# liuhuang31/Megatts2_HierSpeechpp

Measured on AMD Instinct MI355X. Metric: 16kHz audio samples/sec (whole node) + RTF, HierSpeech++ vocoder batch=32, higher is better.
Workload: dtype f32; 1 GPU; vocoder-only infer(): 32 utterances x 4 s per GPU (BASELINE.json configs[1]), synthetic weights; batch_per_gpu=32, frames=200, global_batch=32, parallelism=dp1 (contiguous utterance shards of the global batch, one RCCL weight broadcast), launch_mode=hipGraph replay of the captured step

## Files before the change

include/hsp.h:

```cpp
#ifndef HSP_H_
#define HSP_H_

#include <stdint.h>

#ifdef __cplusplus
extern "C" {
#endif
#if defined(__GNUC__) || defined(__clang__)
#pragma GCC visibility push(default)
#endif

#define HSP_VERSION 104
#define HSP_EINVAL (-1)

int hsp_version(void);
const char* hsp_arch(void);


enum {
  HSP_PRO_NONE = 0,
  HSP_PRO_LRELU = 1,
  HSP_PRO_ACT1D = 2,
  HSP_PRO_SILU = 3
};

enum {
  HSP_ACT_NONE = 0,
  HSP_ACT_TANH = 1,
  HSP_ACT_GELU_TANH = 2,
  HSP_ACT_RELU = 3,
  HSP_ACT_MISH = 4,
  HSP_ACT_SILU = 5,
  HSP_ACT_SOFTPLUS = 6,
  HSP_ACT_GELU_ERF = 7
};

enum {
  HSP_ROWS_PLAIN = 0,
  HSP_ROWS_GATE_WN = 1,
  HSP_ROWS_GATE_GLU = 2,
  HSP_ROWS_SHUFFLE = 3
};

enum { HSP_MASK_NONE = 0, HSP_MASK_PRE = 1, HSP_MASK_POST = 2, HSP_MASK_BOTH = 3 };

typedef struct hsp_conv1d_args {
  const float* x;
  int64_t x_bs, x_cs, x_ts;
  int32_t B, Cin, Lin;
  const float* w;
  int32_t K, M, dil, pad, stride;
  const float* zeros;
  int32_t w_ld;
  float* y;
  int64_t y_bs, y_cs;
  int32_t Cout, Lout;
  int32_t ncols;
  int32_t prologue;
  float slope;
  const float* alpha_exp;
  const float* beta_inv;
  const float* filt;
  int32_t rows, gate_half, up, shuf_pad;
  const float* bias;
  const float* cbias;
  int64_t cbias_bs;
  int32_t act;
  const float* mask;
  int64_t mask_bs;
  int32_t mask_mode;
  const float* cscale;
  int64_t cscale_bs;
  float scale;
  const float* res;
  int64_t res_bs, res_cs;
  int32_t accumulate;
  float post_scale;
  int32_t debug;
  const float* ln_c1;
  float ln_eps;
  int32_t split_row;
  int32_t accumulate2;
  int32_t mask_mode2;
  float* y2;
  int64_t y2_bs, y2_cs;
  int64_t res_ts;
  int64_t w_bs;
} hsp_conv1d_args;

int hsp_conv1d_mfma_f32(const hsp_conv1d_args* a, void* stream);
int hsp_conv1d_direct_f32(const hsp_conv1d_args* a, void* stream);
int hsp_conv1d_mfma_plan(const hsp_conv1d_args* a, int32_t out4[4]);

int hsp_act_f32(const float* x, float* y, int64_t n, int32_t act, void* stream);
int hsp_reflect_pad_f32(const float* x, int64_t x_bs, float* y, int32_t B, int32_t L, int32_t pad, void* stream);
int hsp_f0_convert_f32(const float* f0_src, int32_t n_src, const float* f0_trg, int32_t n_trg, float* out, void* stream);

int hsp_reflect_pad_ragged_f32(const float* x, int64_t x_bs, const int64_t* lengths, float* y, int64_t y_bs, int32_t B,
                               int32_t L, int32_t pad, int32_t Lo, void* stream);
int hsp_f0_convert_batch_f32(const float* f0_src, int64_t src_bs, const int64_t* n_src, const float* f0_trg,
                             int64_t trg_bs, const int64_t* n_trg, int32_t nt_max, float* out, int64_t out_bs,
                             int32_t B, int32_t n_max, void* stream);
int hsp_stft_frames_ragged_f32(const float* x, int64_t x_bs, const int64_t* lengths, const float* window, float* frames,
                               int32_t B, int32_t L, int32_t n_fft, int32_t hop, int32_t T, int32_t f_ld, void* stream);
int hsp_abs_max_rows_f32(const float* x, int64_t x_bs, const int64_t* lengths, float* out, int32_t B, int64_t n,
                         void* stream);
int hsp_peak_int16_gains(const float* x, int64_t x_bs, const int64_t* lengths, const float* gains, int16_t* out,
                         int64_t o_bs, int32_t B, int64_t n, void* stream);

int hsp_mag_pha_f32(const float* spec, int64_t s_ld, float* mag, float* pha, int32_t n_freqs, int32_t T, float compress,
                    void* stream);
int hsp_lsigmoid_mul_f32(const float* m, const float* slope, float beta, const float* mag, float* out, int32_t T,
                         int32_t F, void* stream);
int hsp_atan2_f32(const float* y, const float* x, float* out, int64_t n, void* stream);
int hsp_polar_f32(const float* mag, const float* pha, float power, float* re, int64_t re_ld, float* im, int64_t im_ld,
                  int32_t F, int32_t T, void* stream);

int hsp_norm_factor_rows_f32(const float* x, int64_t x_bs, const int64_t* lengths, float* scale, float* inv, int32_t B,
                             int64_t L, void* stream);
int hsp_stft_frames_packed_f32(const float* x, int64_t x_bs, const int64_t* lengths, const float* scale,
                               const float* window, float* frames, const int32_t* seg, const int32_t* seg_host, int32_t B,
                               int64_t L, int32_t n_fft, int32_t hop, int32_t T_tot, int32_t f_ld, void* stream);
int hsp_instnorm_prelu_seg_f32(float* x, int64_t x_cs, int32_t C, int32_t T_tot, int32_t F, const int32_t* seg,
                               const int32_t* seg_host, int32_t B, const float* gamma, const float* beta,
                               const float* slope, float eps, void* stream);
int hsp_zero_gaps_f32(float* x, int64_t x_cs, int32_t C, int32_t T_tot, int32_t F, const int32_t* seg,
                      const int32_t* seg_host, int32_t B, void* stream);
int hsp_dwconv_bn_silu_seg_f32(const float* x, const float* w, const float* bias, const float* bn_weight,
                               const float* bn_bias, const float* bn_mean, const float* bn_var, float bn_eps, float* y,
                               int32_t A, int32_t C, int32_t N, int32_t K, const int32_t* seg, const int32_t* seg_host,
                               int32_t B, void* stream);
int hsp_istft_ola_seg_f32(const float* frames, int64_t f_ld, const float* window, const float* inv, float* out,
                          int64_t out_bs, int64_t n_max, int32_t n_fft, int32_t hop, const int32_t* seg,
                          const int32_t* seg_host, int32_t B, int32_t T_tot, void* stream);

int hsp_act1d_snakebeta_f32(const float* x, float* y, int32_t B, int32_t C, int32_t L,
                            const float* alpha_exp, const float* beta_inv, const float* filt,
                            void* stream);
int hsp_act1d_snakebeta_ragged_f32(const float* x, float* y, int32_t B, int32_t C, int32_t L, const int64_t* lens,
                                   const float* alpha_exp, const float* beta_inv, const float* filt, void* stream);
int hsp_snake_consts_f32(const float* alpha_log, const float* beta_log, float* alpha_exp,
                         float* beta_inv, int32_t C, void* stream);

int hsp_fold_weight_norm_f32(const float* v, const float* g, float* w, int32_t rows, int32_t cols,
                             void* stream);
int hsp_gather_f32(const float* src, const int32_t* map, float* dst, int64_t n, void* stream);

int hsp_sequence_mask_f32(const int64_t* length, float* mask, int32_t B, int32_t T, void* stream);
int hsp_flip_channels_f32(const float* x, float* y, int32_t B, int32_t C, int32_t T, void* stream);
int hsp_sample_prior_f32(const float* stats, const float* noise, const float* mask, float* z,
                         int32_t B, int32_t C, int32_t T, float noise_scale, void* stream);
int hsp_layernorm_mod_f32(const float* x, float* y, int32_t B, int32_t C, int32_t T, float eps,
                          const float* mask, const float* shift, const float* scale, int64_t mod_bs,
                          const float* gamma, const float* beta, void* stream);
typedef struct hsp_mha_args {
  const float *q, *k, *v;
  float* o;
  int64_t q_bs, k_bs, v_bs, o_bs;
  int32_t B, H, D, Tq, Tk;
  float qk_scale;
  const float* mask_q;
  const float* mask_k;
  const float* rel_k;
  const float* rel_v;
  int32_t window;
  int64_t q_cs, k_cs, v_cs, o_cs;
  const float* mask_dense;
  int64_t mask_dense_bs;
} hsp_mha_args;
int hsp_mha_f32(const hsp_mha_args* a, void* stream);
#define HSP_MHA_TOK 0
#define HSP_MHA_MFMA_WHOLE 1
#define HSP_MHA_MFMA_SLAB 2
#define HSP_MHA_MFMA_STREAM 3
#define HSP_MHA_ROW 4
#define HSP_MHA_ROW_STREAM 5
int hsp_mha_plan(const hsp_mha_args* a, int32_t out4[4]);
typedef struct hsp_mha_proj_args {
  const float *q, *k, *v;
  int64_t q_bs, q_cs, k_bs, k_cs, v_bs, v_cs;
  int32_t B, H, D, Tq, Tk;
  float qk_scale;
  const float* wt;
  int32_t M, wt_ld;
  const float* bias;
  const float* mask;
  int64_t mask_bs;
  const float* cscale;
  int64_t cscale_bs;
  const float* res;
  int64_t res_bs, res_cs, res_ts;
  float* y;
  int64_t y_bs, y_cs, y_ts;
  int32_t debug;
  const int64_t* key_len;
} hsp_mha_proj_args;
int hsp_mha_proj_f32(const hsp_mha_proj_args* a, void* stream);
int hsp_mha_proj_supported(int32_t H, int32_t D, int32_t M, int32_t Tk);
int hsp_masked_mean_f32(const float* x, const float* mask, float* out, int32_t B, int32_t C,
                        int32_t T, void* stream);
int hsp_mask_mul_f32(const float* x, const float* mask, float* y, int32_t B, int32_t C, int32_t T, void* stream);
int hsp_linear_interp_f32(const float* x, float* y, int32_t B, int32_t C, int32_t Lin, int32_t Lout, void* stream);
int hsp_linear_interp_ragged_f32(const float* x, float* y, int32_t B, int32_t C, int32_t Lin, int32_t Lout,
                                 const int64_t* lin, const int64_t* lout, void* stream);
int hsp_axpby_f32(const float* x, const float* z, float* y, float a, float b, int64_t n, void* stream);


int hsp_plm_embed_f32(const float* tc, int64_t tc_bs, int64_t tc_cs, int32_t Dtc, const int64_t* codes,
                      int64_t codes_bs, const float* emb, int32_t Demb, int32_t n_emb, const float* pe_t,
                      int32_t P, const float* alpha, float* x, int64_t x_bs, int64_t x_cs, int32_t B, int32_t n,
                      void* stream);
int hsp_plm_embed_step_f32(const float* tc, int64_t tc_bs, int64_t tc_cs, int32_t Dtc, int64_t* codes,
                           int64_t codes_bs, const float* emb, int32_t Demb, int32_t n_emb, const float* pe_t,
                           int32_t P, const float* alpha, float* x, int64_t x_bs, int64_t x_cs, int32_t B, int32_t n,
                           const float* logits, int64_t l_bs, int64_t l_cs, int32_t n_logits, void* stream);
int hsp_argmax_f32(const float* logits, int64_t l_bs, int64_t l_cs, int32_t B, int32_t N, int64_t* out,
                   int64_t out_bs, void* stream);

typedef struct hsp_sample_args {
  float temperature;
  int32_t top_k;
  float top_p;
  float repetition_penalty;
  const int64_t* seeds;
  float* probs;
  int64_t probs_bs;
} hsp_sample_args;
int hsp_plm_embed_sample_f32(const float* tc, int64_t tc_bs, int64_t tc_cs, int32_t Dtc, int64_t* codes,
                             int64_t codes_bs, const float* emb, int32_t Demb, int32_t n_emb, const float* pe_t,
                             int32_t P, const float* alpha, float* x, int64_t x_bs, int64_t x_cs, int32_t B, int32_t n,
                             const float* logits, int64_t l_bs, int64_t l_cs, int32_t n_logits, int32_t j,
                             const hsp_sample_args* args, void* stream);
int hsp_sample_f32(const float* logits, int64_t l_bs, int64_t l_cs, int32_t B, int32_t N, int64_t* out, int64_t out_bs,
                   int32_t j, const hsp_sample_args* args, void* stream);

#define HSP_PLM_DECODE_SPLIT 12
typedef struct hsp_plm_decode_args {
  const float* x;
  int64_t x_bs, x_cs;
  float* y;
  int64_t y_bs, y_cs;
  float *k_cache, *v_cache;
  int64_t bs, cs;
  int32_t t, B, D, H, F;
  float eps;
  const float *g1, *b1, *wqkv_t, *bqkv, *wo_t, *bo, *g2, *b2, *w1_t, *c1, *w2_t, *c2;
  void* workspace;
  int64_t workspace_bytes;
  int32_t debug;
} hsp_plm_decode_args;
int hsp_plm_decode_supported(int32_t D, int32_t H, int32_t F);
int64_t hsp_plm_decode_workspace_bytes(int32_t B, int32_t D);
int hsp_plm_decode_layer_f32(const hsp_plm_decode_args* a, void* stream);
int hsp_plm_decode_layer_pos_f32(const hsp_plm_decode_args* a, const int32_t* pos, void* stream);
int hsp_plm_embed_pos_f32(const float* tc, int64_t tc_bs, int64_t tc_cs, int32_t Dtc, const int64_t* codes,
                          int64_t codes_bs, const float* emb, int32_t Demb, int32_t n_emb, const float* pe_t, int32_t P,
                          const float* alpha, float* x, int64_t x_bs, int64_t x_cs, int32_t B, const int32_t* pos,
                          int32_t max_pos, void* stream);
int hsp_plm_choose_advance_f32(const float* logits, int64_t l_bs, int64_t l_cs, int32_t B, int32_t N, int64_t* codes,
                               int64_t codes_bs, int32_t* pos, const int32_t* len, int32_t max_pos,
                               const hsp_sample_args* args, void* stream);
#define HSP_PLM_PREFILL_MAX_N 65536
typedef struct hsp_plm_prefill_attn_args {
  const float* qkv;
  int64_t q_rs;
  float* out;
  int64_t o_rs;
  float *k_cache, *v_cache;
  int64_t cs;
  int32_t n, D, H;
  int32_t debug;
} hsp_plm_prefill_attn_args;
int hsp_plm_prefill_attn_supported(int32_t D, int32_t H);
int hsp_plm_prefill_attn_f32(const hsp_plm_prefill_attn_args* a, void* stream);
int hsp_copy_strided_f32(const float* x, int64_t s_bs, int64_t s_cs, int64_t s_ts, float* y, int32_t B,
                         int32_t C, int32_t T, void* stream);


int hsp_embedding_sum_f32(const int64_t* id0, const int64_t* id1, const int64_t* id2, const float* tab0,
                          const float* tab1, const float* tab2, int32_t n0, int32_t n1, int32_t n2, float scale,
                          float* out, int64_t o_bs, int64_t o_cs, int32_t B, int32_t C, int32_t T, void* stream);
int hsp_lstm_bidir_f32(const float* xproj, int64_t xp_bs, const float* whh_t, const float* bhh,
                       const int64_t* lengths, float* out, int64_t o_bs, int64_t o_cs, int32_t B, int32_t H,
                       int32_t N, void* stream);
int hsp_duration_f32(const float* logw, int64_t lw_bs, const int64_t* lengths, float length_scale, float* dur,
                     int64_t d_bs, float* frames, int32_t B, int32_t N, void* stream);
int hsp_maxpool1d_f32(const float* x, int64_t x_bs, int64_t x_cs, float* y, int32_t B, int32_t C, int32_t L,
                      int32_t k, void* stream);
int hsp_vq_nearest_f32(const float* x, int64_t x_bs, int64_t x_cs, const float* embed, int64_t* codes, int64_t c_bs,
                       int32_t B, int32_t D, int32_t T, int32_t bins, int32_t rep, int32_t Tout, void* stream);
int hsp_gaussian_upsample_f32(const float* x, int64_t x_bs, int64_t x_cs, const float* dur, int64_t d_bs,
                              const float* rng, int64_t r_bs, const int64_t* lengths, const float* frames,
                              float* out, int32_t B, int32_t C, int32_t N, int32_t T, void* stream);
int hsp_add_cbias_f32(const float* x, int64_t x_bs, int64_t x_cs, const float* cb, int64_t cb_bs, float* y,
                      int32_t B, int32_t C, int32_t T, void* stream);

int hsp_zero_below_f32(const float* x, float thr, float* y, int64_t n, void* stream);
int hsp_peak_int16(const float* x, int64_t x_bs, const int64_t* lengths, float gain, int16_t* out, int64_t o_bs,
                   int32_t B, int64_t n, void* stream);

int64_t hsp_loudness_workspace_bytes(int32_t B, int64_t n);
int hsp_loudness_coefs_f64(int32_t sample_rate, double* coefs);
int hsp_loudness_f32(const float* x, int64_t x_bs, const int64_t* lengths, int32_t B, int64_t n, int32_t sample_rate,
                     void* workspace, int64_t workspace_bytes, float* lufs, float* peak, void* stream);
int hsp_loudness_gains_f32(const float* lufs, const float* peak, float target_lufs, float ceiling, float* gains,
                           int32_t* limited, int32_t B, void* stream);

int hsp_resample_f32(const float* x, int64_t x_bs, const int64_t* lengths, int32_t B, int32_t L, const float* bank,
                     const int32_t* tap0, int32_t n_taps, int32_t o, int32_t n, int32_t width, float* y, int64_t y_bs,
                     int32_t T_out, void* stream);

int hsp_stft_frames_f32(const float* x, const float* window, float* frames, int32_t B, int32_t L, int32_t n_fft,
                        int32_t hop, int32_t T, int32_t f_ld, void* stream);
int hsp_power_mel_log_f32(const float* spec, int64_t s_bs, int32_t s_ld, const float* fb, const int32_t* f_lo,
                          const int32_t* f_hi, float* out, int32_t B, int32_t n_freqs, int32_t n_mels,
                          int32_t T_out, float eps, void* stream);

#define HSP_DFTSEG_TABLE_FLOATS 4160
typedef struct hsp_dftseg_args {
  const float* x;
  int64_t x_bs, x_cs;
  float* y;
  int64_t y_bs, y_cs;
  int32_t B, C, L;
  int32_t k, dil, pad, nseg, Np;
  float* xf;
  int64_t xf_bs;
  const float* dft;
  const float* bias;
  const float* res;
  int64_t res_bs, res_cs;
  int32_t accumulate;
  float post_scale;
  const float* act_alpha_exp;
  const float* act_beta_inv;
  const float* act_filt;
  int32_t prod3;
  const int64_t* act_len;
} hsp_dftseg_args;
int hsp_dftseg_fwd_f32(const hsp_dftseg_args* a, void* stream);
int hsp_dftseg_inv_f32(const hsp_dftseg_args* a, void* stream);
int hsp_dftseg_tables_f32(float* fwd, float* inv);
int hsp_dftseg_pair_supported(const hsp_dftseg_args* inv, const hsp_dftseg_args* fwd);
int hsp_dftseg_pair_f32(const hsp_dftseg_args* inv, const hsp_dftseg_args* fwd, void* stream);

int hsp_dftseg_supported(const hsp_dftseg_args* a);

typedef struct hsp_cprod3_args {
  const float* xf;
  float* yf;
  const float* w;
  const float* zeros;
  int64_t xf_bs, yf_bs;
  int32_t bins, C, Np;
  int32_t debug;
} hsp_cprod3_args;
int hsp_cprod3_f32(const hsp_cprod3_args* a, void* stream);
int hsp_cprod3_supported(const hsp_cprod3_args* a);
#define HSP_WSPEC_BLOCK 0
#define HSP_WSPEC_THREE 1
int hsp_dftseg_weight_spectrum_f32(const float* w, int32_t k, int32_t C, int32_t w_ld, const double* tw, float* out,
                                   int32_t form, void* stream);

int hsp_conv1d_f32(const hsp_conv1d_args* a, void* stream);
int hsp_convtr1d_f32(const hsp_conv1d_args* a, void* stream);
int hsp_wn_layer_f32(const hsp_conv1d_args* in_layer, const hsp_conv1d_args* res, const hsp_conv1d_args* skip,
                     void* stream);
int hsp_ffn_conv_f32(const hsp_conv1d_args* fc1, const hsp_conv1d_args* fc2, void* stream);
int hsp_layernorm_modulate_f32(const float* x, float* y, int32_t B, int32_t C, int32_t T, float eps,
                               const float* mask, const float* shift, const float* scale, int64_t mod_bs,
                               void* stream);

#if defined(__GNUC__) || defined(__clang__)
#pragma GCC visibility pop
#endif
#ifdef __cplusplus
}
#endif
#endif
```

megatts2_hierspeechpp_amd/_lib.py:

```python
from __future__ import annotations

import ctypes as C
import os
from typing import Optional

import torch

_HERE = os.path.dirname(os.path.abspath(__file__))
LIB_PATH = os.environ.get("HSP_LIB", os.path.join(_HERE, "libhsp.so"))

PRO_NONE, PRO_LRELU, PRO_ACT1D, PRO_SILU = 0, 1, 2, 3
ACT_NONE, ACT_TANH, ACT_GELU_TANH, ACT_RELU, ACT_MISH, ACT_SILU, ACT_SOFTPLUS, ACT_GELU_ERF = 0, 1, 2, 3, 4, 5, 6, 7
ROWS_PLAIN, ROWS_GATE_WN, ROWS_GATE_GLU, ROWS_SHUFFLE = 0, 1, 2, 3
MASK_NONE, MASK_PRE, MASK_POST, MASK_BOTH = 0, 1, 2, 3
EINVAL = -1
MHA_TOK, MHA_MFMA_WHOLE, MHA_MFMA_SLAB, MHA_MFMA_STREAM, MHA_ROW, MHA_ROW_STREAM = range(6)

_fp = C.c_void_p


class Conv1dArgs(C.Structure):
    _fields_ = [
        ("x", _fp), ("x_bs", C.c_int64), ("x_cs", C.c_int64), ("x_ts", C.c_int64),
        ("B", C.c_int32), ("Cin", C.c_int32), ("Lin", C.c_int32),
        ("w", _fp), ("K", C.c_int32), ("M", C.c_int32), ("dil", C.c_int32), ("pad", C.c_int32), ("stride", C.c_int32),
        ("zeros", _fp), ("w_ld", C.c_int32),
        ("y", _fp), ("y_bs", C.c_int64), ("y_cs", C.c_int64),
        ("Cout", C.c_int32), ("Lout", C.c_int32), ("ncols", C.c_int32),
        ("prologue", C.c_int32), ("slope", C.c_float),
        ("alpha_exp", _fp), ("beta_inv", _fp), ("filt", _fp),
        ("rows", C.c_int32), ("gate_half", C.c_int32), ("up", C.c_int32), ("shuf_pad", C.c_int32),
        ("bias", _fp), ("cbias", _fp), ("cbias_bs", C.c_int64),
        ("act", C.c_int32),
        ("mask", _fp), ("mask_bs", C.c_int64), ("mask_mode", C.c_int32),
        ("cscale", _fp), ("cscale_bs", C.c_int64), ("scale", C.c_float),
        ("res", _fp), ("res_bs", C.c_int64), ("res_cs", C.c_int64),
        ("accumulate", C.c_int32), ("post_scale", C.c_float), ("debug", C.c_int32),
        ("ln_c1", _fp), ("ln_eps", C.c_float),
        ("split_row", C.c_int32), ("accumulate2", C.c_int32), ("mask_mode2", C.c_int32), ("y2", _fp),
        ("y2_bs", C.c_int64), ("y2_cs", C.c_int64), ("res_ts", C.c_int64), ("w_bs", C.c_int64),
    ]


class MhaArgs(C.Structure):
    _fields_ = [
        ("q", _fp), ("k", _fp), ("v", _fp), ("o", _fp),
        ("q_bs", C.c_int64), ("k_bs", C.c_int64), ("v_bs", C.c_int64), ("o_bs", C.c_int64),
        ("B", C.c_int32), ("H", C.c_int32), ("D", C.c_int32), ("Tq", C.c_int32), ("Tk", C.c_int32),
        ("qk_scale", C.c_float),
        ("mask_q", _fp), ("mask_k", _fp), ("rel_k", _fp), ("rel_v", _fp), ("window", C.c_int32),
        ("q_cs", C.c_int64), ("k_cs", C.c_int64), ("v_cs", C.c_int64), ("o_cs", C.c_int64),
        ("mask_dense", _fp), ("mask_dense_bs", C.c_int64),
    ]


class MhaProjArgs(C.Structure):
    _fields_ = [
        ("q", _fp), ("k", _fp), ("v", _fp),
        ("q_bs", C.c_int64), ("q_cs", C.c_int64), ("k_bs", C.c_int64), ("k_cs", C.c_int64), ("v_bs", C.c_int64),
        ("v_cs", C.c_int64),
        ("B", C.c_int32), ("H", C.c_int32), ("D", C.c_int32), ("Tq", C.c_int32), ("Tk", C.c_int32),
        ("qk_scale", C.c_float),
        ("wt", _fp), ("M", C.c_int32), ("wt_ld", C.c_int32),
        ("bias", _fp), ("mask", _fp), ("mask_bs", C.c_int64), ("cscale", _fp), ("cscale_bs", C.c_int64),
        ("res", _fp), ("res_bs", C.c_int64), ("res_cs", C.c_int64), ("res_ts", C.c_int64),
        ("y", _fp), ("y_bs", C.c_int64), ("y_cs", C.c_int64), ("y_ts", C.c_int64), ("debug", C.c_int32),
        ("key_len", _fp),
    ]


class DftSegArgs(C.Structure):
    _fields_ = [
        ("x", _fp), ("x_bs", C.c_int64), ("x_cs", C.c_int64),
        ("y", _fp), ("y_bs", C.c_int64), ("y_cs", C.c_int64),
        ("B", C.c_int32), ("C", C.c_int32), ("L", C.c_int32),
        ("k", C.c_int32), ("dil", C.c_int32), ("pad", C.c_int32), ("nseg", C.c_int32), ("Np", C.c_int32),
        ("xf", _fp), ("xf_bs", C.c_int64), ("dft", _fp),
        ("bias", _fp), ("res", _fp), ("res_bs", C.c_int64), ("res_cs", C.c_int64),
        ("accumulate", C.c_int32), ("post_scale", C.c_float),
        ("act_alpha_exp", _fp), ("act_beta_inv", _fp), ("act_filt", _fp), ("prod3", C.c_int32),
        ("act_len", _fp),
    ]


class Cprod3Args(C.Structure):
    _fields_ = [
        ("xf", _fp), ("yf", _fp), ("w", _fp), ("zeros", _fp), ("xf_bs", C.c_int64), ("yf_bs", C.c_int64),
        ("bins", C.c_int32), ("C", C.c_int32), ("Np", C.c_int32), ("debug", C.c_int32),
    ]


class SampleArgs(C.Structure):
    _fields_ = [
        ("temperature", C.c_float), ("top_k", C.c_int32), ("top_p", C.c_float), ("repetition_penalty", C.c_float),
        ("seeds", _fp), ("probs", _fp), ("probs_bs", C.c_int64),
    ]


class PlmDecodeArgs(C.Structure):
    _fields_ = [
        ("x", _fp), ("x_bs", C.c_int64), ("x_cs", C.c_int64),
        ("y", _fp), ("y_bs", C.c_int64), ("y_cs", C.c_int64),
        ("k_cache", _fp), ("v_cache", _fp), ("bs", C.c_int64), ("cs", C.c_int64),
        ("t", C.c_int32), ("B", C.c_int32), ("D", C.c_int32), ("H", C.c_int32), ("F", C.c_int32), ("eps", C.c_float),
        ("g1", _fp), ("b1", _fp), ("wqkv_t", _fp), ("bqkv", _fp), ("wo_t", _fp), ("bo", _fp), ("g2", _fp), ("b2", _fp),
        ("w1_t", _fp), ("c1", _fp), ("w2_t", _fp), ("c2", _fp),
        ("workspace", _fp), ("workspace_bytes", C.c_int64), ("debug", C.c_int32),
    ]


class PlmPrefillAttnArgs(C.Structure):
    _fields_ = [
        ("qkv", _fp), ("q_rs", C.c_int64), ("out", _fp), ("o_rs", C.c_int64),
        ("k_cache", _fp), ("v_cache", _fp), ("cs", C.c_int64),
        ("n", C.c_int32), ("D", C.c_int32), ("H", C.c_int32), ("debug", C.c_int32),
    ]


WSPEC_BLOCK, WSPEC_THREE = 0, 1


SIGNATURES = {
    "hsp_version": (C.c_int, []),
    "hsp_arch": (C.c_char_p, []),
    "hsp_conv1d_mfma_f32": (C.c_int, [C.POINTER(Conv1dArgs), _fp]),
    "hsp_conv1d_direct_f32": (C.c_int, [C.POINTER(Conv1dArgs), _fp]),
    "hsp_conv1d_mfma_plan": (C.c_int, [C.POINTER(Conv1dArgs), C.POINTER(C.c_int32 * 4)]),
    "hsp_act1d_snakebeta_f32": (C.c_int, [_fp, _fp, C.c_int32, C.c_int32, C.c_int32, _fp, _fp, _fp, _fp]),
    "hsp_act1d_snakebeta_ragged_f32": (C.c_int, [_fp, _fp, C.c_int32, C.c_int32, C.c_int32, _fp, _fp, _fp, _fp, _fp]),
    "hsp_snake_consts_f32": (C.c_int, [_fp, _fp, _fp, _fp, C.c_int32, _fp]),
    "hsp_fold_weight_norm_f32": (C.c_int, [_fp, _fp, _fp, C.c_int32, C.c_int32, _fp]),
    "hsp_gather_f32": (C.c_int, [_fp, _fp, _fp, C.c_int64, _fp]),
    "hsp_sequence_mask_f32": (C.c_int, [_fp, _fp, C.c_int32, C.c_int32, _fp]),
    "hsp_flip_channels_f32": (C.c_int, [_fp, _fp, C.c_int32, C.c_int32, C.c_int32, _fp]),
    "hsp_sample_prior_f32": (C.c_int, [_fp, _fp, _fp, _fp, C.c_int32, C.c_int32, C.c_int32, C.c_float, _fp]),
    "hsp_layernorm_mod_f32": (C.c_int, [_fp, _fp, C.c_int32, C.c_int32, C.c_int32, C.c_float, _fp, _fp, _fp,
                                        C.c_int64, _fp, _fp, _fp]),
    "hsp_mha_f32": (C.c_int, [C.POINTER(MhaArgs), _fp]),
    "hsp_mha_plan": (C.c_int, [C.POINTER(MhaArgs), C.POINTER(C.c_int32 * 4)]),
    "hsp_mha_proj_f32": (C.c_int, [C.POINTER(MhaProjArgs), _fp]),
    "hsp_dftseg_fwd_f32": (C.c_int, [C.POINTER(DftSegArgs), _fp]),
    "hsp_dftseg_inv_f32": (C.c_int, [C.POINTER(DftSegArgs), _fp]),
    "hsp_dftseg_tables_f32": (C.c_int, [_fp, _fp]),
    "hsp_dftseg_pair_supported": (C.c_int, [C.POINTER(DftSegArgs), C.POINTER(DftSegArgs)]),
    "hsp_dftseg_pair_f32": (C.c_int, [C.POINTER(DftSegArgs), C.POINTER(DftSegArgs), _fp]),
    "hsp_dftseg_supported": (C.c_int, [C.POINTER(DftSegArgs)]),
    "hsp_cprod3_f32": (C.c_int, [C.POINTER(Cprod3Args), _fp]),
    "hsp_cprod3_supported": (C.c_int, [C.POINTER(Cprod3Args)]),
    "hsp_dftseg_weight_spectrum_f32": (C.c_int, [_fp, C.c_int32, C.c_int32, C.c_int32, _fp, _fp, C.c_int32, _fp]),
    "hsp_mha_proj_supported": (C.c_int, [C.c_int32, C.c_int32, C.c_int32, C.c_int32]),
    "hsp_masked_mean_f32": (C.c_int, [_fp, _fp, _fp, C.c_int32, C.c_int32, C.c_int32, _fp]),
    "hsp_mask_mul_f32": (C.c_int, [_fp, _fp, _fp, C.c_int32, C.c_int32, C.c_int32, _fp]),
    "hsp_linear_interp_f32": (C.c_int, [_fp, _fp, C.c_int32, C.c_int32, C.c_int32, C.c_int32, _fp]),
    "hsp_linear_interp_ragged_f32": (C.c_int, [_fp, _fp, C.c_int32, C.c_int32, C.c_int32, C.c_int32, _fp, _fp, _fp]),
    "hsp_axpby_f32": (C.c_int, [_fp, _fp, _fp, C.c_float, C.c_float, C.c_int64, _fp]),
    "hsp_plm_embed_f32": (C.c_int, [_fp, C.c_int64, C.c_int64, C.c_int32, _fp, C.c_int64, _fp, C.c_int32, C.c_int32,
                                    _fp, C.c_int32, _fp, _fp, C.c_int64, C.c_int64, C.c_int32, C.c_int32, _fp]),
    "hsp_plm_embed_step_f32": (C.c_int, [_fp, C.c_int64, C.c_int64, C.c_int32, _fp, C.c_int64, _fp, C.c_int32, C.c_int32,
                                         _fp, C.c_int32, _fp, _fp, C.c_int64, C.c_int64, C.c_int32, C.c_int32, _fp, C.c_int64,
                                         C.c_int64, C.c_int32, _fp]),
    "hsp_argmax_f32": (C.c_int, [_fp, C.c_int64, C.c_int64, C.c_int32, C.c_int32, _fp, C.c_int64, _fp]),
    "hsp_plm_embed_sample_f32": (C.c_int, [_fp, C.c_int64, C.c_int64, C.c_int32, _fp, C.c_int64, _fp, C.c_int32,
                                           C.c_int32, _fp, C.c_int32, _fp, _fp, C.c_int64, C.c_int64, C.c_int32,
                                           C.c_int32, _fp, C.c_int64, C.c_int64, C.c_int32, C.c_int32,
                                           C.POINTER(SampleArgs), _fp]),
    "hsp_sample_f32": (C.c_int, [_fp, C.c_int64, C.c_int64, C.c_int32, C.c_int32, _fp, C.c_int64, C.c_int32,
                                 C.POINTER(SampleArgs), _fp]),
    "hsp_plm_decode_supported": (C.c_int, [C.c_int32, C.c_int32, C.c_int32]),
    "hsp_plm_decode_workspace_bytes": (C.c_int64, [C.c_int32, C.c_int32]),
    "hsp_plm_decode_layer_f32": (C.c_int, [C.POINTER(PlmDecodeArgs), _fp]),
    "hsp_plm_decode_layer_pos_f32": (C.c_int, [C.POINTER(PlmDecodeArgs), _fp, _fp]),
    "hsp_plm_embed_pos_f32": (C.c_int, [_fp, C.c_int64, C.c_int64, C.c_int32, _fp, C.c_int64, _fp, C.c_int32, C.c_int32,
                                        _fp, C.c_int32, _fp, _fp, C.c_int64, C.c_int64, C.c_int32, _fp, C.c_int32, _fp]),
    "hsp_plm_choose_advance_f32": (C.c_int, [_fp, C.c_int64, C.c_int64, C.c_int32, C.c_int32, _fp, C.c_int64, _fp, _fp,
                                             C.c_int32, C.POINTER(SampleArgs), _fp]),
    "hsp_plm_prefill_attn_supported": (C.c_int, [C.c_int32, C.c_int32]),
    "hsp_plm_prefill_attn_f32": (C.c_int, [C.POINTER(PlmPrefillAttnArgs), _fp]),
    "hsp_embedding_sum_f32": (C.c_int, [_fp, _fp, _fp, _fp, _fp, _fp, C.c_int32, C.c_int32, C.c_int32, C.c_float, _fp,
                                        C.c_int64, C.c_int64, C.c_int32, C.c_int32, C.c_int32, _fp]),
    "hsp_lstm_bidir_f32": (C.c_int, [_fp, C.c_int64, _fp, _fp, _fp, _fp, C.c_int64, C.c_int64, C.c_int32, C.c_int32,
                                     C.c_int32, _fp]),
    "hsp_duration_f32": (C.c_int, [_fp, C.c_int64, _fp, C.c_float, _fp, C.c_int64, _fp, C.c_int32, C.c_int32, _fp]),
    "hsp_gaussian_upsample_f32": (C.c_int, [_fp, C.c_int64, C.c_int64, _fp, C.c_int64, _fp, C.c_int64, _fp, _fp, _fp,
                                            C.c_int32, C.c_int32, C.c_int32, C.c_int32, _fp]),
    "hsp_act_f32": (C.c_int, [_fp, _fp, C.c_int64, C.c_int32, _fp]),
    "hsp_reflect_pad_f32": (C.c_int, [_fp, C.c_int64, _fp, C.c_int32, C.c_int32, C.c_int32, _fp]),
    "hsp_f0_convert_f32": (C.c_int, [_fp, C.c_int32, _fp, C.c_int32, _fp, _fp]),
    "hsp_reflect_pad_ragged_f32": (C.c_int, [_fp, C.c_int64, _fp, _fp, C.c_int64, C.c_int32, C.c_int32, C.c_int32,
                                             C.c_int32, _fp]),
    "hsp_f0_convert_batch_f32": (C.c_int, [_fp, C.c_int64, _fp, _fp, C.c_int64, _fp, C.c_int32, _fp, C.c_int64, C.c_int32,
                                           C.c_int32, _fp]),
    "hsp_stft_frames_ragged_f32": (C.c_int, [_fp, C.c_int64, _fp, _fp, _fp, C.c_int32, C.c_int32, C.c_int32, C.c_int32,
                                             C.c_int32, C.c_int32, _fp]),
    "hsp_abs_max_rows_f32": (C.c_int, [_fp, C.c_int64, _fp, _fp, C.c_int32, C.c_int64, _fp]),
    "hsp_peak_int16_gains": (C.c_int, [_fp, C.c_int64, _fp, _fp, _fp, C.c_int64, C.c_int32, C.c_int64, _fp]),
    "hsp_mag_pha_f32": (C.c_int, [_fp, C.c_int64, _fp, _fp, C.c_int32, C.c_int32, C.c_float, _fp]),
    "hsp_lsigmoid_mul_f32": (C.c_int, [_fp, _fp, C.c_float, _fp, _fp, C.c_int32, C.c_int32, _fp]),
    "hsp_atan2_f32": (C.c_int, [_fp, _fp, _fp, C.c_int64, _fp]),
    "hsp_polar_f32": (C.c_int, [_fp, _fp, C.c_float, _fp, C.c_int64, _fp, C.c_int64, C.c_int32, C.c_int32, _fp]),
    "hsp_norm_factor_rows_f32": (C.c_int, [_fp, C.c_int64, _fp, _fp, _fp, C.c_int32, C.c_int64, _fp]),
    "hsp_stft_frames_packed_f32": (C.c_int, [_fp, C.c_int64, _fp, _fp, _fp, _fp, _fp, _fp, C.c_int32, C.c_int64, C.c_int32,
                                             C.c_int32, C.c_int32, C.c_int32, _fp]),
    "hsp_instnorm_prelu_seg_f32": (C.c_int, [_fp, C.c_int64, C.c_int32, C.c_int32, C.c_int32, _fp, _fp, C.c_int32, _fp, _fp,
                                             _fp, C.c_float, _fp]),
    "hsp_zero_gaps_f32": (C.c_int, [_fp, C.c_int64, C.c_int32, C.c_int32, C.c_int32, _fp, _fp, C.c_int32, _fp]),
    "hsp_dwconv_bn_silu_seg_f32": (C.c_int, [_fp, _fp, _fp, _fp, _fp, _fp, _fp, C.c_float, _fp, C.c_int32, C.c_int32,
                                             C.c_int32, C.c_int32, _fp, _fp, C.c_int32, _fp]),
    "hsp_istft_ola_seg_f32": (C.c_int, [_fp, C.c_int64, _fp, _fp, _fp, C.c_int64, C.c_int64, C.c_int32, C.c_int32, _fp, _fp,
                                        C.c_int32, C.c_int32, _fp]),
    "hsp_maxpool1d_f32": (C.c_int, [_fp, C.c_int64, C.c_int64, _fp, C.c_int32, C.c_int32, C.c_int32, C.c_int32, _fp]),
    "hsp_vq_nearest_f32": (C.c_int, [_fp, C.c_int64, C.c_int64, _fp, _fp, C.c_int64, C.c_int32, C.c_int32, C.c_int32,
                                     C.c_int32, C.c_int32, C.c_int32, _fp]),
    "hsp_add_cbias_f32": (C.c_int, [_fp, C.c_int64, C.c_int64, _fp, C.c_int64, _fp, C.c_int32, C.c_int32, C.c_int32, _fp]),
    "hsp_zero_below_f32": (C.c_int, [_fp, C.c_float, _fp, C.c_int64, _fp]),
    "hsp_peak_int16": (C.c_int, [_fp, C.c_int64, _fp, C.c_float, _fp, C.c_int64, C.c_int32, C.c_int64, _fp]),
    "hsp_loudness_workspace_bytes": (C.c_int64, [C.c_int32, C.c_int64]),
    "hsp_loudness_coefs_f64": (C.c_int, [C.c_int32, _fp]),
    "hsp_loudness_f32": (C.c_int, [_fp, C.c_int64, _fp, C.c_int32, C.c_int64, C.c_int32, _fp, C.c_int64, _fp, _fp, _fp]),
    "hsp_loudness_gains_f32": (C.c_int, [_fp, _fp, C.c_float, C.c_float, _fp, _fp, C.c_int32, _fp]),
    "hsp_resample_f32": (C.c_int, [_fp, C.c_int64, _fp, C.c_int32, C.c_int32, _fp, _fp, C.c_int32, C.c_int32, C.c_int32,
                                   C.c_int32, _fp, C.c_int64, C.c_int32, _fp]),
    "hsp_copy_strided_f32": (C.c_int, [_fp, C.c_int64, C.c_int64, C.c_int64, _fp, C.c_int32, C.c_int32, C.c_int32,
                                       _fp]),
    "hsp_conv1d_f32": (C.c_int, [C.POINTER(Conv1dArgs), _fp]),
    "hsp_convtr1d_f32": (C.c_int, [C.POINTER(Conv1dArgs), _fp]),
    "hsp_wn_layer_f32": (C.c_int, [C.POINTER(Conv1dArgs), C.POINTER(Conv1dArgs), C.POINTER(Conv1dArgs), _fp]),
    "hsp_ffn_conv_f32": (C.c_int, [C.POINTER(Conv1dArgs), C.POINTER(Conv1dArgs), _fp]),
    "hsp_layernorm_modulate_f32": (C.c_int, [_fp, _fp, C.c_int32, C.c_int32, C.c_int32, C.c_float, _fp, _fp, _fp,
                                             C.c_int64, _fp]),
    "hsp_stft_frames_f32": (C.c_int, [_fp, _fp, _fp, C.c_int32, C.c_int32, C.c_int32, C.c_int32, C.c_int32, C.c_int32,
                                      _fp]),
    "hsp_power_mel_log_f32": (C.c_int, [_fp, C.c_int64, C.c_int32, _fp, _fp, _fp, _fp, C.c_int32, C.c_int32, C.c_int32,
                                        C.c_int32, C.c_float, _fp]),
}

_lib: Optional[C.CDLL] = None


class HspError(RuntimeError):
    pass


def lib() -> C.CDLL:
    global _lib
    if _lib is None:
        if not os.path.exists(LIB_PATH):
            raise HspError(
                f"{LIB_PATH} not found: build the HIP kernels first "
                "(python -c 'import __graft_entry__ as g; g.build()' or make -C megatts2_hierspeechpp_amd/csrc). "
                "There is no CPU fallback for the product path.")
        handle = C.CDLL(LIB_PATH)
        for name, (res, args) in SIGNATURES.items():
            fn = getattr(handle, name)
            fn.restype, fn.argtypes = res, args
        _lib = handle
    return _lib


def check(code: int, what: str) -> None:
    if code != 0:
        kind = "invalid arguments" if code == EINVAL else f"hipError_t {code}"
        raise HspError(f"{what} failed: {kind}")


def ptr(t: Optional[torch.Tensor]) -> Optional[int]:
    if t is None:
        return None
    if not t.is_cuda:
        raise HspError("libhsp kernels run on the GPU only (got a CPU tensor); there is no CPU fallback")
    return t.data_ptr()


def fptr(t: Optional[torch.Tensor]) -> Optional[int]:
    if t is not None and t.dtype != torch.float32:
        raise HspError(f"expected float32, got {t.dtype}")
    return ptr(t)


def stream_ptr() -> int:
    return torch.cuda.current_stream().cuda_stream
```

megatts2_hierspeechpp_amd/csrc/hsp_bgemm.hip:

```cpp
#include "hsp_device.h"

#ifdef HSP_TUNING
#define BG_DBG(a, bit) (((a).debug & (bit)) != 0)
#else
#define BG_DBG(a, bit) false
#endif

namespace {

typedef float bg_f32x16 __attribute__((ext_vector_type(16)));
constexpr int BG_KS = 48;
constexpr int bg_gs(int tm, int tn) { return tm * tn >= 2 ? 2 : 4; }

#define BG_GPTR(p) ((const __attribute__((address_space(1))) void*)(p))
#define BG_LPTR(p) ((__attribute__((address_space(3))) void*)(p))

template <int TM, int TN>
struct BgCfg {
  static constexpr int BM = 64 * TM, BN = 64 * TN;
  static constexpr int NST = TM * TN == 2 ? 4 : 3;
  static constexpr int STAGE = BG_KS * (BM + BN);
  static constexpr int NIW = BG_KS * BM / 256, NIX = BG_KS * BN / 256;
  static constexpr int LPW = (NIW + NIX) / 4;
  static constexpr int LDS_BYTES = NST * STAGE * (int)sizeof(float);
  static_assert(NIW % 4 == 0 && NIX % 4 == 0, "four producer waves share a stage evenly");
  static_assert(LPW * (NST - 1) <= 63, "vmcnt is six bits");
};

__device__ __forceinline__ void bg_barrier() {
  asm volatile("s_waitcnt lgkmcnt(0)" ::: "memory");
  __builtin_amdgcn_s_barrier();
  asm volatile("" ::: "memory");
}

typedef const __attribute__((address_space(3))) float* bg_lptr;
template <int TM, int TN, int G>
__device__ __forceinline__ void bg_read(float (&A)[bg_gs(TM, TN) * TM], float (&B)[bg_gs(TM, TN) * TN], bg_lptr wa, bg_lptr xa) {
  constexpr int GS = bg_gs(TM, TN);
#pragma unroll
  for (int step = 0; step < GS; ++step) {
    const int kk = GS * G + step;
#pragma unroll
    for (int j = 0; j < TM; ++j) A[step * TM + j] = wa[kk * 2 * 64 * TM + j * 32];
#pragma unroll
    for (int j = 0; j < TN; ++j) B[step * TN + j] = xa[kk * 2 * 64 * TN + j * 32];
  }
}

template <int TM, int TN, bool LN, int SEL, bool TAIL, int G = 0>
__device__ __forceinline__ void bg_stage(bg_f32x16 (&acc)[TM * TN], float (&A0)[bg_gs(TM, TN) * TM],
                                         float (&B0)[bg_gs(TM, TN) * TN], float (&A1)[bg_gs(TM, TN) * TM],
                                         float (&B1)[bg_gs(TM, TN) * TN], bg_lptr wa, bg_lptr xa, float& s1, float& s2,
                                         float pivot, int rows2) {
  constexpr int GS = bg_gs(TM, TN), NG = BG_KS / (2 * GS);
  if constexpr (G < NG) {
    if constexpr (G + 1 < NG) bg_read<TM, TN, G + 1>(A1, B1, wa, xa);
#pragma unroll
    for (int i = 0; i < GS; ++i) {
      if constexpr (LN) {
        float d = B0[i * TN + SEL] - pivot;
        if constexpr (TAIL) d = GS * G + i < rows2 ? d : 0.0f;
        s1 += d;
        s2 = fmaf(d, d, s2);
      }
#pragma unroll
      for (int tm = 0; tm < TM; ++tm)
#pragma unroll
        for (int tn = 0; tn < TN; ++tn)
          acc[tm * TN + tn] = __builtin_amdgcn_mfma_f32_32x32x2f32(A0[i * TM + tm], B0[i * TN + tn], acc[tm * TN + tn], 0, 0, 0);
    }
    __builtin_amdgcn_sched_barrier(0);
    bg_stage<TM, TN, LN, SEL, TAIL, G + 1>(acc, A1, B1, A0, B0, wa, xa, s1, s2, pivot, rows2);
  }
}

template <int TM, int TN, bool LN, int ACT>
__device__ __forceinline__ void bg_epilogue(const hsp_conv1d_args& a, const bg_f32x16 (&acc)[TM * TN], int b, int mw, int nw,
                                            int l32, int half, float bvl, float c1l, const float (&mean)[TN],
                                            const float (&rstd)[TN]) {
#pragma unroll
  for (int tm = 0; tm < TM; ++tm) {
    float bvr[16], c1r[16];
#pragma unroll
    for (int r = 0; r < 16; ++r) {
      const int src = tm * 32 + (r & 3) + 8 * (r >> 2) + 4 * half;
      bvr[r] = __shfl(bvl, src, 64);
      c1r[r] = LN ? __shfl(c1l, src, 64) : 0.0f;
    }
    {
      const unsigned yo = 4u * (unsigned)(l32 + 4 * half * a.y_cs), ro = 4u * (unsigned)(l32 + 4 * half * a.res_cs);
      const char* ybase = reinterpret_cast<const char*>(a.y + (int64_t)b * a.y_bs + nw);
      const char* rbase = a.res ? reinterpret_cast<const char*>(a.res + (int64_t)b * a.res_bs + nw) : nullptr;
#pragma unroll
      for (int tn = 0; tn < TN; ++tn) {
        if (nw + tn * 32 + l32 < a.ncols) {
          float rv[16];
#pragma unroll
          for (int r = 0; r < 16; ++r) {
            const int mc = min(mw + tm * 32 + (r & 3) + 8 * (r >> 2), a.Cout - 1 - 4 * half);
            rv[r] = rbase ? *reinterpret_cast<const float*>(rbase + (int64_t)mc * a.res_cs * 4 + tn * 128 + ro) : 0.0f;
          }
#pragma unroll
          for (int q = 0; q < 4; ++q) {
            const int mu = mw + tm * 32 + 8 * q;
            if (mu + 4 * half < a.Cout) {
#pragma unroll
              for (int i = 0; i < 4; ++i) {
                const int r = 4 * q + i;
                const float fin = acc[tm * TN + tn][r];
                float v = fin + bvr[r];
                if constexpr (LN) v = fmaf(rstd[tn], fmaf(-mean[tn], c1r[r], fin), bvr[r]);
                if constexpr (ACT == HSP_ACT_RELU) v = fmaxf(v, 0.0f);
                else if constexpr (ACT == HSP_ACT_GELU_TANH) v = hsp_apply_act(v, HSP_ACT_GELU_TANH);
                v += rv[r];
                *reinterpret_cast<float*>(const_cast<char*>(ybase) + (int64_t)(mu + i) * a.y_cs * 4 + tn * 128 + yo) = v;
              }
            }
          }
        }
      }
    }
  }
}

template <int TM, int TN, int ACT>
__device__ __forceinline__ void bg_epilogue_ext(const hsp_conv1d_args& a, const bg_f32x16 (&acc)[TM * TN], int b, int m0, int mw,
                                                int nw, int l32, int half, float bvl) {
  const bool second = a.split_row > 0 && m0 >= a.split_row;
  const int mo = second ? a.split_row : 0;
  const int mmode = second ? a.mask_mode2 : a.mask_mode;
  const bool accum = (second ? a.accumulate2 : a.accumulate) != 0;
  const int64_t ycs = second ? a.y2_cs : a.y_cs;
  const char* ybase = reinterpret_cast<const char*>((second ? a.y2 + (int64_t)b * a.y2_bs : a.y + (int64_t)b * a.y_bs) + nw);
  const char* rbase = (a.res && !second) ? reinterpret_cast<const char*>(a.res + (int64_t)b * a.res_bs + nw) : nullptr;
  const unsigned yo = 4u * (unsigned)(l32 + 4 * half * (int)ycs), ro = 4u * (unsigned)(l32 + 4 * half * a.res_cs);
  const float csl = a.cscale ? a.cscale[(int64_t)b * a.cscale_bs + min(mw + l32 + 32 * half, a.Cout - 1)] : 1.0f;
  const float sc = a.scale, ps = a.post_scale;
#pragma unroll
  for (int tm = 0; tm < TM; ++tm) {
    float bvr[16], csr[16];
#pragma unroll
    for (int r = 0; r < 16; ++r) {
      const int src = tm * 32 + (r & 3) + 8 * (r >> 2) + 4 * half;
      bvr[r] = __shfl(bvl, src, 64);
      csr[r] = __shfl(csl, src, 64);
    }
#pragma unroll
    for (int tn = 0; tn < TN; ++tn) {
      const int n = nw + tn * 32 + l32;
      if (n < a.ncols) {
        const float mk = mmode != HSP_MASK_NONE ? a.mask[(int64_t)b * a.mask_bs + n] : 1.0f;
        const float mk_pre = (mmode & HSP_MASK_PRE) ? mk : 1.0f, mk_post = (mmode & HSP_MASK_POST) ? mk : 1.0f;
        float rv[16], yv[16];
#pragma unroll
        for (int r = 0; r < 16; ++r) {
          const int mc = min(mw + tm * 32 + (r & 3) + 8 * (r >> 2), a.Cout - 1 - 4 * half) - mo;
          rv[r] = rbase ? *reinterpret_cast<const float*>(rbase + (int64_t)mc * a.res_cs * 4 + tn * 128 + ro) : 0.0f;
          yv[r] = accum ? *reinterpret_cast<const float*>(ybase + (int64_t)mc * ycs * 4 + tn * 128 + yo) : 0.0f;
        }
#pragma unroll
        for (int q = 0; q < 4; ++q) {
          const int mu = mw + tm * 32 + 8 * q;
          if (mu + 4 * half < a.Cout) {
#pragma unroll
            for (int i = 0; i < 4; ++i) {
              const int r = 4 * q + i;
              float v = acc[tm * TN + tn][r] + bvr[r];
              if constexpr (ACT == HSP_ACT_RELU) v = fmaxf(v, 0.0f);
              else if constexpr (ACT == HSP_ACT_GELU_TANH) v = hsp_apply_act(v, HSP_ACT_GELU_TANH);
              v *= mk_pre;
              v *= csr[r];
              v *= sc;
              v += rv[r];
              v *= mk_post;
              v += yv[r];
              *reinterpret_cast<float*>(const_cast<char*>(ybase) + (int64_t)(mu + i - mo) * ycs * 4 + tn * 128 + yo) = v * ps;
            }
          }
        }
      }
    }
  }
}

template <int N>
__device__ __forceinline__ void bg_wait_vm() { asm volatile("s_waitcnt vmcnt(%0)" ::"n"(N) : "memory"); }

template <int TM, int TN, bool LN, bool EXT>
__global__ __launch_bounds__(512, 1) void bgemm_kernel(const hsp_conv1d_args a, int n_mt, int n_nt, int per_xcd,
                                                       int total) {
  using C = BgCfg<TM, TN>;
  extern __shared__ __attribute__((aligned(16))) float lds[];
  const int xcd = blockIdx.x & 7, idx = blockIdx.x >> 3;
  int id = xcd * per_xcd + idx;
  if (id >= total) return;
  const int mt = id % n_mt;
  id /= n_mt;
  const int nt = id % n_nt;
  const int b = id / n_nt;
  const int m0 = mt * C::BM, n0 = nt * C::BN;
  const int tid = threadIdx.x, lane = tid & 63, wave = __builtin_amdgcn_readfirstlane(tid >> 6);
  const int K = a.Cin;
  const int nstage = (K + BG_KS - 1) / BG_KS;
#ifdef HSP_TUNING
  unsigned long long* stamps = ((a.debug & (1 << 20)) && blockIdx.x == 0 && lane == 0 && (wave == 0 || wave == 4))
                                   ? (unsigned long long*)a.filt : nullptr;
#define BG_STAMP(i) do { if (stamps) stamps[i] = __builtin_readcyclecounter(); } while (0)
#else
#define BG_STAMP(i) do { } while (0)
#endif
  if (wave == 0) BG_STAMP(0);

  if (wave >= 4) {
    const int pw = wave - 4;
    constexpr int LPRW = C::BM / 4, RPIW = 64 / LPRW;
    constexpr int LPRX = C::BN / 4, RPIX = 64 / LPRX;
    const int rw = lane / LPRW, cw = (lane % LPRW) * 4;
    const int rx = lane / LPRX, cx = (lane % LPRX) * 4;
    const bool mok = m0 + cw < a.M, nok = n0 + cx < a.ncols;
    const float* wsrc = a.w + m0 + cw;
    const float* xsrc = a.x + (int64_t)b * a.x_bs + n0 + cx;
    const bool wfast = m0 + C::BM <= a.M, xfast = n0 + C::BN <= a.ncols && a.x_cs < (1 << 26);
    const float* wlane = a.w + m0 + rw * a.w_ld + cw;
    const float* xlane = a.x + (int64_t)b * a.x_bs + n0 + (xfast ? rx * (int)a.x_cs : 0) + cx;
    const int wld = a.w_ld, xcs = (int)a.x_cs;
    auto issue = [&](int s) __attribute__((always_inline)) {
      float* Ws = lds + (s % C::NST) * C::STAGE;
      float* Xs = Ws + BG_KS * C::BM;
      const int k0 = s * BG_KS;
      const bool kfull = k0 + BG_KS <= K;
      if (wfast && kfull) {
#pragma unroll
        for (int q = 0; q < C::NIW / 4; ++q) {
          const int r0 = (pw + 4 * q) * RPIW;
          const int eo = __builtin_amdgcn_readfirstlane((k0 + r0) * wld);
          __builtin_amdgcn_global_load_lds(BG_GPTR(wlane + eo), BG_LPTR(Ws + r0 * C::BM), 16, 0, 0);
        }
      } else {
#pragma unroll
        for (int q = 0; q < C::NIW / 4; ++q) {
          const int r0 = (pw + 4 * q) * RPIW;
          const int k = k0 + r0 + rw;
          const float* src = (mok && k < K) ? wsrc + (int64_t)k * a.w_ld : a.zeros;
          __builtin_amdgcn_global_load_lds(BG_GPTR(src), BG_LPTR(Ws + r0 * C::BM), 16, 0, 0);
        }
      }
      if (xfast && kfull) {
#pragma unroll
        for (int q = 0; q < C::NIX / 4; ++q) {
          const int r0 = (pw + 4 * q) * RPIX;
          const int eo = __builtin_amdgcn_readfirstlane((k0 + r0) * xcs);
          __builtin_amdgcn_global_load_lds(BG_GPTR(xlane + eo), BG_LPTR(Xs + r0 * C::BN), 16, 0, 0);
        }
      } else {
#pragma unroll
        for (int q = 0; q < C::NIX / 4; ++q) {
          const int r0 = (pw + 4 * q) * RPIX;
          const int k = k0 + r0 + rx;
          const float* src = (nok && k < K) ? xsrc + (int64_t)k * a.x_cs : a.zeros;
          __builtin_amdgcn_global_load_lds(BG_GPTR(src), BG_LPTR(Xs + r0 * C::BN), 16, 0, 0);
        }
      }
    };
    const int npre = nstage < C::NST ? nstage : C::NST;
    BG_STAMP(4);
    for (int s = 0; s < npre; ++s) issue(s);
    BG_STAMP(5);
    for (int s = 0; s < nstage; ++s) {
      const int behind = (s + C::NST < nstage ? s + C::NST : nstage) - (s + 1);
      if (behind >= 3) bg_wait_vm<3 * C::LPW>();
      else if (behind == 2) bg_wait_vm<2 * C::LPW>();
      else if (behind == 1) bg_wait_vm<C::LPW>();
      else bg_wait_vm<0>();
      if (s == 0) BG_STAMP(6);
      bg_barrier();
      if (s + C::NST < nstage) {
        bg_barrier();
        if (!BG_DBG(a, 1)) issue(s + C::NST);
      }
    }
    return;
  }

  const int l32 = lane & 31, half = lane >> 5;
  const int wm = wave & 1, wn = wave >> 1;
  const int mw = m0 + wm * (32 * TM), nw = n0 + wn * (32 * TN);
  bg_f32x16 acc[TM * TN];
#pragma unroll
  for (int t = 0; t < TM * TN; ++t)
#pragma unroll
    for (int r = 0; r < 16; ++r) acc[t][r] = 0.0f;
  float bvl, c1l = 0.0f;
  {
    const int mc = min(mw + lane, a.Cout - 1);
    bvl = a.bias ? a.bias[mc] : 0.0f;
    if (a.cbias) bvl += a.cbias[(int64_t)b * a.cbias_bs + mc];
    if constexpr (LN) c1l = a.ln_c1[mc];
  }
  constexpr int GS = bg_gs(TM, TN);
  const int sel = TN == 2 ? wm : 0;
  float s1 = 0.0f, s2 = 0.0f, pivot = 0.0f;
  float A0[GS * TM], B0[GS * TN], A1[GS * TM], B1[GS * TN];
  for (int s = 0; s < nstage; ++s) {
    bg_barrier();
    if (s == 0) BG_STAMP(1);
    const float* Ws = lds + (s % C::NST) * C::STAGE;
    const float* Xs = Ws + BG_KS * C::BM;
    if (LN && s == 0) pivot = Xs[wn * (32 * TN) + sel * 32 + l32];
    int rows = K - s * BG_KS;
    rows = rows > BG_KS ? BG_KS : rows;
    const bg_lptr wa = (bg_lptr)(Ws + half * C::BM + wm * (32 * TM) + l32);
    const bg_lptr xa = (bg_lptr)(Xs + half * C::BN + wn * (32 * TN) + l32);
    if (!BG_DBG(a, 2)) {
      bg_read<TM, TN, 0>(A0, B0, wa, xa);
      if constexpr (!LN) {
        bg_stage<TM, TN, false, 0, false>(acc, A0, B0, A1, B1, wa, xa, s1, s2, pivot, 0);
      } else if (BG_DBG(a, 1 << 25)) {
        bg_stage<TM, TN, false, 0, false>(acc, A0, B0, A1, B1, wa, xa, s1, s2, pivot, 0);
        s2 = 1.0f;
      } else if (rows == BG_KS) {
        if (sel) bg_stage<TM, TN, true, TN - 1, false>(acc, A0, B0, A1, B1, wa, xa, s1, s2, pivot, 0);
        else bg_stage<TM, TN, true, 0, false>(acc, A0, B0, A1, B1, wa, xa, s1, s2, pivot, 0);
      } else {
        if (sel) bg_stage<TM, TN, true, TN - 1, true>(acc, A0, B0, A1, B1, wa, xa, s1, s2, pivot, rows >> 1);
        else bg_stage<TM, TN, true, 0, true>(acc, A0, B0, A1, B1, wa, xa, s1, s2, pivot, rows >> 1);
      }
    }
    if (s + C::NST < nstage) bg_barrier();
  }

  BG_STAMP(2);
  float mean[TN], rstd[TN];
#pragma unroll
  for (int tn = 0; tn < TN; ++tn) {
    mean[tn] = 0.0f;
    rstd[tn] = 1.0f;
  }
  if constexpr (LN) {
    const float t1 = s1 + __shfl_xor(s1, 32, 64);
    const float t2 = s2 + __shfl_xor(s2, 32, 64);
    const float dm = t1 / (float)K;
    const float mu = pivot + dm;
    const float var = fmaxf(t2 / (float)K - dm * dm, 0.0f);
    const float rs = 1.0f / sqrtf(var + a.ln_eps);
    if constexpr (TN == 1) {
      mean[0] = mu;
      rstd[0] = rs;
    } else {
      float* xch = lds + (nstage % C::NST) * C::STAGE;
      if (half == 0) {
        xch[((wn * 2 + wm) * 2 + 0) * 32 + l32] = mu;
        xch[((wn * 2 + wm) * 2 + 1) * 32 + l32] = rs;
      }
      bg_barrier();
      const float mu2 = xch[((wn * 2 + (1 - wm)) * 2 + 0) * 32 + l32];
      const float rs2 = xch[((wn * 2 + (1 - wm)) * 2 + 1) * 32 + l32];
      mean[0] = wm == 0 ? mu : mu2;
      mean[TN - 1] = wm == 0 ? mu2 : mu;
      rstd[0] = wm == 0 ? rs : rs2;
      rstd[TN - 1] = wm == 0 ? rs2 : rs;
    }
  }

  if constexpr (EXT) {
    static_assert(!LN, "the extended epilogue is not built with the fused LayerNorm");
    if (a.act == HSP_ACT_RELU) bg_epilogue_ext<TM, TN, HSP_ACT_RELU>(a, acc, b, m0, mw, nw, l32, half, bvl);
    else if (a.act == HSP_ACT_GELU_TANH) bg_epilogue_ext<TM, TN, HSP_ACT_GELU_TANH>(a, acc, b, m0, mw, nw, l32, half, bvl);
    else bg_epilogue_ext<TM, TN, HSP_ACT_NONE>(a, acc, b, m0, mw, nw, l32, half, bvl);
  } else {
    if (a.act == HSP_ACT_RELU) bg_epilogue<TM, TN, LN, HSP_ACT_RELU>(a, acc, b, mw, nw, l32, half, bvl, c1l, mean, rstd);
    else if (a.act == HSP_ACT_GELU_TANH) bg_epilogue<TM, TN, LN, HSP_ACT_GELU_TANH>(a, acc, b, mw, nw, l32, half, bvl, c1l, mean, rstd);
    else bg_epilogue<TM, TN, LN, HSP_ACT_NONE>(a, acc, b, mw, nw, l32, half, bvl, c1l, mean, rstd);
  }
  BG_STAMP(3);
#undef BG_STAMP
}

template <int TM, int TN, bool LN, bool EXT>
int bg_launch(const hsp_conv1d_args& a, hipStream_t s, int n_mt, int n_nt, int total) {
  using C = BgCfg<TM, TN>;
  static_assert(C::LDS_BYTES > 32 * 1024, "every launch raises the LDS limit");
  const int per_xcd = (total + 7) / 8;
  return hsp_launch<bgemm_kernel<TM, TN, LN, EXT>>(8 * per_xcd, 512, C::LDS_BYTES, C::LDS_BYTES, s, a, n_mt, n_nt, per_xcd, total);
}

inline bool bg_extended(const hsp_conv1d_args& a) {
  return a.mask_mode != HSP_MASK_NONE || a.cscale || a.accumulate || a.scale != 1.0f || a.post_scale != 1.0f || a.split_row > 0;
}

template <int TM, int TN>
int bg_go(const hsp_conv1d_args& a, hipStream_t s, int32_t* plan_out) {
  using C = BgCfg<TM, TN>;
  const int n_mt = (a.M + C::BM - 1) / C::BM, n_nt = (a.ncols + C::BN - 1) / C::BN;
  const int64_t total = (int64_t)n_mt * n_nt * a.B;
  if (total <= 0 || total > 0x3fffffff) return -1;
  if (plan_out) {
    plan_out[0] = C::BM; plan_out[1] = C::BN; plan_out[2] = -2; plan_out[3] = C::LDS_BYTES;
    return 0;
  }
  if (bg_extended(a)) return bg_launch<TM, TN, false, true>(a, s, n_mt, n_nt, (int)total);
  return a.ln_c1 ? bg_launch<TM, TN, true, false>(a, s, n_mt, n_nt, (int)total)
                 : bg_launch<TM, TN, false, false>(a, s, n_mt, n_nt, (int)total);
}

}

int hsp_bgemm_try(const hsp_conv1d_args& a, hipStream_t s, int32_t* plan_out) {
  auto al16 = [](const void* p) { return (reinterpret_cast<uintptr_t>(p) & 15) == 0; };
  if (BG_DBG(a, 1 << 22)) return -1;
  if (a.K != 1 || a.stride != 1 || a.pad != 0 || a.prologue != HSP_PRO_NONE || a.rows != HSP_ROWS_PLAIN) return -1;
  if (a.x_ts != 1 || a.Lin != a.ncols || a.Lout != a.ncols) return -1;
  if ((a.Cin & 3) || (a.ncols & 3) || (a.x_bs & 3) || (a.x_cs & 3) || !al16(a.x) || !al16(a.w) || (a.w_ld & 3)) return -1;
  if (a.Cin < 96 || a.Cin > 8192) return -1;
  if (a.ln_c1 && !(a.ln_eps > 0.0f)) return -1;
  if (a.mask_mode != HSP_MASK_NONE && !a.mask) return -1;
  if (a.act != HSP_ACT_NONE && a.act != HSP_ACT_RELU && a.act != HSP_ACT_GELU_TANH) return -1;
  if (a.y_cs >= (1 << 24) || a.res_cs >= (1 << 24) || (a.Cout & 3)) return -1;
  const bool ext = bg_extended(a);
  if (ext && a.ln_c1) return -1;
  if (a.split_row) {
    if (a.split_row < 0 || (a.split_row % 64) || a.split_row >= a.Cout || !a.y2 || a.y2_cs >= (1 << 24)) return -1;
    if (a.mask_mode2 != HSP_MASK_NONE && !a.mask) return -1;
  }
#ifdef HSP_TUNING
  if (!a.split_row) {
    if (a.debug & (1 << 18)) return bg_go<2, 2>(a, s, plan_out);
    if (a.debug & (1 << 19)) return bg_go<2, 1>(a, s, plan_out);
    if (a.debug & (1 << 21)) return bg_go<1, 2>(a, s, plan_out);
  }
  if (a.debug & (1 << 23)) return bg_go<1, 1>(a, s, plan_out);
#endif
  auto tiles = [&](int bm, int bn) { return (int64_t)((a.M + bm - 1) / bm) * ((a.ncols + bn - 1) / bn) * a.B; };
  auto waste_ok = [&](int bm) { return 4 * (int64_t)(((a.M + bm - 1) / bm) * bm - a.M) <= a.M; };
  const int64_t t64 = tiles(64, 64);
  if (t64 < 96 && !a.split_row) return -1;
  if (t64 >= 5000 && a.Cin <= 256 && !a.ln_c1 && !a.split_row && !bg_extended(a)) return -1;
  if (t64 >= 700 && a.M >= 768 && waste_ok(128) && a.ncols >= 512 && !a.split_row) {
    const int64_t t128 = tiles(128, 128);
    const int64_t rounds = (t128 + 255) / 256;
    if (100 * rounds * 256 <= 115 * t128) return bg_go<2, 2>(a, s, plan_out);
  }
  return bg_go<1, 1>(a, s, plan_out);
}
```

megatts2_hierspeechpp_amd/csrc/hsp_conv1d_direct.hip:

```cpp
#include <type_traits>
#include "hsp_device.h"

namespace {

__global__ __launch_bounds__(256) void conv1d_direct_kernel(const hsp_conv1d_args a) {
  const int64_t total = (int64_t)a.B * a.Cout * a.Lout;
  for (int64_t idx = (int64_t)blockIdx.x * blockDim.x + threadIdx.x; idx < total;
       idx += (int64_t)gridDim.x * blockDim.x) {
    const int t = (int)(idx % a.Lout);
    const int64_t r = idx / a.Lout;
    const int co = (int)(r % a.Cout);
    const int b = (int)(r / a.Cout);
    const float* xb = a.x + (int64_t)b * a.x_bs;
    float acc = 0.0f;
    for (int j = 0; j < a.K; ++j) {
      const int p = t * a.stride + j * a.dil - a.pad;
      if (p < 0 || p >= a.Lin) continue;
      const float* wj = a.w + (int64_t)j * a.Cin * a.w_ld + co;
      const float* xp = xb + (int64_t)p * a.x_ts;
      if (a.prologue == HSP_PRO_NONE) {
        float acc4[4] = {0.f, 0.f, 0.f, 0.f};
        int ci = 0;
        for (; ci + 8 <= a.Cin; ci += 8) {
          float wv[8], xv[8];
#pragma unroll
          for (int u = 0; u < 8; ++u) {
            wv[u] = wj[(int64_t)(ci + u) * a.w_ld];
            xv[u] = xp[(int64_t)(ci + u) * a.x_cs];
          }
#pragma unroll
          for (int u = 0; u < 8; ++u) acc4[u & 3] = fmaf(wv[u], xv[u], acc4[u & 3]);
        }
        for (; ci < a.Cin; ++ci) acc4[0] = fmaf(wj[(int64_t)ci * a.w_ld], xp[(int64_t)ci * a.x_cs], acc4[0]);
        acc += (acc4[0] + acc4[1]) + (acc4[2] + acc4[3]);
      } else {
        for (int ci = 0; ci < a.Cin; ++ci) {
          float xv = xp[(int64_t)ci * a.x_cs];
          if (a.prologue == HSP_PRO_LRELU) xv = xv > 0.0f ? xv : xv * a.slope;
          else if (a.prologue == HSP_PRO_SILU) xv = xv * hsp_sigmoid(xv);
          acc = fmaf(wj[(int64_t)ci * a.w_ld], xv, acc);
        }
      }
    }
    float v = acc;
    if (a.bias) v += a.bias[co];
    if (a.cbias) v += a.cbias[(int64_t)b * a.cbias_bs + co];
    v = hsp_apply_act(v, a.act);
    hsp_epilogue_store(a, b, co, t, v);
  }
}

constexpr int C1_MAXW = 4096;

template <int N, class F>
__device__ __forceinline__ void c1_static_for(F&& f) {
  if constexpr (N > 0) {
    c1_static_for<N - 1>(f);
    f(std::integral_constant<int, N - 1>{});
  }
}

template <int K>
__global__ __launch_bounds__(256) void conv1d_cout1_kernel(const hsp_conv1d_args a, int n_tiles) {
  constexpr int H = (K - 1) / 2, CU = 4;
  __shared__ float ws[C1_MAXW];
  for (int e = threadIdx.x; e < a.Cin * K; e += 256) {
    const int c = e / K, j = e - c * K;
    ws[e] = a.w[((int64_t)j * a.Cin + c) * a.w_ld];
  }
  __syncthreads();
  const int tile = blockIdx.x % n_tiles, b = blockIdx.x / n_tiles;
  const int t = tile * 1024 + 4 * threadIdx.x;
  if (t >= a.Lout) return;
  const int L = a.Lin;
  const float* xb = a.x + (int64_t)b * a.x_bs + t;
  const int64_t xcs = a.x_cs;
  float acc0 = 0.f, acc1 = 0.f, acc2 = 0.f, acc3 = 0.f;
  const bool lo = t - 4 >= 0, hi = t + 4 < L;
  const int offl = lo ? -4 : 0, offh = hi ? 4 : 0;
  const int ngroups = a.Cin / CU;
  for (int g = 0; g < ngroups; ++g) {
    const float* xc = xb + (int64_t)(g * CU) * xcs;
    float4 va[CU], vb[CU], vc[CU];
    c1_static_for<CU>([&](auto uu) __attribute__((always_inline)) {
      constexpr int u = decltype(uu)::value;
      va[u] = *reinterpret_cast<const float4*>(xc + u * xcs + offl);
      vb[u] = *reinterpret_cast<const float4*>(xc + u * xcs);
      vc[u] = *reinterpret_cast<const float4*>(xc + u * xcs + offh);
    });
    c1_static_for<CU>([&](auto uu) __attribute__((always_inline)) {
      constexpr int u = decltype(uu)::value;
      const float w_[12] = {lo ? va[u].x : 0.f, lo ? va[u].y : 0.f, lo ? va[u].z : 0.f, lo ? va[u].w : 0.f,
                            vb[u].x, vb[u].y, vb[u].z, vb[u].w,
                            hi ? vc[u].x : 0.f, hi ? vc[u].y : 0.f, hi ? vc[u].z : 0.f, hi ? vc[u].w : 0.f};
      const float* wc = ws + (g * CU + u) * K;
      c1_static_for<K>([&](auto jj) __attribute__((always_inline)) {
        constexpr int j = decltype(jj)::value;
        const float wj = wc[j];
        acc0 = fmaf(wj, w_[4 + j - H], acc0);
        acc1 = fmaf(wj, w_[5 + j - H], acc1);
        acc2 = fmaf(wj, w_[6 + j - H], acc2);
        acc3 = fmaf(wj, w_[7 + j - H], acc3);
      });
    });
  }
  for (int c = ngroups * CU; c < a.Cin; ++c) {
    const float* xc = xb + (int64_t)c * xcs;
    const float4 va = *reinterpret_cast<const float4*>(xc + offl);
    const float4 vb = *reinterpret_cast<const float4*>(xc);
    const float4 vc = *reinterpret_cast<const float4*>(xc + offh);
    const float w_[12] = {lo ? va.x : 0.f, lo ? va.y : 0.f, lo ? va.z : 0.f, lo ? va.w : 0.f, vb.x, vb.y, vb.z, vb.w,
                          hi ? vc.x : 0.f, hi ? vc.y : 0.f, hi ? vc.z : 0.f, hi ? vc.w : 0.f};
    const float* wc = ws + c * K;
    c1_static_for<K>([&](auto jj) __attribute__((always_inline)) {
      constexpr int j = decltype(jj)::value;
      const float wj = wc[j];
      acc0 = fmaf(wj, w_[4 + j - H], acc0);
      acc1 = fmaf(wj, w_[5 + j - H], acc1);
      acc2 = fmaf(wj, w_[6 + j - H], acc2);
      acc3 = fmaf(wj, w_[7 + j - H], acc3);
    });
  }
  const float bz = a.bias ? a.bias[0] : 0.0f;
  const float sc = a.scale * a.post_scale;
  float4 o;
  o.x = hsp_apply_act(acc0 + bz, a.act) * sc;
  o.y = hsp_apply_act(acc1 + bz, a.act) * sc;
  o.z = hsp_apply_act(acc2 + bz, a.act) * sc;
  o.w = hsp_apply_act(acc3 + bz, a.act) * sc;
  *reinterpret_cast<float4*>(a.y + (int64_t)b * a.y_bs + t) = o;
}

constexpr int LV_WAVES = 8, LV_BB = 8, LV_MAXC = 1024;

__global__ __launch_bounds__(64 * LV_WAVES) void linear_vec_kernel(const hsp_conv1d_args a) {
  __shared__ float xs[LV_BB][LV_MAXC];
  __shared__ float part[LV_WAVES][LV_BB][64];
  const int tid = threadIdx.x, lane = tid & 63, wave = tid >> 6;
  const int co = blockIdx.x * 64 + lane;
  const int b0 = blockIdx.y * LV_BB, nb = min(LV_BB, a.B - b0);
  for (int e = tid; e < nb * a.Cin; e += 64 * LV_WAVES) {
    const int bb = e / a.Cin, ci = e - bb * a.Cin;
    float v = a.x[(int64_t)(b0 + bb) * a.x_bs + (int64_t)ci * a.x_cs];
    if (a.prologue == HSP_PRO_LRELU) v = v > 0.0f ? v : v * a.slope;
    else if (a.prologue == HSP_PRO_SILU) v = v * hsp_sigmoid(v);
    xs[bb][ci] = v;
  }
  __syncthreads();
  const int per = (a.Cin + LV_WAVES - 1) / LV_WAVES;
  const int c0 = wave * per, c1 = min(c0 + per, a.Cin);
  const float* wc = a.w + min(co, a.M - 1);
  float acc[LV_BB];
#pragma unroll
  for (int bb = 0; bb < LV_BB; ++bb) acc[bb] = 0.0f;
  int ci = c0;
  for (; ci + 8 <= c1; ci += 8) {
    float wv[8];
#pragma unroll
    for (int u = 0; u < 8; ++u) wv[u] = wc[(int64_t)(ci + u) * a.w_ld];
#pragma unroll
    for (int u = 0; u < 8; ++u)
#pragma unroll
      for (int bb = 0; bb < LV_BB; ++bb) acc[bb] = fmaf(wv[u], xs[bb][ci + u], acc[bb]);
  }
  for (; ci < c1; ++ci) {
    const float wv = wc[(int64_t)ci * a.w_ld];
#pragma unroll
    for (int bb = 0; bb < LV_BB; ++bb) acc[bb] = fmaf(wv, xs[bb][ci], acc[bb]);
  }
#pragma unroll
  for (int bb = 0; bb < LV_BB; ++bb) part[wave][bb][lane] = acc[bb];
  __syncthreads();
  if (co >= a.Cout) return;
  for (int bb = wave; bb < nb; bb += LV_WAVES) {
    float v = 0.0f;
#pragma unroll
    for (int w = 0; w < LV_WAVES; ++w) v += part[w][bb][lane];
    const int b = b0 + bb;
    if (a.bias) v += a.bias[co];
    if (a.cbias) v += a.cbias[(int64_t)b * a.cbias_bs + co];
    v = hsp_apply_act(v, a.act);
    hsp_epilogue_store(a, b, co, 0, v);
  }
}

bool linear_vec_fast(const hsp_conv1d_args& a) {
  return a.K == 1 && a.Lin == 1 && a.Lout == 1 && a.stride == 1 && a.pad == 0 && a.Cin >= 64 && a.Cin <= LV_MAXC && a.Cout >= 64;
}

bool cout1_fast(const hsp_conv1d_args& a) {
  auto al16 = [](const void* p) { return (reinterpret_cast<uintptr_t>(p) & 15) == 0; };
  return a.Cout == 1 && a.stride == 1 && a.dil == 1 && a.K <= 9 && (a.K & 1) && a.pad == (a.K - 1) / 2 && a.x_ts == 1 &&
         a.Lin == a.Lout && (a.Lin & 3) == 0 && (a.x_cs & 3) == 0 && (a.x_bs & 3) == 0 && (a.y_bs & 3) == 0 && al16(a.x) &&
         al16(a.y) && a.prologue == HSP_PRO_NONE && !a.cbias && !a.cscale && !a.res && !a.accumulate &&
         a.mask_mode == HSP_MASK_NONE && (int64_t)a.Cin * a.K <= C1_MAXW;
}

}

extern "C" int hsp_conv1d_direct_f32(const hsp_conv1d_args* ap, void* stream) {
  if (!ap) return HSP_EINVAL;
  const hsp_conv1d_args& a = *ap;
  if (!a.x || !a.w || !a.y) return HSP_EINVAL;
  if (a.B <= 0 || a.Cin <= 0 || a.Lin <= 0 || a.K <= 0 || a.M <= 0 || a.Cout <= 0 || a.Lout <= 0) return HSP_EINVAL;
  if (a.stride < 1 || a.dil < 1 || a.rows != HSP_ROWS_PLAIN || a.Cout > a.M || a.w_ld < a.M) return HSP_EINVAL;
  if (a.prologue != HSP_PRO_NONE && a.prologue != HSP_PRO_LRELU && a.prologue != HSP_PRO_SILU) return HSP_EINVAL;
  if (a.mask_mode != HSP_MASK_NONE && !a.mask) return HSP_EINVAL;
  if (a.res && a.res_ts > 1) return HSP_EINVAL;
  if (a.w_bs) return HSP_EINVAL;
  if (a.ln_c1 || a.split_row) return HSP_EINVAL;
  if (linear_vec_fast(a)) {
    const unsigned gx = (unsigned)((a.Cout + 63) / 64), gy = (unsigned)((a.B + LV_BB - 1) / LV_BB);
    if (gy > 65535) return HSP_EINVAL;
    hipLaunchKernelGGL(linear_vec_kernel, dim3(gx, gy), dim3(64 * LV_WAVES), 0, static_cast<hipStream_t>(stream), a);
    return (int)hipGetLastError();
  }
  if (cout1_fast(a)) {
    const int n_tiles = (a.Lout + 1023) / 1024;
    const int64_t nb = (int64_t)n_tiles * a.B;
    if (nb > 0x7fffffff) return HSP_EINVAL;
    const hipStream_t st = static_cast<hipStream_t>(stream);
    switch (a.K) {
      case 1: hipLaunchKernelGGL(conv1d_cout1_kernel<1>, dim3((unsigned)nb), dim3(256), 0, st, a, n_tiles); break;
      case 3: hipLaunchKernelGGL(conv1d_cout1_kernel<3>, dim3((unsigned)nb), dim3(256), 0, st, a, n_tiles); break;
      case 5: hipLaunchKernelGGL(conv1d_cout1_kernel<5>, dim3((unsigned)nb), dim3(256), 0, st, a, n_tiles); break;
      case 7: hipLaunchKernelGGL(conv1d_cout1_kernel<7>, dim3((unsigned)nb), dim3(256), 0, st, a, n_tiles); break;
      default: hipLaunchKernelGGL(conv1d_cout1_kernel<9>, dim3((unsigned)nb), dim3(256), 0, st, a, n_tiles); break;
    }
    return (int)hipGetLastError();
  }
  const int64_t total = (int64_t)a.B * a.Cout * a.Lout;
  int64_t blocks = (total + 255) / 256;
  if (blocks > 262144) blocks = 262144;
  hipLaunchKernelGGL(conv1d_direct_kernel, dim3((unsigned)blocks), dim3(256), 0, static_cast<hipStream_t>(stream), a);
  return (int)hipGetLastError();
}
```

megatts2_hierspeechpp_amd/csrc/hsp_conv1d_mfma.hip:

```cpp
#include "hsp_conv1d_mfma_kernel.h"

int hsp_rgemm_try(const hsp_conv1d_args& a, hipStream_t s, int32_t* plan_out);
int hsp_bgemm_try(const hsp_conv1d_args& a, hipStream_t s, int32_t* plan_out);

namespace {
using namespace hspconv;

int validate(const hsp_conv1d_args& a) {
  if (!a.x || !a.w || !a.y) return HSP_EINVAL;
#ifndef HSP_TUNING
  if (a.debug != 0) return HSP_EINVAL;
#endif
  if (a.B <= 0 || a.Cin <= 0 || a.Lin <= 0 || a.K <= 0 || a.M <= 0 || a.Cout <= 0 || a.Lout <= 0 || a.ncols <= 0)
    return HSP_EINVAL;
  if (a.stride != 1 || (a.M & 3) || (a.w_ld & 3) || a.w_ld < a.M || a.dil < 1) return HSP_EINVAL;
  if ((reinterpret_cast<uintptr_t>(a.w) & 15) != 0 || a.w_bs < 0 || (a.w_bs & 3)) return HSP_EINVAL;
  if (a.w_bs && (a.ln_c1 || a.split_row || (a.res && a.res_ts > 1))) return HSP_EINVAL;
  if ((int64_t)a.K * a.Cin * a.w_ld >= (1ll << 31)) return HSP_EINVAL;
  if ((int64_t)a.Cin * a.x_cs + (int64_t)a.Lin * a.x_ts >= (1ll << 31) || a.x_cs < 0 || a.x_ts < 0) return HSP_EINVAL;
  if (a.y_cs < 0 || (int64_t)a.Cout * a.y_cs + a.Lout >= (1ll << 31)) return HSP_EINVAL;
  if (a.res && (a.res_cs < 0 || (int64_t)a.Cout * a.res_cs + a.Lout >= (1ll << 31))) return HSP_EINVAL;
  if (a.res_ts < 0 || (a.res && a.res_ts > 1 && (int64_t)a.Cout * a.res_cs + (int64_t)a.Lout * a.res_ts >= (1ll << 31))) return HSP_EINVAL;
  if (a.prologue == HSP_PRO_ACT1D && (!a.alpha_exp || !a.beta_inv || !a.filt || a.x_ts != 1)) return HSP_EINVAL;
  if (!a.zeros || (reinterpret_cast<uintptr_t>(a.zeros) & 15) != 0) return HSP_EINVAL;
  if (a.prologue != HSP_PRO_NONE && a.prologue != HSP_PRO_LRELU && a.prologue != HSP_PRO_ACT1D) return HSP_EINVAL;
  if (a.mask_mode != HSP_MASK_NONE && !a.mask) return HSP_EINVAL;
  if (a.rows == HSP_ROWS_GATE_WN || a.rows == HSP_ROWS_GATE_GLU) {
    if (a.gate_half <= 0 || (a.gate_half & 31) || a.M != 2 * a.gate_half || a.Cout != a.gate_half) return HSP_EINVAL;
    if (a.prologue == HSP_PRO_ACT1D) return HSP_EINVAL;
  } else if (a.rows == HSP_ROWS_SHUFFLE) {
    if (a.up <= 0 || a.up > 16 || a.M < a.Cout * a.up || a.M - a.Cout * a.up > 3 || a.M > (1 << 16)) return HSP_EINVAL;
  } else if (a.rows != HSP_ROWS_PLAIN) {
    return HSP_EINVAL;
  }
  return 0;
}

int dispatch(const hsp_conv1d_args& a, hipStream_t s, int32_t* plan_out) {
  const bool gated = a.rows == HSP_ROWS_GATE_WN || a.rows == HSP_ROWS_GATE_GLU;
  const bool act = a.prologue == HSP_PRO_ACT1D;
  const bool short_seq = (int64_t)((a.M + 127) / 128) * ((a.ncols + 127) / 128) * a.B <= 128;
  if (a.res && a.res_ts > 1) {
    const int e = hsp_rgemm_try(a, s, plan_out);
    return e >= 0 ? e : HSP_EINVAL;
  }
  if (a.K == 1 && !a.w_bs && !HSP_DBG(a, 128)) {
    const int e = hsp_bgemm_try(a, s, plan_out);
    if (e >= 0) return e;
  }
  if ((short_seq || a.ln_c1 || a.split_row || HSP_DBG(a, 1 << 24)) && !a.w_bs && !HSP_DBG(a, 128)) {
    const int e = hsp_rgemm_try(a, s, plan_out);
    if (e >= 0) return e;
  }
  if (a.ln_c1 || a.split_row) return HSP_EINVAL;
  int epi = select_epilogue(a);
  if (act && epi != HSP_EPI_INIT) epi = HSP_EPI_GEN;
  if ((a.K - 1) * a.dil + 3 > 64)
    return gated ? hsp_conv_tile_S64GW(a, epi, act, s, plan_out) : hsp_conv_tile_S64W(a, epi, act, s, plan_out);
#ifdef HSP_TUNING
  if (!gated && a.debug & 256) return hsp_conv_tile_M128(a, epi, act, s, plan_out);
  if (!gated && a.debug & 1024) return hsp_conv_tile_M64(a, epi, act, s, plan_out);
  if (!gated && a.debug & 4096) return hsp_conv_tile_S64(a, epi, act, s, plan_out);
  if (!gated && a.debug & 8192) return hsp_conv_tile_M64P(a, epi, act, s, plan_out);
#endif
  if (short_seq) {
    if (gated) {
      const int64_t t128 = (int64_t)((a.M + 63) / 64) * ((a.ncols + 127) / 128) * a.B;
      if ((t128 <= 48 || (HSP_DBG(a, 1 << 28) && t128 <= 512)) && !HSP_DBG(a, 1 << 27)) {
        const int e = hsp_conv_tile_S64G2(a, epi, act, s, plan_out);
        if (e != HSP_EINVAL) return e;
      }
      return hsp_conv_tile_S64G(a, epi, act, s, plan_out);
    }
    if (a.M > 32) return hsp_conv_tile_S64(a, epi, act, s, plan_out);
    return hsp_conv_tile_S32(a, epi, act, s, plan_out);
  }
  if (gated) return hsp_conv_tile_M128(a, epi, act, s, plan_out);
  if (a.M > 64) return hsp_conv_tile_M128(a, epi, act, s, plan_out);
  if (a.M > 32) return act ? hsp_conv_tile_M64(a, epi, act, s, plan_out) : hsp_conv_tile_M64P(a, epi, act, s, plan_out);
  return act ? hsp_conv_tile_M32(a, epi, act, s, plan_out) : hsp_conv_tile_M32P(a, epi, act, s, plan_out);
}

}

extern "C" int hsp_conv1d_mfma_f32(const hsp_conv1d_args* a, void* stream) {
  if (!a) return HSP_EINVAL;
  if (int e = validate(*a)) return e;
  return dispatch(*a, static_cast<hipStream_t>(stream), nullptr);
}

extern "C" int hsp_conv1d_mfma_plan(const hsp_conv1d_args* a, int32_t out4[4]) {
  if (!a || !out4) return HSP_EINVAL;
  if (int e = validate(*a)) return e;
  return dispatch(*a, nullptr, out4);
}
```

megatts2_hierspeechpp_amd/csrc/hsp_conv1d_mfma_kernel.h:

```cpp
#pragma once
#include <atomic>
#include <type_traits>
#include "hsp_device.h"

typedef float f32x16 __attribute__((ext_vector_type(16)));

#ifdef HSP_TUNING
#define HSP_DBG(a, bit) (((a).debug & (bit)) != 0)
#else
#define HSP_DBG(a, bit) false
#endif

enum {
  HSP_EPI_INIT = 0,
  HSP_EPI_VEC = 1,
  HSP_EPI_GATE = 2,
  HSP_EPI_SHUF = 3,
  HSP_EPI_GEN = 4
};

namespace hspconv {

template <int WM, int WN, int TM, int TN, int NPW_, int MINW_, int XSLACK_ = 64, int KS_ = 1>
struct Cfg {
  static constexpr int kKS = KS_;
  static constexpr int NCW = WM * WN * KS_;
  static constexpr int kWM = WM, kWN = WN, kTM = TM, kTN = TN;
  static constexpr int BM = WM * TM * 32;
  static constexpr int BN = WN * TN * 32;
  static constexpr int NPW = NPW_;
  static constexpr int NPT = NPW_ * 64;
  static constexpr int THREADS = 64 * (WM * WN * KS_ + NPW_);
  static constexpr int MINW = MINW_;
  static constexpr int XWP = BN + XSLACK_;
};

struct LdsPlan {
  int kc, lkc;
  int rpw;
  int xw;
  int xwp;
  int xrw;
  int xrwp;
  int a2w;
  int ws_sz, xa_sz, scr_sz;
  int xa_off, scr_off, total;
};

template <class C>
__host__ __device__ inline LdsPlan make_plan(int K, int dil, int prologue, int lkc) {
  LdsPlan p;
  p.lkc = lkc;
  p.kc = 1 << lkc;
  p.rpw = (p.kc + C::NPW - 1) / C::NPW;
  p.xw = C::BN + (K - 1) * dil;
  p.xwp = C::XWP;
  p.xrw = p.xw + 10;
  p.xrwp = (p.xrw + 63) & ~63;
  p.a2w = 2 * p.xw + 10;
  p.ws_sz = K * p.kc * C::BM;
  p.xa_sz = p.kc * p.xwp;
  p.scr_sz = prologue == HSP_PRO_ACT1D ? 2 * p.rpw * p.xrwp + ((p.a2w + 3) & ~3) : 0;
  p.xa_off = 2 * p.ws_sz;
  p.scr_off = p.xa_off + 2 * p.xa_sz;
  p.total = p.scr_off + C::NPW * p.scr_sz;
  return p;
}

template <int N, class F>
__device__ __forceinline__ void static_for(F&& f) {
  if constexpr (N > 0) {
    static_for<N - 1>(f);
    f(std::integral_constant<int, N - 1>{});
  }
}

__device__ __forceinline__ void lds_barrier() {
  asm volatile("s_waitcnt lgkmcnt(0)" ::: "memory");
  __builtin_amdgcn_s_barrier();
  asm volatile("" ::: "memory");
}

#define HSP_BARRIER(a) do { if (!HSP_DBG(a, 2048)) lds_barrier(); } while (0)

__device__ __forceinline__ unsigned lds_addr(const float* p) {
  return (unsigned)(size_t)(const __attribute__((address_space(3))) float*)p;
}

template <int N, int I = 0>
__device__ __forceinline__ void ds_read_frags(float (&f)[N], unsigned addr) {
  if constexpr (I < N) {
    asm volatile("ds_read_b32 %0, %1 offset:%2" : "=v"(f[I]) : "v"(addr), "n"(I * 128));
    ds_read_frags<N, I + 1>(f, addr);
  }
}

template <int N, int OFF, int I = 0>
__device__ __forceinline__ void ds_read_frags_at(float (&f)[N], unsigned addr) {
  if constexpr (I < N) {
    static_assert(OFF + I * 128 < 65536, "ds_read immediate offsets are 16 bits");
    asm volatile("ds_read_b32 %0, %1 offset:%2" : "=v"(f[I]) : "v"(addr), "n"(OFF + I * 128));
    ds_read_frags_at<N, OFF, I + 1>(f, addr);
  }
}

template <int N, int I = 0>
__device__ __forceinline__ void bind_frags(float (&f)[N]) {
  if constexpr (I < N) {
    asm volatile("" : "+v"(f[I]));
    bind_frags<N, I + 1>(f);
  }
}
template <int NA, int NB>
__device__ __forceinline__ void wait_frags(float (&fa)[NA], float (&fb)[NB]) {
  asm volatile("s_waitcnt lgkmcnt(0)" ::: "memory");
  bind_frags<NA>(fa);
  bind_frags<NB>(fb);
}

__device__ __forceinline__ void wave_lds_fence() { asm volatile("s_waitcnt lgkmcnt(0)" ::: "memory"); }

struct ProdArgs {
  const float* w;
  const float* zeros;
  const float* alpha_exp;
  const float* beta_inv;
  const float* filt;
  int K, Cin, Lin, M, w_ld, x_cs, x_ts, prologue;
  float slope;
};

#define HSP_GPTR(p) ((const __attribute__((address_space(1))) void*)(p))
#define HSP_LPTR(p) ((__attribute__((address_space(3))) void*)(p))
__device__ __forceinline__ void dma16(const float* g, float* l) {
  __builtin_amdgcn_global_load_lds(HSP_GPTR(g), HSP_LPTR(l), 16, 0, 0);
}
__device__ __forceinline__ void dma4(const float* g, float* l) {
  __builtin_amdgcn_global_load_lds(HSP_GPTR(g), HSP_LPTR(l), 4, 0, 0);
}
__device__ __forceinline__ void wait_vm0() { asm volatile("s_waitcnt vmcnt(0)" ::: "memory"); }

template <class C>
struct Prod {
  static constexpr int CPR = C::BM / 4;
  static constexpr int RPI = (64 / CPR) > 0 ? (64 / CPR) : 1;

  static __device__ __forceinline__ void dma_w(const ProdArgs& a, const LdsPlan& P, float* Ws, int c0, int m0, int pw,
                                               int lane) {
    const int r_in = lane / CPR, col = (lane % CPR) * 4;
    const int lipj = P.lkc - __builtin_ctz(RPI);
    const int ninstr = a.K << lipj;
    const bool colok = m0 + col < a.M;
    const float* wcol = a.w + m0 + col;
    for (int q = pw; q < ninstr; q += C::NPW) {
      const int j = q >> lipj, g = q & ((1 << lipj) - 1);
      const int ci = c0 + g * RPI + r_in;
      const float* src = (colok && ci < a.Cin) ? wcol + (j * a.Cin + ci) * a.w_ld : a.zeros;
      dma16(src, Ws + ((j << P.lkc) + g * RPI) * C::BM);
    }
  }

  static __device__ __forceinline__ void dma_x(const ProdArgs& a, const LdsPlan& P, float* Xa, const float* xb, int c0,
                                               int p0, int pw, int lane) {
    const int npr = P.xwp >> 6;
    for (int kc = pw; kc < P.kc; kc += C::NPW) {
      const int ci = c0 + kc;
      const float* xc = xb + ci * a.x_cs;
      for (int i = 0; i < npr; ++i) {
        const int p = p0 + lane + 64 * i;
        const float* src = (ci < a.Cin && p >= 0 && p < a.Lin) ? xc + p * a.x_ts : a.zeros;
        dma4(src, Xa + kc * P.xwp + 64 * i);
      }
    }
  }
  static __device__ __forceinline__ void dma_x16(const ProdArgs& a, const LdsPlan& P, float* Xa, const float* xb,
                                                 int c0, int p0a, int pw, int lane) {
    const int ngrp = (P.xw + 3 + 3) >> 2;
    for (int kc = pw; kc < P.kc; kc += C::NPW) {
      const int ci = c0 + kc;
      const float* xc = xb + ci * a.x_cs;
      for (int g0 = 0; g0 < ngrp; g0 += 64) {
        const int g = g0 + lane, p = p0a + 4 * g;
        if (g < ngrp) {
          const float* src = (ci < a.Cin && p >= 0 && p < a.Lin) ? xc + p : a.zeros;
          dma16(src, Xa + kc * P.xwp + 4 * g0);
        }
      }
    }
  }
  static __device__ __forceinline__ void dma_w_fast(const float* wtile, int w_ld, int Cin, int K, const LdsPlan& P,
                                                    float* Ws, int c0, int pw, unsigned wofs) {
    const int lipj = P.lkc - __builtin_ctz(RPI);
    const int ninstr = K << lipj;
    for (int q = pw; q < ninstr; q += C::NPW) {
      const int j = q >> lipj, g = q & ((1 << lipj) - 1);
      const char* base = reinterpret_cast<const char*>(wtile + (size_t)(j * Cin + c0 + g * RPI) * (size_t)w_ld);
      dma16(reinterpret_cast<const float*>(base + wofs), Ws + ((j << P.lkc) + g * RPI) * C::BM);
    }
  }
  static __device__ __forceinline__ void dma_x16_fast(const float* xtile, int x_cs, int Lin, const LdsPlan& P, float* Xa,
                                                      int c0, int p0a, int pw, int lane) {
    const int ngrp = (P.xw + 3 + 3) >> 2;
    for (int g0 = 0; g0 < ngrp; g0 += 64) {
      const int g = g0 + lane, p = p0a + 4 * g;
      if (g < ngrp && p >= 0 && p < Lin) {
        const unsigned xofs = 16u * (unsigned)lane;
        for (int kc = pw; kc < P.kc; kc += C::NPW) {
          const char* base = reinterpret_cast<const char*>(xtile + (size_t)(c0 + kc) * (size_t)x_cs + 4 * g0);
          dma16(reinterpret_cast<const float*>(base + xofs), Xa + kc * P.xwp + 4 * g0);
        }
      }
    }
  }
  static __device__ __forceinline__ void zero_x_rows(const LdsPlan& P, float* Xa0, int pw, int lane) {
    for (int bsel = 0; bsel < 2; ++bsel)
      for (int kc = pw; kc < P.kc; kc += C::NPW)
        for (int s = lane; s < P.xwp; s += 64) Xa0[bsel * P.xa_sz + kc * P.xwp + s] = 0.0f;
    wave_lds_fence();
  }
  static __device__ __forceinline__ void lrelu_x(const ProdArgs& a, const LdsPlan& P, float* Xa, int pw, int lane) {
    for (int kc = pw; kc < P.kc; kc += C::NPW)
      for (int s = lane; s < P.xwp; s += 64) {
        const float v = Xa[kc * P.xwp + s];
        Xa[kc * P.xwp + s] = v > 0.0f ? v : v * a.slope;
      }
  }

  static __device__ __forceinline__ void dma_raw(const ProdArgs& a, const LdsPlan& P, float* rawbuf, const float* xb,
                                                 int c0, int p0, int pw, int lane) {
    const int npr = P.xrwp >> 6;
    for (int rs = 0; rs < P.rpw; ++rs) {
      const int ci = c0 + pw + rs * C::NPW;
      const float* xc = xb + ci * a.x_cs;
      for (int i = 0; i < npr; ++i) {
        const float* src = ci < a.Cin ? xc + hsp_clampi(p0 - 5 + lane + 64 * i, 0, a.Lin - 1) : a.zeros;
        dma4(src, rawbuf + rs * P.xrwp + 64 * i);
      }
    }
  }

  typedef float f32x2 __attribute__((ext_vector_type(2)));
  static __device__ __forceinline__ void act_row(const ProdArgs& a, const LdsPlan& P, const float* raw, float* a2,
                                                 float* xa, int ci, int p0, int lane) {
    const int L = a.Lin;
    const int mlo = 2 * p0 - 5;
    const bool interior = mlo >= 0 && mlo + P.a2w <= 2 * L;
    const float* hu = a.filt;
    const float* hd = a.filt + 12;
    const int cic = ci < a.Cin ? ci : a.Cin - 1;
    const float kf = a.alpha_exp[cic] * 0.318309886183790672f, kb = 0.5f * a.beta_inv[cic];
    if (interior) {
      const int npair = (P.a2w - 1) >> 1;
      for (int i = lane; i < npair; i += 64) {
        float xv[7];
#pragma unroll
        for (int t = 0; t < 7; ++t) xv[t] = raw[i + t];
        f32x2 u = {0.0f, 0.0f};
#pragma unroll
        for (int t = 0; t < 6; ++t) {
          const f32x2 xx = {xv[t], xv[t + 1]};
          const f32x2 hh = {hu[11 - 2 * t], hu[10 - 2 * t]};
          u = __builtin_elementwise_fma(xx, hh, u);
        }
        u = u * 2.0f;
        a2[2 * i + 1] = hsp_snake_hw(u.x, kf, kb);
        a2[2 * i + 2] = hsp_snake_hw(u.y, kf, kb);
      }
      if (lane < 2) {
        const float* xr_ = lane ? raw + P.xw + 4 : raw;
        float uu = 0.0f;
#pragma unroll
        for (int t = 0; t < 6; ++t) uu = fmaf(xr_[t], lane ? hu[11 - 2 * t] : hu[10 - 2 * t], uu);
        a2[lane ? P.a2w - 1 : 0] = hsp_snake_hw(2.0f * uu, kf, kb);
      }
    } else {
      for (int s = lane; s < P.a2w; s += 64) {
        const int m = hsp_clampi(mlo + s, 0, 2 * L - 1);
        const int q = m >> 1, odd = m & 1;
        const float* xr_ = raw + (q - 3 + odd) - (p0 - 5);
        float u = 0.0f;
#pragma unroll
        for (int t = 0; t < 6; ++t) u = fmaf(xr_[t], odd ? hu[10 - 2 * t] : hu[11 - 2 * t], u);
        a2[s] = hsp_snake_hw(2.0f * u, kf, kb);
      }
    }
    wave_lds_fence();
    for (int s = lane; s < P.xwp; s += 64) {
      const int p = p0 + s;
      f32x2 v = {0.0f, 0.0f};
      if (p >= 0 && p < L && s < P.xw) {
        const f32x2* ar = reinterpret_cast<const f32x2*>(a2 + 2 * s);
#pragma unroll
        for (int k = 0; k < 6; ++k) {
          const f32x2 hh = {hd[2 * k], hd[2 * k + 1]};
          v = __builtin_elementwise_fma(ar[k], hh, v);
        }
      }
      xa[s] = v.x + v.y;
    }
    wave_lds_fence();
  }

  static __device__ __forceinline__ void act_rows(const ProdArgs& a, const LdsPlan& P, const float* rawbuf, float* a2,
                                                  float* Xa, int c0, int p0, int pw, int lane) {
    for (int rs = 0; rs < P.rpw; ++rs) {
      const int row = pw + rs * C::NPW;
      if (row < P.kc) act_row(a, P, rawbuf + rs * P.xrwp, a2, Xa + row * P.xwp, c0 + row, p0, lane);
    }
  }
};


template <class C, int EPI, bool ACT, int TM, int TN>
__device__ __forceinline__ void conv_consume(const hsp_conv1d_args& a, const LdsPlan& P, float* const lds, const int b,
                                             const int m0, const int t0, const int p0, const int wm, const int wn,
                                             const int lane, const int nchunks, const int lkc, const int xvec,
                                             const int ks = 0) {
  constexpr int BM = C::BM;
  const int KC = P.kc;
  __builtin_assume(nchunks > 0);
  const int wave = wm * C::kWN + wn;
  const int l32 = lane & 31, half = lane >> 5;
  const int mw = m0 + wm * (TM * 32);
  const int tw = t0 + wn * (TN * 32) + l32;
  f32x16 acc[TM][TN];

  static_assert(C::kKS == 1 || EPI != HSP_EPI_INIT, "a K split with the accumulator-init epilogue would add the residual once per group");
  if constexpr (EPI == HSP_EPI_INIT) {
    const int rcs = (int)a.res_cs, ycs = (int)a.y_cs;
    const int lrow = mw + 4 * half;
    int tcl[TN];
#pragma unroll
    for (int n = 0; n < TN; ++n) tcl[n] = min(tw + n * 32, a.ncols - 1);
    auto init = [&](auto full_tag) __attribute__((always_inline)) {
      constexpr bool FULL = decltype(full_tag)::value;
      auto vec1 = [&](const float* p, int c) __attribute__((always_inline)) -> float {
        if constexpr (FULL) return (p + c)[lrow];
        else return p[min(lrow + c, a.Cout - 1)];
      };
      auto mat = [&](const float* p, int c, int cs, int n) __attribute__((always_inline)) -> float {
        if constexpr (FULL) return (p + c * cs)[lrow * cs + tcl[n]];
        else return p[min(lrow + c, a.Cout - 1) * cs + tcl[n]];
      };
      float add[TM][16];
      if (a.bias) {
        static_for<TM>([&](auto ii) __attribute__((always_inline)) {
          constexpr int i = decltype(ii)::value;
          static_for<16>([&](auto rr) __attribute__((always_inline)) {
            constexpr int r = decltype(rr)::value;
            add[i][r] = vec1(a.bias, i * 32 + HSP_ACC_ROW(r, 0));
          });
        });
      } else {
#pragma unroll
        for (int i = 0; i < TM; ++i)
#pragma unroll
          for (int r = 0; r < 16; ++r) add[i][r] = 0.0f;
      }
      if (a.res) {
        const float* const rb = a.res + (int64_t)b * a.res_bs;
        static_for<TM>([&](auto ii) __attribute__((always_inline)) {
          constexpr int i = decltype(ii)::value;
          static_for<16>([&](auto rr) __attribute__((always_inline)) {
            constexpr int r = decltype(rr)::value;
            static_for<TN>([&](auto nn) __attribute__((always_inline)) {
              constexpr int n = decltype(nn)::value;
              acc[i][n][r] = mat(rb, i * 32 + HSP_ACC_ROW(r, 0), rcs, n);
            });
          });
        });
      } else {
#pragma unroll
        for (int i = 0; i < TM; ++i)
#pragma unroll
          for (int n = 0; n < TN; ++n)
#pragma unroll
            for (int r = 0; r < 16; ++r) acc[i][n][r] = 0.0f;
      }
      static_for<TM>([&](auto ii) __attribute__((always_inline)) {
        constexpr int i = decltype(ii)::value;
        static_for<TN>([&](auto nn) __attribute__((always_inline)) {
          constexpr int n = decltype(nn)::value;
          static_for<16>([&](auto rr) __attribute__((always_inline)) {
            constexpr int r = decltype(rr)::value;
            acc[i][n][r] += add[i][r];
          });
        });
      });
      if (a.cbias) {
        const float* const cb = a.cbias + (int64_t)b * a.cbias_bs;
        static_for<TM>([&](auto ii) __attribute__((always_inline)) {
          constexpr int i = decltype(ii)::value;
          static_for<16>([&](auto rr) __attribute__((always_inline)) {
            constexpr int r = decltype(rr)::value;
            const float c = vec1(cb, i * 32 + HSP_ACC_ROW(r, 0));
            static_for<TN>([&](auto nn) __attribute__((always_inline)) {
              constexpr int n = decltype(nn)::value;
              acc[i][n][r] += c;
            });
          });
        });
      }
      if (a.accumulate) {
        const float* const yb = a.y + (int64_t)b * a.y_bs;
        static_for<TM>([&](auto ii) __attribute__((always_inline)) {
          constexpr int i = decltype(ii)::value;
          static_for<TN>([&](auto nn) __attribute__((always_inline)) {
            constexpr int n = decltype(nn)::value;
            float tmp[16];
            static_for<16>([&](auto rr) __attribute__((always_inline)) {
              constexpr int r = decltype(rr)::value;
              tmp[r] = mat(yb, i * 32 + HSP_ACC_ROW(r, 0), ycs, n);
            });
            __builtin_amdgcn_sched_barrier(0);
            static_for<16>([&](auto rr) __attribute__((always_inline)) {
              constexpr int r = decltype(rr)::value;
              acc[i][n][r] += tmp[r];
            });
            __builtin_amdgcn_sched_barrier(0);
          });
        });
      }
    };
    if (mw + TM * 32 <= a.Cout) {
      init(std::true_type{});
    } else if (mw < a.Cout) {
      init(std::false_type{});
    } else {
#pragma unroll
      for (int i = 0; i < TM; ++i)
#pragma unroll
        for (int n = 0; n < TN; ++n)
#pragma unroll
          for (int r = 0; r < 16; ++r) acc[i][n][r] = 0.0f;
    }
  } else {
#pragma unroll
    for (int i = 0; i < TM; ++i)
#pragma unroll
      for (int j = 0; j < TN; ++j)
#pragma unroll
        for (int r = 0; r < 16; ++r) acc[i][j][r] = 0.0f;
  }

  const int wlane = half * BM + wm * (TM * 32) + l32;
  const int xlane = half * P.xwp + wn * (TN * 32) + l32 + (xvec ? (p0 & 3) : 0);
  const int nsteps = ((a.K * KC) >> 1) / C::kKS;

  HSP_BARRIER(a);
  {
    constexpr int kStepA = 2 * BM * 4;
    constexpr int rowB = 2 * C::XWP * 4;
    const int spanB = (KC >> 1) * rowB;
    const int tapB = 4 * a.dil;
    float fa0[TM], fb0[TN], fa1[TM], fb1[TN];
    auto mma_set = [&](const float (&fa)[TM], const float (&fb)[TN]) __attribute__((always_inline)) {
#pragma unroll
      for (int i = 0; i < TM; ++i)
#pragma unroll
        for (int n = 0; n < TN; ++n)
          acc[i][n] = __builtin_amdgcn_mfma_f32_32x32x2f32(fa[i], fb[n], acc[i][n], 0, 0, 0);
    };
    unsigned aA = lds_addr(lds + wlane);
    unsigned aB = lds_addr(lds + P.xa_off + xlane);
    int offA0 = 0, pairB0 = 0, tapoff0 = 0;
    if constexpr (C::kKS > 1) {
      const int s0 = ks * nsteps;
      offA0 = s0 * kStepA;
      pairB0 = (s0 & ((KC >> 1) - 1)) * rowB;
      tapoff0 = (s0 >> (lkc - 1)) * tapB;
    }
    unsigned va = aA + (unsigned)offA0, vb = aB + (unsigned)(pairB0 + tapoff0);
    const bool run = !HSP_DBG(a, 2);
    if (run) {
      ds_read_frags<TM>(fa0, va);
      ds_read_frags<TN>(fb0, vb);
    }
    for (int c = 0; c < nchunks; ++c) {
      if (!run) {
        HSP_BARRIER(a);
        continue;
      }
      int offA = offA0, pairB = pairB0, tapoff = tapoff0;
      int offB = 0;
      auto advance = [&]() __attribute__((always_inline)) {
        int t;
        asm volatile(
            "s_add_i32 %[oa], %[oa], %[sa]\n\t"
            "s_add_i32 %[pb], %[pb], %[sb]\n\t"
            "s_cmp_eq_u32 %[pb], %[span]\n\t"
            "s_cselect_b32 %[pb], 0, %[pb]\n\t"
            "s_cselect_b32 %[t], %[tap], 0\n\t"
            "s_add_i32 %[to], %[to], %[t]"
            : [oa] "+s"(offA), [pb] "+s"(pairB), [to] "+s"(tapoff), [t] "=&s"(t)
            : [sa] "n"(2 * kStepA), [sb] "n"(2 * rowB), [span] "s"(spanB), [tap] "s"(tapB)
            : "scc");
        offB = pairB + tapoff;
      };
      auto slot_a = [&](bool walk) __attribute__((always_inline)) {
        wait_frags(fa0, fb0);
        __builtin_amdgcn_sched_barrier(0);
        if (walk) advance();
        ds_read_frags_at<TM, kStepA>(fa1, va);
        ds_read_frags_at<TN, rowB>(fb1, vb);
        __builtin_amdgcn_sched_barrier(0);
        mma_set(fa0, fb0);
        __builtin_amdgcn_sched_barrier(0);
      };
      for (int s = 0; s + 2 < nsteps; s += 2) {
        slot_a(true);
        wait_frags(fa1, fb1);
        __builtin_amdgcn_sched_barrier(0);
        va = aA + (unsigned)offA;
        vb = aB + (unsigned)offB;
        ds_read_frags<TM>(fa0, va);
        ds_read_frags<TN>(fb0, vb);
        __builtin_amdgcn_sched_barrier(0);
        mma_set(fa1, fb1);
        __builtin_amdgcn_sched_barrier(0);
      }
      slot_a(false);
      HSP_BARRIER(a);
      bind_frags<TM>(fa1);
      bind_frags<TN>(fb1);
      if (c + 1 < nchunks) {
        const int nb = (c + 1) & 1;
        aA = lds_addr(lds + nb * P.ws_sz + wlane);
        aB = lds_addr(lds + P.xa_off + nb * P.xa_sz + xlane);
        va = aA + (unsigned)offA0;
        vb = aB + (unsigned)(pairB0 + tapoff0);
        __builtin_amdgcn_sched_barrier(0);
        ds_read_frags<TM>(fa0, va);
        ds_read_frags<TN>(fb0, vb);
      }
      __builtin_amdgcn_sched_barrier(0);
      mma_set(fa1, fb1);
      __builtin_amdgcn_sched_barrier(0);
    }
  }

  if constexpr (C::kKS > 1) {
    static_assert(C::kKS == 2, "one partner group per wave");
    float* const red = lds + C::kWM * C::kWN * (32 * 36) + (wm * C::kWN + wn) * (TM * TN * 16 * 64) + lane;
    if (ks > 0) {
      static_for<TM>([&](auto ii) __attribute__((always_inline)) {
        constexpr int i = decltype(ii)::value;
        static_for<TN>([&](auto nn) __attribute__((always_inline)) {
          constexpr int n = decltype(nn)::value;
          static_for<16>([&](auto rr) __attribute__((always_inline)) {
            constexpr int r = decltype(rr)::value;
            red[((i * TN + n) * 16 + r) * 64] = acc[i][n][r];
          });
        });
      });
    }
    lds_barrier();
    if (ks > 0) return;
    static_for<TM>([&](auto ii) __attribute__((always_inline)) {
      constexpr int i = decltype(ii)::value;
      static_for<TN>([&](auto nn) __attribute__((always_inline)) {
        constexpr int n = decltype(nn)::value;
        static_for<16>([&](auto rr) __attribute__((always_inline)) {
          constexpr int r = decltype(rr)::value;
          acc[i][n][r] += red[((i * TN + n) * 16 + r) * 64];
        });
      });
    });
  }

  if (HSP_DBG(a, 16)) return;
  if constexpr (EPI == HSP_EPI_INIT) {
    float* const yb = a.y + (int64_t)b * a.y_bs;
    const int ycs = (int)a.y_cs;
    const bool full = mw + TM * 32 <= a.Cout && t0 + wn * (TN * 32) + TN * 32 <= a.ncols;
    const float ps = a.post_scale;
    if (full) {
      const int lrow = mw + 4 * half;
      int voff[TN];
#pragma unroll
      for (int n = 0; n < TN; ++n) voff[n] = lrow * ycs + tw + n * 32;
      static_for<TM>([&](auto ii) __attribute__((always_inline)) {
        constexpr int i = decltype(ii)::value;
        static_for<16>([&](auto rr) __attribute__((always_inline)) {
          constexpr int r = decltype(rr)::value;
          float* const yp = yb + (i * 32 + HSP_ACC_ROW(r, 0)) * ycs;
          static_for<TN>([&](auto nn) __attribute__((always_inline)) {
            constexpr int n = decltype(nn)::value;
            if (HSP_DBG(a, 65536)) __builtin_nontemporal_store(acc[i][n][r] * ps, yp + voff[n]);
            else yp[voff[n]] = acc[i][n][r] * ps;
          });
        });
      });
    } else {
      static_for<TM>([&](auto ii) __attribute__((always_inline)) {
        constexpr int i = decltype(ii)::value;
        static_for<TN>([&](auto nn) __attribute__((always_inline)) {
          constexpr int n = decltype(nn)::value;
          const int t = tw + n * 32;
          static_for<16>([&](auto rr) __attribute__((always_inline)) {
            constexpr int r = decltype(rr)::value;
            const int row = mw + i * 32 + HSP_ACC_ROW(r, half);
            if (row < a.Cout && t < a.ncols) yb[row * ycs + t] = acc[i][n][r] * ps;
          });
        });
      });
    }
  } else if constexpr (EPI == HSP_EPI_VEC) {
    constexpr int ESTR = 36;
    float* const stage = lds + wave * (32 * ESTR);
    const int er = lane >> 3, ec = (lane & 7) * 4;
    const float4 z4 = make_float4(0.f, 0.f, 0.f, 0.f);
    static_for<TM>([&](auto ii) __attribute__((always_inline)) {
      constexpr int i = decltype(ii)::value;
      float add[4], cs[4];
#pragma unroll
      for (int q = 0; q < 4; ++q) {
        const int co = mw + i * 32 + er + 8 * q;
        add[q] = 0.0f;
        cs[q] = a.scale;
        if (co < a.Cout) {
          if (a.bias) add[q] = a.bias[co];
          if (a.cbias) add[q] += a.cbias[(int64_t)b * a.cbias_bs + co];
          if (a.cscale) cs[q] *= a.cscale[(int64_t)b * a.cscale_bs + co];
        }
      }
      static_for<TN>([&](auto nn) __attribute__((always_inline)) {
        constexpr int n = decltype(nn)::value;
        const int t = t0 + wn * (TN * 32) + n * 32 + ec;
        const bool tok = t < a.ncols;
        float4 rs[4], yo[4];
#pragma unroll
        for (int q = 0; q < 4; ++q) {
          const int co = mw + i * 32 + er + 8 * q;
          const bool ok = tok && co < a.Cout;
          rs[q] = z4;
          yo[q] = z4;
          if (ok && a.res) rs[q] = *reinterpret_cast<const float4*>(a.res + (int64_t)b * a.res_bs + (int64_t)co * a.res_cs + t);
          if (ok && a.accumulate) yo[q] = *reinterpret_cast<const float4*>(a.y + (int64_t)b * a.y_bs + (int64_t)co * a.y_cs + t);
        }
        float4 mk = make_float4(1.f, 1.f, 1.f, 1.f);
        if (a.mask_mode != HSP_MASK_NONE && tok) mk = *reinterpret_cast<const float4*>(a.mask + (int64_t)b * a.mask_bs + t);
        static_for<16>([&](auto rr) __attribute__((always_inline)) {
          constexpr int r = decltype(rr)::value;
          stage[HSP_ACC_ROW(r, half) * ESTR + l32] = acc[i][n][r];
        });
        wave_lds_fence();
#pragma unroll
        for (int q = 0; q < 4; ++q) {
          const int co = mw + i * 32 + er + 8 * q;
          if (tok && co < a.Cout) {
            const float4 v = *reinterpret_cast<const float4*>(stage + (er + 8 * q) * ESTR + ec);
            float e[4] = {v.x, v.y, v.z, v.w};
            const float r4[4] = {rs[q].x, rs[q].y, rs[q].z, rs[q].w};
            const float y4[4] = {yo[q].x, yo[q].y, yo[q].z, yo[q].w};
            const float m4[4] = {mk.x, mk.y, mk.z, mk.w};
#pragma unroll
            for (int u = 0; u < 4; ++u) {
              float x = hsp_apply_act(e[u] + add[q], a.act);
              if (a.mask_mode & HSP_MASK_PRE) x *= m4[u];
              x = fmaf(x, cs[q], r4[u]);
              if (a.mask_mode & HSP_MASK_POST) x *= m4[u];
              e[u] = (x + y4[u]) * a.post_scale;
            }
            *reinterpret_cast<float4*>(a.y + (int64_t)b * a.y_bs + (int64_t)co * a.y_cs + t) =
                make_float4(e[0], e[1], e[2], e[3]);
          }
        }
        wave_lds_fence();
      });
    });
  } else if constexpr (EPI == HSP_EPI_GATE) {
    static_assert(TM % 2 == 0, "gated rows need both halves of a channel in one wave");
    const int H = a.gate_half;
    static_for<TM / 2>([&](auto ih) __attribute__((always_inline)) {
      constexpr int i = 2 * decltype(ih)::value;
      const int mpair = mw + i * 32;
      static_for<TN>([&](auto nn) __attribute__((always_inline)) {
        constexpr int n = decltype(nn)::value;
        const int t = tw + n * 32;
        if (mpair < a.M && t < a.ncols) {
          static_for<16>([&](auto rr) __attribute__((always_inline)) {
            constexpr int r = decltype(rr)::value;
            const int co = (mpair >> 6) * 32 + HSP_ACC_ROW(r, half);
            if (co < H) {
              float va = acc[i][n][r], vb = acc[i + 1][n][r];
              if (a.bias) { va += a.bias[co]; vb += a.bias[H + co]; }
              if (a.cbias) {
                va += a.cbias[(int64_t)b * a.cbias_bs + co];
                vb += a.cbias[(int64_t)b * a.cbias_bs + H + co];
              }
              const float v = (a.rows == HSP_ROWS_GATE_WN ? hsp_tanh(va) : va) * hsp_sigmoid(vb);
              hsp_epilogue_store(a, b, co, t, v);
            }
          });
        }
      });
    });
  } else if constexpr (EPI == HSP_EPI_SHUF) {
    if ((a.up == 4 || a.up == 2) && !HSP_DBG(a, 262144)) {
      typedef float st4 __attribute__((ext_vector_type(4), aligned(4)));
      typedef float st2 __attribute__((ext_vector_type(2), aligned(4)));
      const float sc = a.scale * a.post_scale;
      const int upl = a.up == 4 ? 2 : 1;
      static_for<TM>([&](auto ii) __attribute__((always_inline)) {
        constexpr int i = decltype(ii)::value;
        float* yrow[4][2];
        float bz[4][2];
        bool rok[4][2];
#pragma unroll
        for (int q = 0; q < 4; ++q)
#pragma unroll
          for (int c2 = 0; c2 < 2; ++c2) {
            const int m = mw + i * 32 + 8 * q + 4 * half + 2 * c2;
            const int co = m >> upl;
            rok[q][c2] = m < a.M && co < a.Cout;
            yrow[q][c2] = a.y + (int64_t)b * a.y_bs + (int64_t)(rok[q][c2] ? co : 0) * a.y_cs;
            bz[q][c2] = (rok[q][c2] && a.bias) ? a.bias[co] : 0.0f;
          }
        static_for<TN>([&](auto nn) __attribute__((always_inline)) {
          constexpr int n = decltype(nn)::value;
          const int t = tw + n * 32;
          if (t < a.ncols) {
            const int to0 = a.up * t - a.shuf_pad;
            const bool inside = to0 >= 0 && to0 + a.up <= a.Lout;
            static_for<4>([&](auto qq) __attribute__((always_inline)) {
              constexpr int q = decltype(qq)::value;
              if (a.up == 4) {
                if (rok[q][0]) {
                  const st4 v = {(acc[i][n][4 * q] + bz[q][0]) * sc, (acc[i][n][4 * q + 1] + bz[q][0]) * sc,
                                 (acc[i][n][4 * q + 2] + bz[q][0]) * sc, (acc[i][n][4 * q + 3] + bz[q][0]) * sc};
                  if (inside) *reinterpret_cast<st4*>(yrow[q][0] + to0) = v;
                  else {
#pragma unroll
                    for (int ph = 0; ph < 4; ++ph)
                      if (to0 + ph >= 0 && to0 + ph < a.Lout) yrow[q][0][to0 + ph] = v[ph];
                  }
                }
              } else {
#pragma unroll
                for (int c2 = 0; c2 < 2; ++c2) {
                  if (rok[q][c2]) {
                    const st2 v = {(acc[i][n][4 * q + 2 * c2] + bz[q][c2]) * sc, (acc[i][n][4 * q + 2 * c2 + 1] + bz[q][c2]) * sc};
                    if (inside) *reinterpret_cast<st2*>(yrow[q][c2] + to0) = v;
                    else {
#pragma unroll
                      for (int ph = 0; ph < 2; ++ph)
                        if (to0 + ph >= 0 && to0 + ph < a.Lout) yrow[q][c2][to0 + ph] = v[ph];
                    }
                  }
                }
              }
            });
          }
        });
      });
      return;
    }
    const float up_inv = 1.0f / (float)a.up;
    static_for<TM>([&](auto ii) __attribute__((always_inline)) {
      constexpr int i = decltype(ii)::value;
      float* yrow[16];
      float bz[16];
      int toff[16];
#pragma unroll
      for (int r = 0; r < 16; ++r) {
        const int m = mw + i * 32 + HSP_ACC_ROW(r, half);
        const int co = (int)(((float)m + 0.5f) * up_inv);
        const bool ok = m < a.M && co < a.Cout;
        toff[r] = ok ? (m - co * a.up) - a.shuf_pad : -(1 << 30);
        yrow[r] = a.y + (int64_t)b * a.y_bs + (int64_t)(ok ? co : 0) * a.y_cs;
        bz[r] = (ok && a.bias) ? a.bias[co] : 0.0f;
      }
      static_for<TN>([&](auto nn) __attribute__((always_inline)) {
        constexpr int n = decltype(nn)::value;
        const int t = tw + n * 32;
        if (t < a.ncols) {
          static_for<16>([&](auto rr) __attribute__((always_inline)) {
            constexpr int r = decltype(rr)::value;
            const int to = a.up * t + toff[r];
            if (to >= 0 && to < a.Lout) yrow[r][to] = (acc[i][n][r] + bz[r]) * a.scale * a.post_scale;
          });
        }
      });
    });
  } else {
    const float up_inv = a.rows == HSP_ROWS_SHUFFLE ? 1.0f / (float)a.up : 1.0f;
    static_for<TM>([&](auto ii) __attribute__((always_inline)) {
      constexpr int i = decltype(ii)::value;
      static_for<TN>([&](auto nn) __attribute__((always_inline)) {
        constexpr int n = decltype(nn)::value;
        const int t = tw + n * 32;
        if (t < a.ncols) {
          static_for<16>([&](auto rr) __attribute__((always_inline)) {
            constexpr int r = decltype(rr)::value;
            const int m = mw + i * 32 + HSP_ACC_ROW(r, half);
            int co = m, to = t;
            bool ok = m < a.M;
            if (a.rows == HSP_ROWS_SHUFFLE) {
              co = (int)(((float)m + 0.5f) * up_inv);
              to = a.up * t + (m - co * a.up) - a.shuf_pad;
              ok = ok && to >= 0 && to < a.Lout;
            }
            ok = ok && co < a.Cout;
            if (ok) {
              float v = acc[i][n][r];
              if (a.bias) v += a.bias[co];
              if (a.cbias) v += a.cbias[(int64_t)b * a.cbias_bs + co];
              v = hsp_apply_act(v, a.act);
              hsp_epilogue_store(a, b, co, to, v);
            }
          });
        }
      });
    });
  }
}

template <class C, int EPI, bool ACT>
constexpr bool has_tail_path() {
  return EPI == HSP_EPI_INIT && !ACT && C::kWM * C::kWN == 4 && C::kTM * C::kWM == 4 && C::kTN * C::kWN == 4;
}

template <class C, int EPI, bool ACT>
__global__ __launch_bounds__(C::THREADS, C::MINW) void conv1d_mfma_kernel(const hsp_conv1d_args a, const int n_mt,
                                                                          const int n_nt, const int lkc,
                                                                          const int xvec, const int sched) {
  extern __shared__ __attribute__((aligned(16))) float lds[];
  constexpr int BM = C::BM, BN = C::BN, TM = C::kTM, TN = C::kTN;
  const LdsPlan P = make_plan<C>(a.K, a.dil, ACT ? HSP_PRO_ACT1D : HSP_PRO_NONE, lkc);
  const int KC = P.kc;

  int mt, ct;
  {
    const int g = sched & 255;
    const int bid = blockIdx.x;
    if (g == 0) {
      mt = bid % n_mt;
      ct = bid / n_mt;
    } else {
      const int x = bid & 7, q = bid >> 3;
      const int groups_m = n_mt / g, nx = 8 / groups_m;
      mt = (x % groups_m) * g + q % g;
      ct = (q / g) * nx + x / groups_m;
      if (ct >= n_nt * a.B) return;
    }
  }
  int nt, b;
  bool tail_tile = false;
  if (sched >> 8) {
    const int n_main = (n_nt - 1) * a.B;
    if (ct < n_main) {
      nt = ct % (n_nt - 1);
      b = ct / (n_nt - 1);
    } else {
      nt = n_nt - 1;
      b = ct - n_main;
      tail_tile = true;
    }
  } else {
    nt = ct % n_nt;
    b = ct / n_nt;
  }
  const int m0 = mt * BM, t0 = nt * BN;
  const int p0 = t0 - a.pad;

  const int wave = __builtin_amdgcn_readfirstlane(threadIdx.x >> 6);
  const int lane = threadIdx.x & 63;
  const int nchunks = (a.Cin + KC - 1) >> lkc;

  if (wave >= C::NCW) {
    const int pw = wave - C::NCW;
    const float* const wb = a.w + (int64_t)b * a.w_bs;
    const ProdArgs pa{wb, a.zeros, a.alpha_exp, a.beta_inv, a.filt, a.K, a.Cin, a.Lin, a.M, a.w_ld, (int)a.x_cs,
                      (int)a.x_ts, a.prologue, a.slope};
    const float* xb = a.x + (int64_t)b * a.x_bs;
    using PR = Prod<C>;
    float* const Ws0 = lds;
    float* const Xa0 = lds + P.xa_off;
    if constexpr (!ACT) {
      const int p0a = p0 & ~3;
      const bool fast = xvec && m0 + BM <= a.M && (a.Cin & (KC - 1)) == 0 && !HSP_DBG(a, 512);
      if (fast) {
        const float* const wtile = wb + m0;
        const float* const xtile = xb + p0a;
        const int xcs = (int)a.x_cs;
        const unsigned wofs = 4u * (unsigned)((lane / PR::CPR) * a.w_ld + (lane % PR::CPR) * 4);
        if (p0a < 0 || p0a + 4 * ((P.xw + 3 + 3) >> 2) > a.Lin) PR::zero_x_rows(P, Xa0, pw, lane);
        PR::dma_w_fast(wtile, a.w_ld, a.Cin, a.K, P, Ws0, 0, pw, wofs);
        PR::dma_x16_fast(xtile, xcs, a.Lin, P, Xa0, 0, p0a, pw, lane);
        wait_vm0();
        if (a.prologue == HSP_PRO_LRELU) PR::lrelu_x(pa, P, Xa0, pw, lane);
        HSP_BARRIER(a);
        for (int c = 0; c < nchunks; ++c) {
          const int nb = (c + 1) & 1;
          if (c + 1 < nchunks && !HSP_DBG(a, 1)) {
            PR::dma_w_fast(wtile, a.w_ld, a.Cin, a.K, P, Ws0 + nb * P.ws_sz, (c + 1) << lkc, pw, wofs);
            PR::dma_x16_fast(xtile, xcs, a.Lin, P, Xa0 + nb * P.xa_sz, (c + 1) << lkc, p0a, pw, lane);
            wait_vm0();
            if (a.prologue == HSP_PRO_LRELU) PR::lrelu_x(pa, P, Xa0 + nb * P.xa_sz, pw, lane);
          }
          HSP_BARRIER(a);
        }
        return;
      }
      PR::dma_w(pa, P, Ws0, 0, m0, pw, lane);
      if (xvec) PR::dma_x16(pa, P, Xa0, xb, 0, p0a, pw, lane); else PR::dma_x(pa, P, Xa0, xb, 0, p0, pw, lane);
      wait_vm0();
      if (a.prologue == HSP_PRO_LRELU) PR::lrelu_x(pa, P, Xa0, pw, lane);
      HSP_BARRIER(a);
      for (int c = 0; c < nchunks; ++c) {
        const int nb = (c + 1) & 1;
        if (c + 1 < nchunks && !HSP_DBG(a, 1)) {
          PR::dma_w(pa, P, Ws0 + nb * P.ws_sz, (c + 1) << lkc, m0, pw, lane);
          if (xvec) PR::dma_x16(pa, P, Xa0 + nb * P.xa_sz, xb, (c + 1) << lkc, p0a, pw, lane);
          else PR::dma_x(pa, P, Xa0 + nb * P.xa_sz, xb, (c + 1) << lkc, p0, pw, lane);
          wait_vm0();
          if (a.prologue == HSP_PRO_LRELU) PR::lrelu_x(pa, P, Xa0 + nb * P.xa_sz, pw, lane);
        }
        HSP_BARRIER(a);
      }
    } else {
      float* const scr = lds + P.scr_off + pw * P.scr_sz;
      float* const a2 = scr + 2 * P.rpw * P.xrwp;
      const int rsz = P.rpw * P.xrwp;
      PR::dma_raw(pa, P, scr, xb, 0, p0, pw, lane);
      PR::dma_w(pa, P, Ws0, 0, m0, pw, lane);
      wait_vm0();
      PR::act_rows(pa, P, scr, a2, Xa0, 0, p0, pw, lane);
      if (nchunks > 1) PR::dma_raw(pa, P, scr + rsz, xb, KC, p0, pw, lane);
      wait_vm0();
      HSP_BARRIER(a);
      for (int c = 0; c < nchunks; ++c) {
        const int nb = (c + 1) & 1;
        if (c + 1 < nchunks && !HSP_DBG(a, 1)) {
          PR::dma_w(pa, P, Ws0 + nb * P.ws_sz, (c + 1) << lkc, m0, pw, lane);
          if (c + 2 < nchunks) PR::dma_raw(pa, P, scr + (c & 1) * rsz, xb, (c + 2) << lkc, p0, pw, lane);
          PR::act_rows(pa, P, scr + nb * rsz, a2, Xa0 + nb * P.xa_sz, (c + 1) << lkc, p0, pw, lane);
          wait_vm0();
        }
        HSP_BARRIER(a);
      }
    }
    return;
  }

  if constexpr (has_tail_path<C, EPI, ACT>()) {
    if (tail_tile) {
      conv_consume<C, EPI, ACT, 1, 1>(a, P, lds, b, m0, t0, p0, wave, 0, lane, nchunks, lkc, xvec);
      return;
    }
  }
  if constexpr (C::kKS > 1) {
    const int ks = wave / (C::kWM * C::kWN), w2 = wave % (C::kWM * C::kWN);
    conv_consume<C, EPI, ACT, TM, TN>(a, P, lds, b, m0, t0, p0, w2 / C::kWN, w2 % C::kWN, lane, nchunks, lkc, xvec, ks);
  } else {
    conv_consume<C, EPI, ACT, TM, TN>(a, P, lds, b, m0, t0, p0, wave / C::kWN, wave % C::kWN, lane, nchunks, lkc, xvec);
  }
}

constexpr int kMaxLdsBytes = 160 * 1024;
constexpr int kLdsTarget = 80 * 1024;

template <class C>
int pick_lkc(const hsp_conv1d_args& a, int lds_limit) {
  const bool act = a.prologue == HSP_PRO_ACT1D;
  if (C::BN + (a.K - 1) * a.dil + 3 > C::XWP) return -1;
  int cin_p2 = 2;
  while ((1 << cin_p2) < a.Cin && cin_p2 < 6) ++cin_p2;
  for (int lkc = cin_p2; lkc >= 2; --lkc) {
    const LdsPlan P = make_plan<C>(a.K, a.dil, a.prologue, lkc);
    if (P.total * (int)sizeof(float) > lds_limit) continue;
    if (P.kc < Prod<C>::RPI) continue;
    if (C::kKS > 1 && (((a.K * P.kc) >> 1) % (2 * C::kKS) != 0 || P.total < C::kWM * C::kWN * (32 * 36 + C::kTM * C::kTN * 16 * 64))) continue;
    if (act && P.rpw > 2) continue;
    return lkc;
  }
  return -1;
}

template <class C, int EPI, bool ACT>
int launch_one(const hsp_conv1d_args& a, hipStream_t s, int32_t* plan_out) {
  const int64_t tiles = (int64_t)((a.M + C::BM - 1) / C::BM) * ((a.ncols + C::BN - 1) / C::BN) * a.B;
  const bool deep_k3 = HSP_DBG(a, 1 << 29) && a.K <= 3;
  const bool two_per_cu = !deep_k3 && (C::MINW * 256 >= 2 * C::THREADS || ((tiles > 256 || HSP_DBG(a, 1 << 26)) && tiles <= 512 && !HSP_DBG(a, 1 << 21)));
  int lkc = pick_lkc<C>(a, two_per_cu ? kLdsTarget : kMaxLdsBytes);
  if (lkc < 0) lkc = pick_lkc<C>(a, kMaxLdsBytes);
  if (lkc < 0) return HSP_EINVAL;
  int lds_bytes = make_plan<C>(a.K, a.dil, a.prologue, lkc).total * (int)sizeof(float);
  if (plan_out) {
    plan_out[0] = C::BM; plan_out[1] = C::BN; plan_out[2] = 1 << lkc; plan_out[3] = lds_bytes;
    return 0;
  }
  const int n_mt = (a.M + C::BM - 1) / C::BM;
  const int n_nt = (a.ncols + C::BN - 1) / C::BN;
  const int64_t n_ct = (int64_t)n_nt * a.B;
  int g = 0;
  if (HSP_DBG(a, 16384) && n_mt >= 1 && n_mt <= 8 && (8 % n_mt) == 0) {
    const int64_t slab = (int64_t)a.K * a.Cin * C::BM * (int64_t)sizeof(float);
    g = 1;
    for (int cand = n_mt; cand > 1; cand >>= 1)
      if (n_mt % cand == 0 && (int64_t)cand * slab <= (int64_t)3200 * 1024) { g = cand; break; }
  }
  const int rem = a.ncols - (n_nt - 1) * C::BN;
  const int tail = (has_tail_path<C, EPI, ACT>() && n_nt >= 2 && rem <= 32 && !HSP_DBG(a, 32768)) ? 1 : 0;
  int64_t blocks = (int64_t)n_mt * n_ct;
  if (g > 0) {
    const int nx = 8 / (n_mt / g);
    blocks = 8 * (int64_t)g * ((n_ct + nx - 1) / nx);
  }
  if (blocks <= 0 || blocks > 0x7fffffff) return HSP_EINVAL;
  const int sched = g | (tail << 8);
  auto kern = conv1d_mfma_kernel<C, EPI, ACT>;
  static hsp_lds_flags flags;
  if (lds_bytes > 32 * 1024)
    if (int e = hsp_raise_lds_limit(reinterpret_cast<const void*>(kern), kMaxLdsBytes, flags)) return e;
  if (EPI == HSP_EPI_VEC && lds_bytes < C::NCW * 32 * 36 * 4) lds_bytes = C::NCW * 32 * 36 * 4;
  auto al16 = [](const void* p) { return (reinterpret_cast<uintptr_t>(p) & 15) == 0; };
  const bool xvec = !ACT && a.x_ts == 1 && (a.Lin & 3) == 0 && (a.x_cs & 3) == 0 && (a.x_bs & 3) == 0 && al16(a.x) &&
                    !HSP_DBG(a, 64);
  hipLaunchKernelGGL(kern, dim3((unsigned)blocks), dim3(C::THREADS), lds_bytes, s, a, n_mt, n_nt, lkc, xvec ? 1 : 0, sched);
  return (int)hipGetLastError();
}

inline int select_epilogue(const hsp_conv1d_args& a) {
  if (a.rows == HSP_ROWS_GATE_WN || a.rows == HSP_ROWS_GATE_GLU) return HSP_EPI_GATE;
  const bool pointwise = a.act != HSP_ACT_NONE || a.mask_mode != HSP_MASK_NONE || a.cscale;
  if (a.rows == HSP_ROWS_SHUFFLE)
    return (!pointwise && !a.cbias && !a.res && !a.accumulate) ? HSP_EPI_SHUF : HSP_EPI_GEN;
  if (!pointwise && a.scale == 1.0f && !HSP_DBG(a, 32)) return HSP_EPI_INIT;
  auto al16 = [](const void* p) { return (reinterpret_cast<uintptr_t>(p) & 15) == 0; };
  const bool vec = (a.ncols & 3) == 0 && al16(a.y) && (a.y_bs & 3) == 0 && (a.y_cs & 3) == 0 &&
                   (!a.res || (al16(a.res) && (a.res_bs & 3) == 0 && (a.res_cs & 3) == 0)) &&
                   (a.mask_mode == HSP_MASK_NONE || (al16(a.mask) && (a.mask_bs & 3) == 0));
  return vec ? HSP_EPI_VEC : HSP_EPI_GEN;
}

using M128 = Cfg<2, 2, 2, 2, 4, 4>;
using M64 = Cfg<1, 4, 2, 2, 8, 3>;
using M32 = Cfg<1, 4, 1, 4, 8, 3>;
using M64P = Cfg<1, 4, 2, 2, 4, 4>;
using M32P = Cfg<1, 4, 1, 4, 4, 4>;
using S64 = Cfg<2, 2, 1, 1, 4, 2>;
using S64G = Cfg<1, 4, 2, 1, 4, 2>;
using S32 = Cfg<1, 4, 1, 1, 4, 2>;
using S64W = Cfg<2, 2, 1, 1, 4, 2, 128>;
using S64GW = Cfg<1, 4, 2, 1, 4, 2, 128>;
using S64G2 = Cfg<1, 2, 2, 1, 4, 2, 64, 2>;

}

#define HSP_TILE_LIST(X) X(M128) X(M64) X(M32) X(M64P) X(M32P) X(S64) X(S64G) X(S32) X(S64W) X(S64GW) X(S64G2)
#define HSP_TILE_DECL(name) \
  int hsp_conv_tile_##name(const hsp_conv1d_args& a, int epi, bool act, hipStream_t s, int32_t* plan_out);
HSP_TILE_LIST(HSP_TILE_DECL)
#undef HSP_TILE_DECL
```

megatts2_hierspeechpp_amd/hip_layers.py:

```python
from __future__ import annotations

import contextvars
import ctypes as C
import os
from typing import Dict, List, Optional, Tuple

import numpy as np
import torch
from torch import nn

from . import _lib as L
from . import functional as Fh
from .synth import kaiser_sinc_filter12


LAUNCH_HOOK = None
DEBUG_FLAGS = 0


_ZEROS = {}


def _zeros(device) -> torch.Tensor:
    z = _ZEROS.get(device)
    if z is None:
        z = _ZEROS[device] = torch.zeros(64, dtype=torch.float32, device=device)
    return z


_DFT = {}


def _dft_tables(device):
    t = _DFT.get(device)
    if t is None:
        n = 4160
        f = np.zeros(n, dtype=np.float32)
        finv = np.zeros(n, dtype=np.float32)
        L.check(L.lib().hsp_dftseg_tables_f32(f.ctypes.data, finv.ctypes.data), "hsp_dftseg_tables_f32")
        t = _DFT[device] = (torch.from_numpy(f).to(device), torch.from_numpy(finv).to(device))
    return t


_TW = {}


def _wspec_twiddles(device):
    t = _TW.get(device)
    if t is None:
        ang = 2.0 * np.pi * np.arange(128, dtype=np.float64) / 128.0
        t = _TW[device] = torch.from_numpy(np.concatenate([np.cos(ang), np.sin(ang)])).to(device)
    return t


FFT_PRODUCT = os.environ.get("HSP_FFT_PRODUCT", "three")


class RowLengths:

    def __init__(self, frames: torch.Tensor, T: int):
        if frames.dtype != torch.int64 or frames.dim() != 1:
            raise L.HspError(f"row lengths must be int64 [B], got {frames.dtype} {tuple(frames.shape)}")
        self.frames, self.T = frames.contiguous(), int(T)
        self._lens: Dict[int, torch.Tensor] = {}
        self._masks: Dict[int, torch.Tensor] = {}

    def factor(self, L_: int) -> int:
        if L_ % self.T != 0:
            raise L.HspError(f"row_exact: a tensor of {L_} columns is not a whole multiple of the {self.T} frames")
        return L_ // self.T

    def at(self, L_: int) -> torch.Tensor:
        t = self._lens.get(L_)
        if t is None:
            f = self.factor(L_)
            t = self._lens[L_] = self.frames if f == 1 else self.frames * f
        return t

    def mask(self, L_: int) -> torch.Tensor:
        m = self._masks.get(L_)
        if m is None:
            m = self._masks[L_] = Fh.sequence_mask(self.at(L_), L_)
        return m

    def prepare(self, L_: int):
        self.at(L_)
        self.mask(L_)


_ROWS: "contextvars.ContextVar[Optional[RowLengths]]" = contextvars.ContextVar("hsp_row_lengths", default=None)


class row_exact:

    def __init__(self, rows: Optional[RowLengths]):
        self.rows = rows

    def __enter__(self):
        self._token = _ROWS.set(self.rows)
        return self.rows

    def __exit__(self, *exc):
        _ROWS.reset(self._token)
        return False


def row_lengths() -> Optional[RowLengths]:
    return _ROWS.get()


def fft_act_fusable(x) -> bool:
    return (x.stride(2) == 1 and x.shape[2] % 4 == 0 and x.stride(0) % 4 == 0 and x.stride(1) % 4 == 0
            and x.data_ptr() % 16 == 0)


SURVEY_ABI = os.environ.get("HSP_SURVEY_ABI", "0") == "1"
_DEFER: "contextvars.ContextVar[Optional[list]]" = contextvars.ContextVar("hsp_deferred", default=None)


class deferred:

    def __enter__(self):
        assert _DEFER.get() is None, "deferred() does not nest"
        structs = []
        self._token = _DEFER.set(structs)
        return structs

    def __exit__(self, *exc):
        _DEFER.reset(self._token)
        return False


def _bracket(kind: str, call, flops: int, nbytes: int, arg, soft: bool = False, span=None):
    hook = LAUNCH_HOOK
    if call is None:
        if hook is not None and span[0] is not None:
            hook(kind, flops, nbytes, span[0], span[1], arg)
        return 0, span[0], span[1]
    e0 = e1 = None
    if hook is not None:
        e0, e1 = (torch.cuda.Event(enable_timing=True) for _ in range(2))
        e0.record()
    rc = call()
    if soft and rc == L.EINVAL:
        return rc, None, None
    L.check(rc, kind)
    if hook is not None:
        e1.record()
        hook(kind, flops, nbytes, e0, e1, arg)
    return 0, e0, e1


def launch_group(kind: str, fn, structs, *extra):
    flops = sum(e[1] for e in structs if e is not None)
    nbytes = sum(e[2] for e in structs if e is not None)
    ptrs = [C.byref(e[0]) if e is not None else None for e in structs]
    _bracket(kind, lambda: fn(*ptrs, *extra, L.stream_ptr()), flops, nbytes, structs[0][0])


def _launch(kind: str, fn, a, flops: int, nbytes: int, soft: bool = False, keep=()):
    a.debug = DEBUG_FLAGS
    structs = _DEFER.get()
    if structs is not None:
        if soft or a.ln_c1 or a.split_row:
            raise L.HspError("deferred(): no soft / fused-LayerNorm / split launches")
        structs.append((a, flops, nbytes, keep))
        return 0
    if SURVEY_ABI:
        fn = L.lib().hsp_convtr1d_f32 if a.rows == L.ROWS_SHUFFLE else L.lib().hsp_conv1d_f32
    return _bracket(kind, lambda: fn(C.byref(a), L.stream_ptr()), flops, nbytes, a, soft=soft)[0]


def _round_up(x: int, m: int) -> int:
    return (x + m - 1) // m * m


def plain_rows(cout: int) -> np.ndarray:
    m = _round_up(cout, 4)
    rows = np.full(m, -1, np.int64)
    rows[:cout] = np.arange(cout)
    return rows


def gated_rows(half: int) -> np.ndarray:
    assert half % 32 == 0, "gated convs need a half-width that is a multiple of 32"
    m = np.arange(2 * half)
    return ((m >> 5) & 1) * half + (m >> 6) * 32 + (m & 31)


def conv_pack_map(cout: int, cin: int, k: int, rows: np.ndarray) -> np.ndarray:
    M = rows.shape[0]
    j = np.arange(k)[:, None, None]
    ci = np.arange(cin)[None, :, None]
    co = rows[None, None, :]
    idx = (co * cin + ci) * k + j
    idx = np.where(co >= 0, idx, -1)
    return np.ascontiguousarray(np.broadcast_to(idx, (k, cin, M))).astype(np.int32).reshape(-1)


def convtr_pack_map(cin: int, cout: int, k: int, up: int) -> Tuple[np.ndarray, int, int]:
    kp = -(-k // up)
    M = _round_up(cout * up, 4)
    m = np.arange(M)
    co, r = m // up, m % up
    jp = np.arange(kp)[:, None, None]
    ci = np.arange(cin)[None, :, None]
    tap = r[None, None, :] + (kp - 1 - jp) * up
    idx = (ci * cout + co[None, None, :]) * k + tap
    ok = (tap < k) & (co[None, None, :] < cout)
    return np.where(ok, idx, -1).astype(np.int32).reshape(-1), kp, M


class WeightArena:

    ALIGN = 64

    def __init__(self):
        self.specs: List[Tuple[object, str, int]] = []
        self.buffer: Optional[torch.Tensor] = None
        self.views: Dict[Tuple[int, str], torch.Tensor] = {}
        self._offsets: List[int] = []
        self.total = 0

    def request(self, owner, name: str, numel: int):
        self._offsets.append(self.total)
        self.specs.append((owner, name, numel))
        self.total += _round_up(numel, self.ALIGN)

    def allocate(self, device):
        self.buffer = torch.zeros(max(self.total, 1), dtype=torch.float32, device=device)
        for (owner, name, numel), off in zip(self.specs, self._offsets):
            self.views[(id(owner), name)] = self.buffer[off:off + numel]

    def view(self, owner, name: str) -> torch.Tensor:
        return self.views[(id(owner), name)]


_EPOCH = 0


def _bump_epoch():
    global _EPOCH
    _EPOCH += 1


class HipLayer(nn.Module):

    _hsp_stale = True

    def hsp_requests(self) -> List[Tuple[str, int]]:
        return []

    def hsp_fill(self, arena: WeightArena, materialize: bool) -> None:
        pass

    def _apply(self, fn, *args, **kw):
        before = [(q.device, q.data_ptr()) for q in self._parameters.values() if q is not None]
        r = super()._apply(fn, *args, **kw)
        after = [(q.device, q.data_ptr()) for q in self._parameters.values() if q is not None]
        if before != after:
            self.__dict__["_hsp_stale"] = True
            _bump_epoch()
        return r

    def _load_from_state_dict(self, *args, **kw):
        r = super()._load_from_state_dict(*args, **kw)
        self.__dict__["_hsp_stale"] = True
        _bump_epoch()
        return r


def ensure_ready(model: nn.Module) -> None:
    if model.__dict__.get("_hsp_epoch") == _EPOCH:
        return
    if any(m._hsp_stale for m in model.modules() if isinstance(m, HipLayer)):
        p = next(model.parameters(), None)
        dev = p.device if p is not None else torch.device("cpu")
        if dev.type != "cuda":
            raise L.HspError(f"{type(model).__name__}: parameters are on {dev}; move the model to a ROCm device "
                             "(.cuda() / .to(device)) -- the product path has no CPU fallback")
        fin = getattr(model, "finalize", None)
        if fin is not None:
            fin(dev)
        else:
            finalize(model, dev)
    model.__dict__["_hsp_epoch"] = _EPOCH


def entry(fn):
    import functools

    @functools.wraps(fn)
    def wrapped(self, *args, **kw):
        ensure_ready(self)
        return fn(self, *args, **kw)
    return wrapped


def _gather(src: torch.Tensor, idx_map: np.ndarray, dst: torch.Tensor):
    assert dst.is_contiguous() and src.is_contiguous(), "hsp_gather_f32 reads and writes flat buffers"
    assert idx_map.dtype == np.int32 and idx_map.size == dst.numel() and idx_map.flags["C_CONTIGUOUS"]
    mp = torch.from_numpy(idx_map).to(src.device)
    L.check(L.lib().hsp_gather_f32(L.fptr(src), L.ptr(mp), L.fptr(dst), dst.numel(), L.stream_ptr()), "hsp_gather_f32")
    torch.cuda.current_stream().synchronize()


def _fold(v: torch.Tensor, g: torch.Tensor) -> torch.Tensor:
    rows = v.shape[0]
    cols = v.numel() // rows
    w = torch.empty(v.shape, dtype=v.dtype, device=v.device)
    vc, gc = v.contiguous(), g.contiguous()
    assert gc.numel() == rows
    L.check(L.lib().hsp_fold_weight_norm_f32(L.fptr(vc), L.fptr(gc), L.fptr(w), rows, cols, L.stream_ptr()),
            "hsp_fold_weight_norm_f32")
    return w


def _spectrum(Cc: int, Np: int, device) -> torch.Tensor:
    return torch.empty(64, 2 * Cc, Np, dtype=torch.float32, device=device)


class _ConvBase(HipLayer):
    def __init__(self, weight_shape, rows0: int, bias: bool, weight_norm: bool):
        super().__init__()
        if weight_norm:
            self.weight_g = nn.Parameter(torch.ones(rows0, 1, 1), requires_grad=False)
            self.weight_v = nn.Parameter(torch.zeros(*weight_shape), requires_grad=False)
        else:
            self.weight = nn.Parameter(torch.zeros(*weight_shape), requires_grad=False)
        self.bias = nn.Parameter(torch.zeros(bias), requires_grad=False) if bias else None
        self.has_bias = bool(bias)
        self.wn = weight_norm
        self._w: Optional[torch.Tensor] = None
        self._b: Optional[torch.Tensor] = None
        self._wf: Optional[torch.Tensor] = None

    def _folded(self) -> torch.Tensor:
        if self.wn:
            return _fold(self.weight_v.data, self.weight_g.data)
        return self.weight.data.contiguous()

    def _bias_src(self) -> torch.Tensor:
        return self.bias.data

    def _require_ready(self):
        if self._w is None:
            raise L.HspError(f"{type(self).__name__} used before finalize(): call model.finalize(device) after "
                             "loading weights")


class Conv1d(_ConvBase):

    def __init__(self, cin, cout, k, stride=1, padding=0, dilation=1, bias=True, weight_norm=False,
                 rows=L.ROWS_PLAIN, weight_2d=False):
        super().__init__((cout, cin) if weight_2d else (cout, cin, k), cout, cout if bias else 0, weight_norm)
        self.cin, self.cout, self.k, self.stride, self.padding, self.dilation = cin, cout, k, stride, padding, dilation
        self.rows = rows
        self.trim_right = 0
        if rows in (L.ROWS_GATE_WN, L.ROWS_GATE_GLU):
            self.row_map = gated_rows(cout // 2)
        else:
            self.row_map = plain_rows(cout)
        self.M = int(self.row_map.shape[0])
        self.packed = True
        self._pre_norm, self._c1 = None, None
        self._rowmajor, self._wt = False, None
        self._flip_in = self._flip_out = False
        self._fft, self._wf_form = False, None
        self._fft_ok: Dict[Tuple[int, int], bool] = {}

    def fuse_input_layernorm(self, norm):
        assert self.k == 1 and self.rows == L.ROWS_PLAIN
        self.__dict__["_pre_norm"] = norm

    def _ln_params(self):
        n = self._pre_norm
        g = (n.weight if hasattr(n, "weight") else n.gamma).data
        b = (n.bias if hasattr(n, "weight") else n.beta).data
        return g, b

    def keep_rowmajor_weight(self):
        assert self.k == 1 and self.rows == L.ROWS_PLAIN
        self._rowmajor = True

    def pack_flipped(self, inputs: bool = False, outputs: bool = False):
        assert self.rows == L.ROWS_PLAIN and self._pre_norm is None and not self._rowmajor
        self._flip_in, self._flip_out = bool(inputs), bool(outputs)
        self.__dict__["_hsp_stale"] = True
        _bump_epoch()

    def hsp_requests(self):
        if not self.packed:
            return []
        fused = self._pre_norm is not None
        return [("w", self.k * self.cin * self.M)] + ([("b", self.cout)] if self.has_bias or fused else []) + \
            ([("c1", self.cout)] if fused else []) + \
            ([("wt", self.cout * self.cin)] if self._rowmajor else [])

    def enable_fft(self):
        assert self.stride == 1 and self.rows == L.ROWS_PLAIN and self.cin == self.cout and 2 <= self.k <= 64
        assert self.padding * 2 == (self.k - 1) * self.dilation, "same-length conv"
        self._fft = True

    def fft_form(self) -> str:
        return "three" if FFT_PRODUCT == "three" and self.cin % 64 == 0 else "block"

    def ensure_wf(self):
        if self._wf is not None and self._wf_form == self.fft_form():
            return self._wf
        self._require_ready()
        if torch.cuda.is_current_stream_capturing():
            raise L.HspError("ensure_wf() inside a stream capture: run one eager call first (or prepare_fft(model))")
        Cc, form = self.cin, self.fft_form()
        wf = torch.empty(64 * (3 if form == "three" else 4) * Cc * Cc, dtype=torch.float32, device=self._w.device)
        L.check(L.lib().hsp_dftseg_weight_spectrum_f32(
            L.fptr(self._w), self.k, Cc, self.M, L.ptr(_wspec_twiddles(self._w.device)), L.fptr(wf),
            L.WSPEC_THREE if form == "three" else L.WSPEC_BLOCK, L.stream_ptr()), "hsp_dftseg_weight_spectrum_f32")
        self._wf, self._wf_form = wf, form
        return wf

    def hsp_fill(self, arena, materialize):
        if not self.packed:
            return
        fused = self._pre_norm is not None
        self._w = arena.view(self, "w")
        self._b = arena.view(self, "b") if self.has_bias or fused else None
        self._c1 = arena.view(self, "c1") if fused else None
        self._wt = arena.view(self, "wt").view(self.cout, self.cin) if self._rowmajor else None
        self._wf = None
        if materialize:
            w = self._folded()
            if self._flip_in:
                w = w.flip(1).contiguous()
            if self._flip_out:
                w = w.flip(0).contiguous()
            if self._wt is not None:
                assert not fused
                self._wt.copy_(w.reshape(self.cout, self.cin))
            if fused:
                g, beta = self._ln_params()
                w2 = w.reshape(self.cout, self.cin).double()
                wg = w2 * g.double()[None, :]
                self._c1.copy_(wg.sum(1).float())
                c2 = w2 @ beta.double()
                if self.has_bias:
                    c2 = c2 + self._bias_src().double()
                self._b.copy_(c2.float())
                w = wg.float().reshape(w.shape).contiguous()
            _gather(w, conv_pack_map(self.cout, self.cin, self.k, self.row_map), self._w)
            if self._b is not None and not fused:
                self._b.copy_(self._bias_src().flip(0) if self._flip_out else self._bias_src())

    def _fft_args(self, B, Lx):
        d, k = self.dilation, self.k
        hop = 129 - k
        nseg = -(-(-(-Lx // d)) // hop)
        da = L.DftSegArgs()
        da.B, da.C, da.L, da.k, da.dil, da.pad, da.nseg = B, self.cin, Lx, k, d, self.padding, nseg
        da.Np = _round_up(B * d * nseg, 4)
        da.post_scale = 1.0
        da.prod3 = int(self.fft_form() == "three")
        return da

    def fft_supported(self, B, Lx) -> bool:
        if not self._fft:
            return False
        da = self._fft_args(B, Lx)
        da.xf_bs = 2 * self.cin * da.Np
        return bool(L.lib().hsp_dftseg_supported(C.byref(da)))

    @staticmethod
    def _fft_set_act(da, x_like, act1d):
        if act1d._ea is None:
            raise L.HspError("Activation1d used before finalize()")
        da.act_alpha_exp, da.act_beta_inv, da.act_filt = L.fptr(act1d._ea), L.fptr(act1d._binv), L.fptr(act1d._filt)
        rows = _ROWS.get()
        if rows is not None:
            da.act_len = L.ptr(rows.at(x_like.shape[2]))

    def _fft_forward(self, x, act1d=None):
        B, Cc, Lx = x.shape
        assert Cc == self.cin and x.stride(2) == 1 and self._fft
        da = self._fft_args(B, Lx)
        xf = _spectrum(Cc, da.Np, x.device)
        da.x, da.x_bs, da.x_cs = L.fptr(x), x.stride(0), x.stride(1)
        da.xf, da.xf_bs, da.dft = L.fptr(xf), xf.stride(0), L.fptr(_dft_tables(x.device)[0])
        if act1d is not None:
            if not fft_act_fusable(x):
                raise L.HspError("forward_fft(act1d=...) needs 16-B addressable rows")
            self._fft_set_act(da, x, act1d)
        _, e0, _ = _bracket("hsp_dftseg_fwd_f32", lambda: L.lib().hsp_dftseg_fwd_f32(C.byref(da), L.stream_ptr()),
                            2 * 2 * 64 * 64 * B * Cc * da.dil * da.nseg, 4 * (B * Cc * Lx + 128 * Cc * da.Np), None)
        return xf, e0

    def _fft_product(self, xf):
        Cc, Np = self.cin, xf.shape[2]
        wf = self.ensure_wf()
        yf = _spectrum(Cc, Np, xf.device)
        if self._wf_form == "three":
            pa = L.Cprod3Args()
            pa.xf, pa.yf, pa.w, pa.zeros = L.fptr(xf), L.fptr(yf), L.fptr(wf), L.fptr(_zeros(xf.device))
            pa.xf_bs, pa.yf_bs, pa.bins, pa.C, pa.Np, pa.debug = xf.stride(0), yf.stride(0), 64, Cc, Np, DEBUG_FLAGS
            _bracket("hsp_cprod3_f32", lambda: L.lib().hsp_cprod3_f32(C.byref(pa), L.stream_ptr()),
                     2 * 64 * 3 * Cc * Cc * Np, 4 * (64 * 2 * 2 * Cc * Np + 64 * 3 * Cc * Cc), None)
            return yf
        a = L.Conv1dArgs()
        _set_in(a, xf)
        a.w, a.K, a.dil, a.pad, a.stride = L.fptr(wf), 1, 1, 0, 1
        a.M, a.w_ld, a.w_bs = 2 * Cc, 2 * Cc, 4 * Cc * Cc
        _set_out(a, yf, 64, 2 * Cc, Np)
        a.ncols, a.rows, a.scale, a.post_scale = Np, L.ROWS_PLAIN, 1.0, 1.0
        _launch("hsp_conv1d_mfma_f32", L.lib().hsp_conv1d_mfma_f32, a, 2 * 64 * 4 * Cc * Cc * Np,
                4 * (64 * 2 * 2 * Cc * Np + 64 * 4 * Cc * Cc))
        return yf

    def _fft_inverse_args(self, yf, B, Lx):
        da = self._fft_args(B, Lx)
        da.xf, da.xf_bs, da.dft = L.fptr(yf), yf.stride(0), L.fptr(_dft_tables(yf.device)[1])
        da.bias = L.fptr(self._b) if self._b is not None else None
        return da

    def _fft_inverse(self, yf, B, Lx, *, res=None, out=None, accumulate=False, post_scale=1.0, before_inverse=None):
        Cc = self.cin
        if out is None:
            out = torch.empty(B, Cc, Lx, dtype=torch.float32, device=yf.device)
        assert out.shape == (B, Cc, Lx) and out.stride(2) == 1 and (res is None or (res.shape == out.shape and res.stride(2) == 1))
        if before_inverse is not None:
            torch.cuda.current_stream(yf.device).wait_event(before_inverse)
        da = self._fft_inverse_args(yf, B, Lx)
        da.y, da.y_bs, da.y_cs = L.fptr(out), out.stride(0), out.stride(1)
        if res is not None:
            da.res, da.res_bs, da.res_cs = L.fptr(res), res.stride(0), res.stride(1)
        da.accumulate, da.post_scale = int(bool(accumulate)), float(post_scale)
        _, _, e1 = _bracket("hsp_dftseg_inv_f32", lambda: L.lib().hsp_dftseg_inv_f32(C.byref(da), L.stream_ptr()),
                            2 * 2 * 64 * 64 * B * Cc * da.dil * da.nseg,
                            4 * (B * Cc * Lx * (self._fft_nio(res, accumulate) - 1) + 128 * Cc * da.Np), None)
        return out, e1

    @staticmethod
    def _fft_nio(res, accumulate) -> int:
        return 2 + bool(res is not None) + 2 * bool(accumulate)

    def _fft_report(self, x, taps, res, accumulate, e_first, e_last, arg):
        B, Cc, Lx = x.shape
        _bracket("hsp_fftconv", None, 2 * B * Cc * Cc * taps * Lx,
                 4 * B * Cc * Lx * self._fft_nio(res, accumulate) + 4 * taps * Cc * Cc, arg, span=(e_first, e_last))

    def forward_fft(self, x, *, res=None, out=None, accumulate=False, post_scale=1.0, act1d=None, before_inverse=None):
        self._require_ready()
        B, _, Lx = x.shape
        xf, e_first = self._fft_forward(x, act1d)
        yf = self._fft_product(xf)
        out, e_last = self._fft_inverse(yf, B, Lx, res=res, out=out, accumulate=accumulate, post_scale=post_scale,
                                        before_inverse=before_inverse)
        self._fft_report(x, self.k, res, accumulate, e_first, e_last, None)
        return out

    def fft_pair_ok(self, second, x) -> bool:
        if not self._fft or not second._fft or second.cin != self.cin or x.shape[2] % 4:
            return False
        B, _, Lx = x.shape
        ia, fa = self._fft_args(B, Lx), second._fft_args(B, Lx)
        dummy = L.fptr(_zeros(x.device))
        ia.xf = ia.dft = fa.xf = fa.dft = fa.act_alpha_exp = fa.act_beta_inv = fa.act_filt = dummy
        ia.xf_bs, fa.xf_bs = 2 * self.cin * ia.Np, 2 * self.cin * fa.Np
        return bool(L.lib().hsp_dftseg_pair_supported(C.byref(ia), C.byref(fa)))

    def _fft_pair_launch(self, second, yf, B, Lx, act_second, like):
        Cc = self.cin
        ia = self._fft_inverse_args(yf, B, Lx)
        fa = second._fft_args(B, Lx)
        xf2 = _spectrum(Cc, fa.Np, yf.device)
        fa.xf, fa.xf_bs, fa.dft = L.fptr(xf2), xf2.stride(0), L.fptr(_dft_tables(yf.device)[0])
        self._fft_set_act(fa, like, act_second)
        _bracket("hsp_dftseg_pair_f32", lambda: L.lib().hsp_dftseg_pair_f32(C.byref(ia), C.byref(fa), L.stream_ptr()),
                 2 * 2 * 64 * 64 * B * Cc * (ia.dil * ia.nseg + fa.dil * fa.nseg), 4 * 128 * Cc * (ia.Np + fa.Np), None)
        return xf2

    def forward_fft_pair(self, second, x, *, act_first, act_second, res=None, out=None, accumulate=False, post_scale=1.0,
                         before_inverse=None):
        self._require_ready()
        second._require_ready()
        B, _, Lx = x.shape
        xf, e_first = self._fft_forward(x, act_first)
        yf = self._fft_product(xf)
        xf2 = self._fft_pair_launch(second, yf, B, Lx, act_second, x)
        yf2 = second._fft_product(xf2)
        out, e_last = second._fft_inverse(yf2, B, Lx, res=res, out=out, accumulate=accumulate, post_scale=post_scale,
                                          before_inverse=before_inverse)
        self._fft_report(x, self.k + second.k, res, accumulate, e_first, e_last, 2)
        return out

    def forward(self, x, *, act1d=None, lrelu: Optional[float] = None, silu_in=False, act=L.ACT_NONE, cbias=None,
                mask=None, mask_mode=L.MASK_NONE, cscale=None, scale=1.0, res=None, out=None, accumulate=False,
                post_scale=1.0, force_direct=False, row_range=None, split_out=None, mask_mode2=L.MASK_NONE):
        self._require_ready()
        if act1d is not None and _ROWS.get() is not None:
            raise L.HspError("row_exact: the conv-prologue Activation1d (HSP_FUSE_ACT_MAX_C > 0) has no ragged form")
        B, Cin, Lin = x.shape
        assert Cin == self.cin, (Cin, self.cin)
        gated = self.rows in (L.ROWS_GATE_WN, L.ROWS_GATE_GLU)
        cout = self.cout // 2 if gated else self.cout
        r0 = 0
        if row_range is not None:
            r0, r1 = row_range
            assert not gated and r0 % 4 == 0 and 0 <= r0 < r1 <= self.cout
            cout = r1 - r0
        Lout = (Lin + 2 * self.padding - self.dilation * (self.k - 1) - 1) // self.stride + 1 - self.trim_right
        out2 = None
        if split_out is not None:
            split_row, out2, acc2 = split_out
            assert row_range is None and not gated and self.k == 1 and 0 < split_row < self.cout
            cout = split_row
            if out2 is None:
                assert not acc2
                out2 = torch.empty(B, self.cout - split_row, Lout, dtype=torch.float32, device=x.device)
        if out is None:
            out = torch.empty(B, cout, Lout, dtype=torch.float32, device=x.device)
        a = L.Conv1dArgs()
        _set_in(a, x)
        a.w, a.K, a.dil, a.pad, a.stride = L.fptr(self._w) + 4 * r0, self.k, self.dilation, self.padding, self.stride
        a.M = self.M if row_range is None else _round_up(cout, 4)
        a.w_ld = self.M
        _set_out(a, out, B, cout, Lout)
        a.ncols = Lout
        a.rows, a.gate_half = self.rows, (cout if gated else 0)
        a.bias = (L.fptr(self._b) + 4 * r0) if self._b is not None else None
        _set_epilogue(a, act, cbias, mask, mask_mode, cscale, scale, res, accumulate, post_scale, out)
        if act1d is not None:
            a.prologue = L.PRO_ACT1D
            a.alpha_exp, a.beta_inv, a.filt = L.fptr(act1d._ea), L.fptr(act1d._binv), L.fptr(act1d._filt)
        elif lrelu is not None:
            a.prologue, a.slope = L.PRO_LRELU, float(lrelu)
        elif silu_in:
            a.prologue = L.PRO_SILU
        if self._pre_norm is not None:
            a.ln_c1, a.ln_eps = L.fptr(self._c1), float(self._pre_norm.eps)
            assert not force_direct and row_range is None
        direct = _wants_direct(a, force_direct, silu_in)
        if direct and a.res_ts > 1:
            res = Fh.copy_strided(res)
            a.res, a.res_bs, a.res_cs, a.res_ts = L.fptr(res), res.stride(0), res.stride(1), 0
        rows_full = cout * (2 if gated else 1)
        flops = 2 * B * rows_full * Cin * self.k * Lout
        nbytes = 4 * (B * Cin * Lin + B * cout * Lout * (1 + (res is not None) + bool(accumulate))
                      + rows_full * Cin * self.k)
        keep = (x, out, out2, res, cbias, mask, cscale)
        kind, fn = ("hsp_conv1d_direct_f32", L.lib().hsp_conv1d_direct_f32) if direct else \
            ("hsp_conv1d_mfma_f32", L.lib().hsp_conv1d_mfma_f32)
        if split_out is not None:
            a.Cout = self.cout
            a.split_row, a.accumulate2, a.mask_mode2 = split_row, int(bool(acc2)), mask_mode2
            a.y2, a.y2_bs, a.y2_cs = L.fptr(out2), out2.stride(0), out2.stride(1)
            flops = 2 * B * self.cout * Cin * Lout
            nbytes += 4 * B * (self.cout - split_row) * Lout * (1 + bool(acc2))
            rc = _launch("hsp_conv1d_mfma_f32", L.lib().hsp_conv1d_mfma_f32, a, flops, nbytes, soft=True, keep=keep)
            return None if rc else (out, out2)
        if self._pre_norm is not None:
            if _DEFER.get() is None and not _launch(kind, fn, a, flops, nbytes, soft=True, keep=keep):
                return out
            xn = Fh.layernorm_mod(x, float(self._pre_norm.eps))
            _set_in(a, xn)
            a.ln_c1 = None
            keep += (xn,)
        _launch(kind, fn, a, flops, nbytes, keep=keep)
        return out


class ConvTranspose1d(_ConvBase):

    def __init__(self, cin, cout, k, stride, padding=0, bias=True, weight_norm=False):
        super().__init__((cin, cout, k), cin, cout if bias else 0, weight_norm)
        self.cin, self.cout, self.k, self.up, self.padding = cin, cout, k, stride, padding
        self.pack_map, self.kp, self.M = convtr_pack_map(cin, cout, k, stride)

    def hsp_requests(self):
        return [("w", self.kp * self.cin * self.M)] + ([("b", self.cout)] if self.bias is not None else [])

    def hsp_fill(self, arena, materialize):
        self._w = arena.view(self, "w")
        self._b = arena.view(self, "b") if self.bias is not None else None
        if materialize:
            _gather(self._folded(), self.pack_map, self._w)
            if self._b is not None:
                self._b.copy_(self.bias.data)

    def forward(self, x, *, res=None, out=None, lrelu: Optional[float] = None):
        self._require_ready()
        B, Cin, Lin = x.shape
        assert Cin == self.cin
        Lout = (Lin - 1) * self.up - 2 * self.padding + self.k
        if out is None:
            out = torch.empty(B, self.cout, Lout, dtype=torch.float32, device=x.device)
        a = L.Conv1dArgs()
        _set_in(a, x)
        a.w, a.K, a.M, a.dil, a.pad, a.stride = L.fptr(self._w), self.kp, self.M, 1, self.kp - 1, 1
        a.w_ld = self.M
        _set_out(a, out, B, self.cout, Lout)
        a.ncols = (Lout - 1 + self.padding) // self.up + 1
        a.rows, a.up, a.shuf_pad = L.ROWS_SHUFFLE, self.up, self.padding
        a.bias = L.fptr(self._b)
        _set_epilogue(a, L.ACT_NONE, None, None, L.MASK_NONE, None, 1.0, res, False, 1.0, out)
        if lrelu is not None:
            a.prologue, a.slope = L.PRO_LRELU, float(lrelu)
        flops = 2 * B * Cin * self.cout * self.k * Lin
        nbytes = 4 * (B * Cin * Lin + B * self.cout * Lout * (1 + (res is not None)) + Cin * self.cout * self.k)
        _launch("hsp_conv1d_mfma_f32", L.lib().hsp_conv1d_mfma_f32, a, flops, nbytes)
        return out


class _SubArena:

    def __init__(self, arena, owner, prefix):
        self.arena, self.owner, self.prefix = arena, owner, prefix

    def view(self, _layer, name):
        return self.arena.view(self.owner, self.prefix + name)


class PolyphaseConv1d(HipLayer):

    def __init__(self, cin, cout, k, stride, bias=True):
        super().__init__()
        self.cin, self.cout, self.k, self.stride = cin, cout, k, stride
        self.weight = nn.Parameter(torch.zeros(cout, cin, k), requires_grad=False)
        self.bias = nn.Parameter(torch.zeros(cout), requires_grad=False) if bias else None
        ph = [Conv1d(cin, cout, len(range(p, k, stride)), bias=(bias and p == 0)) for p in range(min(stride, k))]
        self.__dict__["_phases"] = ph

    def hsp_requests(self):
        return [(f"p{i}.{n}", numel) for i, ph in enumerate(self._phases) for n, numel in ph.hsp_requests()]

    def hsp_fill(self, arena, materialize):
        for i, ph in enumerate(self._phases):
            if materialize:
                ph.weight.data = self.weight.data[:, :, i::self.stride].contiguous()
                if ph.bias is not None:
                    ph.bias.data = self.bias.data
                ph.to(self.weight.device)
            ph.hsp_fill(_SubArena(arena, self, f"p{i}."), materialize)

    def forward(self, x, **kw):
        B, Cin, Lin = x.shape
        Lout = (Lin - self.k) // self.stride + 1
        out = torch.empty(B, self.cout, Lout, dtype=torch.float32, device=x.device)
        for i, ph in enumerate(self._phases):
            xp = x[:, :, i: i + self.stride * (Lout + ph.k - 1): self.stride]
            ph(xp, out=out, accumulate=i > 0, **(kw if i == len(self._phases) - 1 else {}))
        return out


class GroupedPosConv1d(HipLayer):

    TAPS = 64

    def __init__(self, channels, k, groups):
        super().__init__()
        assert k % 2 == 0 and channels % groups == 0 and k % self.TAPS == 0
        self.channels, self.k, self.groups, self.cg = channels, k, groups, channels // groups
        self.weight_g = nn.Parameter(torch.ones(1, 1, k), requires_grad=False)
        self.weight_v = nn.Parameter(torch.zeros(channels, self.cg, k), requires_grad=False)
        self.bias = nn.Parameter(torch.zeros(channels), requires_grad=False)
        subs = []
        for _ in range(groups):
            for j0 in range(0, k, self.TAPS):
                pad = k // 2 - j0
                c = Conv1d(self.cg, self.cg, self.TAPS, padding=pad, bias=(j0 == 0))
                c.trim_right = 2 * pad - (self.TAPS - 1)
                subs.append(c)
        self.__dict__["_subs"] = subs

    def hsp_requests(self):
        return [(f"s{i}.{n}", numel) for i, c in enumerate(self._subs) for n, numel in c.hsp_requests()]

    def hsp_fill(self, arena, materialize):
        w = None
        nb = self.k // self.TAPS
        if materialize:
            vp = self.weight_v.data.permute(2, 0, 1).contiguous().reshape(self.k, -1)
            w = _fold(vp, self.weight_g.data.reshape(self.k)).reshape(self.k, self.channels, self.cg).permute(1, 2, 0)
        for i, c in enumerate(self._subs):
            gi, bi = divmod(i, nb)
            if materialize:
                c.weight.data = w[gi * self.cg:(gi + 1) * self.cg, :, bi * self.TAPS:(bi + 1) * self.TAPS].contiguous()
                if c.bias is not None:
                    c.bias.data = self.bias.data[gi * self.cg:(gi + 1) * self.cg].contiguous()
            c.hsp_fill(_SubArena(arena, self, f"s{i}."), materialize)

    def forward(self, x):
        nb = self.k // self.TAPS
        conv = torch.empty_like(x)
        for i, c in enumerate(self._subs):
            gi, bi = divmod(i, nb)
            sl = slice(gi * self.cg, (gi + 1) * self.cg)
            c(x[:, sl], out=conv[:, sl], accumulate=bi > 0)
        return Fh.axpby(x, Fh.act(conv, L.ACT_GELU_ERF), 1.0, 1.0)


class Linear(Conv1d):

    def __init__(self, cin, cout, bias=True):
        super().__init__(cin, cout, 1, bias=bias, weight_2d=True)

    def forward(self, x, **kw):
        x3 = x.reshape(x.shape[0], self.cin, 1)
        return super().forward(x3, force_direct=True, **kw)


class LinearCT(Conv1d):

    def __init__(self, cin, cout, bias=True, packed=True):
        super().__init__(cin, cout, 1, bias=bias, weight_2d=True)
        self.packed = packed


class StackedLinearCT(Conv1d):

    def __init__(self, parts):
        super().__init__(parts[0].cin, sum(p.cout for p in parts), 1, bias=True, weight_2d=True)
        del self._parameters["weight"], self._parameters["bias"]
        self.__dict__["_parts"] = tuple(parts)

    def _folded(self):
        return torch.cat([p.weight.data for p in self._parts], 0).contiguous()

    def _bias_src(self):
        return torch.cat([p.bias.data for p in self._parts], 0)


def _set_in(a, x):
    a.x, a.x_bs, a.x_cs, a.x_ts = L.fptr(x), x.stride(0), x.stride(1), x.stride(2)
    a.B, a.Cin, a.Lin = x.shape
    a.zeros = L.fptr(_zeros(x.device))


def _wants_direct(a, force_direct: bool, silu_in: bool) -> bool:
    gated = a.rows in (L.ROWS_GATE_WN, L.ROWS_GATE_GLU)
    return (not gated and a.prologue != L.PRO_ACT1D and not a.ln_c1 and
            bool(force_direct or a.stride != 1 or a.Cin < 8 or a.Cout < 8 or a.Lout < 8 or silu_in))


def _set_out(a, out, B, cout, Lout):
    assert out.shape == (B, cout, Lout), (tuple(out.shape), (B, cout, Lout))
    assert out.stride(2) == 1 or Lout == 1
    a.y, a.y_bs, a.y_cs = L.fptr(out), out.stride(0), out.stride(1)
    a.Cout, a.Lout = cout, Lout


def _set_epilogue(a, act, cbias, mask, mask_mode, cscale, scale, res, accumulate, post_scale, out):
    a.act = act
    if cbias is not None:
        assert cbias.dim() >= 2 and cbias.stride(1) == 1
        a.cbias, a.cbias_bs = L.fptr(cbias), cbias.stride(0)
    if mask is not None and mask_mode != L.MASK_NONE:
        assert mask.stride(-1) == 1
        a.mask, a.mask_bs, a.mask_mode = L.fptr(mask), mask.stride(0), mask_mode
    if cscale is not None:
        assert cscale.stride(1) == 1
        a.cscale, a.cscale_bs = L.fptr(cscale), cscale.stride(0)
    a.scale = float(scale)
    if res is not None:
        assert res.shape == out.shape
        a.res, a.res_bs, a.res_cs = L.fptr(res), res.stride(0), res.stride(1)
        if res.stride(2) != 1 and res.shape[2] != 1:
            if res.stride(2) < 1:
                raise L.HspError("residual with time stride %d: materialise it (copy_strided) before the launch" % res.stride(2))
            a.res_ts = res.stride(2)
    a.accumulate = 1 if accumulate else 0
    a.post_scale = float(post_scale)


def prepare_fft(model: nn.Module) -> int:
    n = 0
    for m in model.modules():
        if isinstance(m, Conv1d) and m._fft:
            n += m.ensure_wf().numel()
    return n


def finalize(model: nn.Module, device, materialize: bool = True) -> WeightArena:
    device = torch.device(device)
    if device.type != "cuda":
        raise L.HspError("finalize() needs a ROCm device: the product path has no CPU fallback")
    L.lib()
    if materialize:
        model.to(device)
    arena = WeightArena()
    layers = [m for m in model.modules() if isinstance(m, HipLayer)]
    for m in layers:
        for name, numel in m.hsp_requests():
            arena.request(m, name, numel)
    with torch.cuda.device(device):
        arena.allocate(device)
        for m in layers:
            m.hsp_fill(arena, materialize)
            m.__dict__["_hsp_stale"] = False
        torch.cuda.current_stream().synchronize()
    model._hsp_arena = arena
    model.__dict__["_hsp_epoch"] = _EPOCH
    return arena
```

Measured before the change: 35.17 million samples/s.

## Fold batch into column dimension for conv/GEMM tiles when time length misaligns

```diff
diff --git a/include/hsp.h b/include/hsp.h
--- a/include/hsp.h
+++ b/include/hsp.h
@@ -86,6 +86,7 @@
   int64_t y2_bs, y2_cs;
   int64_t res_ts;
   int64_t w_bs;
+  int32_t fold_cols;
 } hsp_conv1d_args;
 
 int hsp_conv1d_mfma_f32(const hsp_conv1d_args* a, void* stream);
diff --git a/megatts2_hierspeechpp_amd/_lib.py b/megatts2_hierspeechpp_amd/_lib.py
--- a/megatts2_hierspeechpp_amd/_lib.py
+++ b/megatts2_hierspeechpp_amd/_lib.py
@@ -39,6 +39,7 @@
         ("ln_c1", _fp), ("ln_eps", C.c_float),
         ("split_row", C.c_int32), ("accumulate2", C.c_int32), ("mask_mode2", C.c_int32), ("y2", _fp),
         ("y2_bs", C.c_int64), ("y2_cs", C.c_int64), ("res_ts", C.c_int64), ("w_bs", C.c_int64),
+        ("fold_cols", C.c_int32),
     ]
 
 
diff --git a/megatts2_hierspeechpp_amd/csrc/hsp_bgemm.hip b/megatts2_hierspeechpp_amd/csrc/hsp_bgemm.hip
--- a/megatts2_hierspeechpp_amd/csrc/hsp_bgemm.hip
+++ b/megatts2_hierspeechpp_amd/csrc/hsp_bgemm.hip
@@ -33,6 +33,15 @@
   asm volatile("" ::: "memory");
 }
 
+__device__ __forceinline__ void bg_fold(int v, int b0, int T, int B, int& b, int& t) {
+  b = b0;
+  t = v - b0 * T;
+  while (t >= T && b + 1 < B) {
+    t -= T;
+    ++b;
+  }
+}
+
 typedef const __attribute__((address_space(3))) float* bg_lptr;
 template <int TM, int TN, int G>
 __device__ __forceinline__ void bg_read(float (&A)[bg_gs(TM, TN) * TM], float (&B)[bg_gs(TM, TN) * TN], bg_lptr wa, bg_lptr xa) {
@@ -74,10 +83,12 @@
   }
 }
 
-template <int TM, int TN, bool LN, int ACT>
+template <int TM, int TN, bool LN, int ACT, bool FOLD>
 __device__ __forceinline__ void bg_epilogue(const hsp_conv1d_args& a, const bg_f32x16 (&acc)[TM * TN], int b, int mw, int nw,
                                             int l32, int half, float bvl, float c1l, const float (&mean)[TN],
                                             const float (&rstd)[TN]) {
+  const int lc = FOLD ? 0 : l32;
+  const float* cbl = (FOLD && a.cbias) ? a.cbias + (int64_t)b * a.cbias_bs + 4 * half : nullptr;
 #pragma unroll
   for (int tm = 0; tm < TM; ++tm) {
     float bvr[16], c1r[16];
@@ -88,17 +99,19 @@
       c1r[r] = LN ? __shfl(c1l, src, 64) : 0.0f;
     }
     {
-      const unsigned yo = 4u * (unsigned)(l32 + 4 * half * a.y_cs), ro = 4u * (unsigned)(l32 + 4 * half * a.res_cs);
+      const unsigned yo = 4u * (unsigned)(lc + 4 * half * a.y_cs), ro = 4u * (unsigned)(lc + 4 * half * a.res_cs);
       const char* ybase = reinterpret_cast<const char*>(a.y + (int64_t)b * a.y_bs + nw);
       const char* rbase = a.res ? reinterpret_cast<const char*>(a.res + (int64_t)b * a.res_bs + nw) : nullptr;
 #pragma unroll
       for (int tn = 0; tn < TN; ++tn) {
-        if (nw + tn * 32 + l32 < a.ncols) {
+        if (nw + tn * 32 + lc < a.ncols) {
           float rv[16];
+          [[maybe_unused]] float cb[16];
 #pragma unroll
           for (int r = 0; r < 16; ++r) {
             const int mc = min(mw + tm * 32 + (r & 3) + 8 * (r >> 2), a.Cout - 1 - 4 * half);
             rv[r] = rbase ? *reinterpret_cast<const float*>(rbase + (int64_t)mc * a.res_cs * 4 + tn * 128 + ro) : 0.0f;
+            if constexpr (FOLD) cb[r] = a.cbias ? cbl[mc] : 0.0f;
           }
 #pragma unroll
           for (int q = 0; q < 4; ++q) {
@@ -108,8 +121,10 @@
               for (int i = 0; i < 4; ++i) {
                 const int r = 4 * q + i;
                 const float fin = acc[tm * TN + tn][r];
-                float v = fin + bvr[r];
-                if constexpr (LN) v = fmaf(rstd[tn], fmaf(-mean[tn], c1r[r], fin), bvr[r]);
+                float bv = bvr[r];
+                if constexpr (FOLD) bv = a.cbias ? bv + cb[r] : bv;
+                float v = fin + bv;
+                if constexpr (LN) v = fmaf(rstd[tn], fmaf(-mean[tn], c1r[r], fin), bv);
                 if constexpr (ACT == HSP_ACT_RELU) v = fmaxf(v, 0.0f);
                 else if constexpr (ACT == HSP_ACT_GELU_TANH) v = hsp_apply_act(v, HSP_ACT_GELU_TANH);
                 v += rv[r];
@@ -123,7 +138,7 @@
   }
 }
 
-template <int TM, int TN, int ACT>
+template <int TM, int TN, int ACT, bool FOLD>
 __device__ __forceinline__ void bg_epilogue_ext(const hsp_conv1d_args& a, const bg_f32x16 (&acc)[TM * TN], int b, int m0, int mw,
                                                 int nw, int l32, int half, float bvl) {
   const bool second = a.split_row > 0 && m0 >= a.split_row;
@@ -133,8 +148,11 @@
   const int64_t ycs = second ? a.y2_cs : a.y_cs;
   const char* ybase = reinterpret_cast<const char*>((second ? a.y2 + (int64_t)b * a.y2_bs : a.y + (int64_t)b * a.y_bs) + nw);
   const char* rbase = (a.res && !second) ? reinterpret_cast<const char*>(a.res + (int64_t)b * a.res_bs + nw) : nullptr;
-  const unsigned yo = 4u * (unsigned)(l32 + 4 * half * (int)ycs), ro = 4u * (unsigned)(l32 + 4 * half * a.res_cs);
-  const float csl = a.cscale ? a.cscale[(int64_t)b * a.cscale_bs + min(mw + l32 + 32 * half, a.Cout - 1)] : 1.0f;
+  const int lc = FOLD ? 0 : l32;
+  const unsigned yo = 4u * (unsigned)(lc + 4 * half * (int)ycs), ro = 4u * (unsigned)(lc + 4 * half * a.res_cs);
+  const float csl = (!FOLD && a.cscale) ? a.cscale[(int64_t)b * a.cscale_bs + min(mw + l32 + 32 * half, a.Cout - 1)] : 1.0f;
+  const float* cbl = (FOLD && a.cbias) ? a.cbias + (int64_t)b * a.cbias_bs + mo + 4 * half : nullptr;
+  const float* csp = (FOLD && a.cscale) ? a.cscale + (int64_t)b * a.cscale_bs + mo + 4 * half : nullptr;
   const float sc = a.scale, ps = a.post_scale;
 #pragma unroll
   for (int tm = 0; tm < TM; ++tm) {
@@ -147,16 +165,21 @@
     }
 #pragma unroll
     for (int tn = 0; tn < TN; ++tn) {
-      const int n = nw + tn * 32 + l32;
+      const int n = nw + tn * 32 + lc;
       if (n < a.ncols) {
         const float mk = mmode != HSP_MASK_NONE ? a.mask[(int64_t)b * a.mask_bs + n] : 1.0f;
         const float mk_pre = (mmode & HSP_MASK_PRE) ? mk : 1.0f, mk_post = (mmode & HSP_MASK_POST) ? mk : 1.0f;
         float rv[16], yv[16];
+        [[maybe_unused]] float cb[16], cs[16];
 #pragma unroll
         for (int r = 0; r < 16; ++r) {
           const int mc = min(mw + tm * 32 + (r & 3) + 8 * (r >> 2), a.Cout - 1 - 4 * half) - mo;
           rv[r] = rbase ? *reinterpret_cast<const float*>(rbase + (int64_t)mc * a.res_cs * 4 + tn * 128 + ro) : 0.0f;
           yv[r] = accum ? *reinterpret_cast<const float*>(ybase + (int64_t)mc * ycs * 4 + tn * 128 + yo) : 0.0f;
+          if constexpr (FOLD) {
+            cb[r] = a.cbias ? cbl[mc] : 0.0f;
+            cs[r] = a.cscale ? csp[mc] : 1.0f;
+          }
         }
 #pragma unroll
         for (int q = 0; q < 4; ++q) {
@@ -165,11 +188,13 @@
 #pragma unroll
             for (int i = 0; i < 4; ++i) {
               const int r = 4 * q + i;
-              float v = acc[tm * TN + tn][r] + bvr[r];
+              float bv = bvr[r];
+              if constexpr (FOLD) bv = a.cbias ? bv + cb[r] : bv;
+              float v = acc[tm * TN + tn][r] + bv;
               if constexpr (ACT == HSP_ACT_RELU) v = fmaxf(v, 0.0f);
               else if constexpr (ACT == HSP_ACT_GELU_TANH) v = hsp_apply_act(v, HSP_ACT_GELU_TANH);
               v *= mk_pre;
-              v *= csr[r];
+              v *= FOLD ? cs[r] : csr[r];
               v *= sc;
               v += rv[r];
               v *= mk_post;
@@ -186,7 +211,7 @@
 template <int N>
 __device__ __forceinline__ void bg_wait_vm() { asm volatile("s_waitcnt vmcnt(%0)" ::"n"(N) : "memory"); }
 
-template <int TM, int TN, bool LN, bool EXT>
+template <int TM, int TN, bool LN, bool EXT, bool FOLD>
 __global__ __launch_bounds__(512, 1) void bgemm_kernel(const hsp_conv1d_args a, int n_mt, int n_nt, int per_xcd,
                                                        int total) {
   using C = BgCfg<TM, TN>;
@@ -197,8 +222,10 @@
   const int mt = id % n_mt;
   id /= n_mt;
   const int nt = id % n_nt;
-  const int b = id / n_nt;
   const int m0 = mt * C::BM, n0 = nt * C::BN;
+  static_assert(!FOLD || TN == 1, "a lane of the folded form owns one column");
+  const int b = FOLD ? n0 / a.ncols : id / n_nt;
+  const int ncv = FOLD ? a.B * a.ncols : a.ncols;
   const int tid = threadIdx.x, lane = tid & 63, wave = __builtin_amdgcn_readfirstlane(tid >> 6);
   const int K = a.Cin;
   const int nstage = (K + BG_KS - 1) / BG_KS;
@@ -217,12 +244,14 @@
     constexpr int LPRX = C::BN / 4, RPIX = 64 / LPRX;
     const int rw = lane / LPRW, cw = (lane % LPRW) * 4;
     const int rx = lane / LPRX, cx = (lane % LPRX) * 4;
-    const bool mok = m0 + cw < a.M, nok = n0 + cx < a.ncols;
+    int bx = b, tx = n0 + cx;
+    if constexpr (FOLD) bg_fold(n0 + cx, b, a.ncols, a.B, bx, tx);
+    const bool mok = m0 + cw < a.M, nok = tx < a.ncols;
     const float* wsrc = a.w + m0 + cw;
-    const float* xsrc = a.x + (int64_t)b * a.x_bs + n0 + cx;
-    const bool wfast = m0 + C::BM <= a.M, xfast = n0 + C::BN <= a.ncols && a.x_cs < (1 << 26);
+    const float* xsrc = a.x + (int64_t)bx * a.x_bs + tx;
+    const bool wfast = m0 + C::BM <= a.M, xfast = n0 + C::BN <= ncv && a.x_cs < (1 << 26);
     const float* wlane = a.w + m0 + rw * a.w_ld + cw;
-    const float* xlane = a.x + (int64_t)b * a.x_bs + n0 + (xfast ? rx * (int)a.x_cs : 0) + cx;
+    const float* xlane = a.x + (int64_t)bx * a.x_bs + tx + (xfast ? rx * (int)a.x_cs : 0);
     const int wld = a.w_ld, xcs = (int)a.x_cs;
     auto issue = [&](int s) __attribute__((always_inline)) {
       float* Ws = lds + (s % C::NST) * C::STAGE;
@@ -285,6 +314,8 @@
   const int l32 = lane & 31, half = lane >> 5;
   const int wm = wave & 1, wn = wave >> 1;
   const int mw = m0 + wm * (32 * TM), nw = n0 + wn * (32 * TN);
+  int be = b, ne = nw;
+  if constexpr (FOLD) bg_fold(nw + l32, b, a.ncols, a.B, be, ne);
   bg_f32x16 acc[TM * TN];
 #pragma unroll
   for (int t = 0; t < TM * TN; ++t)
@@ -294,7 +325,7 @@
   {
     const int mc = min(mw + lane, a.Cout - 1);
     bvl = a.bias ? a.bias[mc] : 0.0f;
-    if (a.cbias) bvl += a.cbias[(int64_t)b * a.cbias_bs + mc];
+    if (!FOLD && a.cbias) bvl += a.cbias[(int64_t)b * a.cbias_bs + mc];
     if constexpr (LN) c1l = a.ln_c1[mc];
   }
   constexpr int GS = bg_gs(TM, TN);
@@ -364,24 +395,24 @@
 
   if constexpr (EXT) {
     static_assert(!LN, "the extended epilogue is not built with the fused LayerNorm");
-    if (a.act == HSP_ACT_RELU) bg_epilogue_ext<TM, TN, HSP_ACT_RELU>(a, acc, b, m0, mw, nw, l32, half, bvl);
-    else if (a.act == HSP_ACT_GELU_TANH) bg_epilogue_ext<TM, TN, HSP_ACT_GELU_TANH>(a, acc, b, m0, mw, nw, l32, half, bvl);
-    else bg_epilogue_ext<TM, TN, HSP_ACT_NONE>(a, acc, b, m0, mw, nw, l32, half, bvl);
+    if (a.act == HSP_ACT_RELU) bg_epilogue_ext<TM, TN, HSP_ACT_RELU, FOLD>(a, acc, be, m0, mw, ne, l32, half, bvl);
+    else if (a.act == HSP_ACT_GELU_TANH) bg_epilogue_ext<TM, TN, HSP_ACT_GELU_TANH, FOLD>(a, acc, be, m0, mw, ne, l32, half, bvl);
+    else bg_epilogue_ext<TM, TN, HSP_ACT_NONE, FOLD>(a, acc, be, m0, mw, ne, l32, half, bvl);
   } else {
-    if (a.act == HSP_ACT_RELU) bg_epilogue<TM, TN, LN, HSP_ACT_RELU>(a, acc, b, mw, nw, l32, half, bvl, c1l, mean, rstd);
-    else if (a.act == HSP_ACT_GELU_TANH) bg_epilogue<TM, TN, LN, HSP_ACT_GELU_TANH>(a, acc, b, mw, nw, l32, half, bvl, c1l, mean, rstd);
-    else bg_epilogue<TM, TN, LN, HSP_ACT_NONE>(a, acc, b, mw, nw, l32, half, bvl, c1l, mean, rstd);
+    if (a.act == HSP_ACT_RELU) bg_epilogue<TM, TN, LN, HSP_ACT_RELU, FOLD>(a, acc, be, mw, ne, l32, half, bvl, c1l, mean, rstd);
+    else if (a.act == HSP_ACT_GELU_TANH) bg_epilogue<TM, TN, LN, HSP_ACT_GELU_TANH, FOLD>(a, acc, be, mw, ne, l32, half, bvl, c1l, mean, rstd);
+    else bg_epilogue<TM, TN, LN, HSP_ACT_NONE, FOLD>(a, acc, be, mw, ne, l32, half, bvl, c1l, mean, rstd);
   }
   BG_STAMP(3);
 #undef BG_STAMP
 }
 
-template <int TM, int TN, bool LN, bool EXT>
+template <int TM, int TN, bool LN, bool EXT, bool FOLD>
 int bg_launch(const hsp_conv1d_args& a, hipStream_t s, int n_mt, int n_nt, int total) {
   using C = BgCfg<TM, TN>;
   static_assert(C::LDS_BYTES > 32 * 1024, "every launch raises the LDS limit");
   const int per_xcd = (total + 7) / 8;
-  return hsp_launch<bgemm_kernel<TM, TN, LN, EXT>>(8 * per_xcd, 512, C::LDS_BYTES, C::LDS_BYTES, s, a, n_mt, n_nt, per_xcd, total);
+  return hsp_launch<bgemm_kernel<TM, TN, LN, EXT, FOLD>>(8 * per_xcd, 512, C::LDS_BYTES, C::LDS_BYTES, s, a, n_mt, n_nt, per_xcd, total);
 }
 
 inline bool bg_extended(const hsp_conv1d_args& a) {
@@ -398,9 +429,18 @@
     plan_out[0] = C::BM; plan_out[1] = C::BN; plan_out[2] = -2; plan_out[3] = C::LDS_BYTES;
     return 0;
   }
-  if (bg_extended(a)) return bg_launch<TM, TN, false, true>(a, s, n_mt, n_nt, (int)total);
-  return a.ln_c1 ? bg_launch<TM, TN, true, false>(a, s, n_mt, n_nt, (int)total)
-                 : bg_launch<TM, TN, false, false>(a, s, n_mt, n_nt, (int)total);
+  if constexpr (TM == 1 && TN == 1) {
+    const int64_t vcols = (int64_t)a.B * a.ncols;
+    if (a.fold_cols && a.B > 1 && (a.ncols % C::BN) != 0 && vcols <= 0x3fffffff) {
+      const int n_vt = (int)((vcols + C::BN - 1) / C::BN), tot = n_mt * n_vt;
+      if (bg_extended(a)) return bg_launch<1, 1, false, true, true>(a, s, n_mt, n_vt, tot);
+      return a.ln_c1 ? bg_launch<1, 1, true, false, true>(a, s, n_mt, n_vt, tot)
+                     : bg_launch<1, 1, false, false, true>(a, s, n_mt, n_vt, tot);
+    }
+  }
+  if (bg_extended(a)) return bg_launch<TM, TN, false, true, false>(a, s, n_mt, n_nt, (int)total);
+  return a.ln_c1 ? bg_launch<TM, TN, true, false, false>(a, s, n_mt, n_nt, (int)total)
+                 : bg_launch<TM, TN, false, false, false>(a, s, n_mt, n_nt, (int)total);
 }
 
 }
diff --git a/megatts2_hierspeechpp_amd/csrc/hsp_conv1d_direct.hip b/megatts2_hierspeechpp_amd/csrc/hsp_conv1d_direct.hip
--- a/megatts2_hierspeechpp_amd/csrc/hsp_conv1d_direct.hip
+++ b/megatts2_hierspeechpp_amd/csrc/hsp_conv1d_direct.hip
@@ -209,6 +209,7 @@
   if (a.res && a.res_ts > 1) return HSP_EINVAL;
   if (a.w_bs) return HSP_EINVAL;
   if (a.ln_c1 || a.split_row) return HSP_EINVAL;
+  if (a.fold_cols) return HSP_EINVAL;
   if (linear_vec_fast(a)) {
     const unsigned gx = (unsigned)((a.Cout + 63) / 64), gy = (unsigned)((a.B + LV_BB - 1) / LV_BB);
     if (gy > 65535) return HSP_EINVAL;
diff --git a/megatts2_hierspeechpp_amd/csrc/hsp_conv1d_mfma.hip b/megatts2_hierspeechpp_amd/csrc/hsp_conv1d_mfma.hip
--- a/megatts2_hierspeechpp_amd/csrc/hsp_conv1d_mfma.hip
+++ b/megatts2_hierspeechpp_amd/csrc/hsp_conv1d_mfma.hip
@@ -25,6 +25,7 @@
   if (!a.zeros || (reinterpret_cast<uintptr_t>(a.zeros) & 15) != 0) return HSP_EINVAL;
   if (a.prologue != HSP_PRO_NONE && a.prologue != HSP_PRO_LRELU && a.prologue != HSP_PRO_ACT1D) return HSP_EINVAL;
   if (a.mask_mode != HSP_MASK_NONE && !a.mask) return HSP_EINVAL;
+  if (a.fold_cols != 0 && a.fold_cols != 1) return HSP_EINVAL;
   if (a.rows == HSP_ROWS_GATE_WN || a.rows == HSP_ROWS_GATE_GLU) {
     if (a.gate_half <= 0 || (a.gate_half & 31) || a.M != 2 * a.gate_half || a.Cout != a.gate_half) return HSP_EINVAL;
     if (a.prologue == HSP_PRO_ACT1D) return HSP_EINVAL;
@@ -41,6 +42,7 @@
   const bool act = a.prologue == HSP_PRO_ACT1D;
   const bool short_seq = (int64_t)((a.M + 127) / 128) * ((a.ncols + 127) / 128) * a.B <= 128;
   if (a.res && a.res_ts > 1) {
+    if (a.fold_cols) return HSP_EINVAL;
     const int e = hsp_rgemm_try(a, s, plan_out);
     return e >= 0 ? e : HSP_EINVAL;
   }
@@ -48,7 +50,11 @@
     const int e = hsp_bgemm_try(a, s, plan_out);
     if (e >= 0) return e;
   }
+  hsp_conv1d_args plain = a;
+  plain.fold_cols = 0;
+  int32_t probe[4];
   if ((short_seq || a.ln_c1 || a.split_row || HSP_DBG(a, 1 << 24)) && !a.w_bs && !HSP_DBG(a, 128)) {
+    if (a.fold_cols && hsp_rgemm_try(plain, nullptr, probe) >= 0) return HSP_EINVAL;
     const int e = hsp_rgemm_try(a, s, plan_out);
     if (e >= 0) return e;
   }
@@ -67,6 +73,7 @@
     if (gated) {
       const int64_t t128 = (int64_t)((a.M + 63) / 64) * ((a.ncols + 127) / 128) * a.B;
       if ((t128 <= 48 || (HSP_DBG(a, 1 << 28) && t128 <= 512)) && !HSP_DBG(a, 1 << 27)) {
+        if (a.fold_cols && hsp_conv_tile_S64G2(plain, epi, act, nullptr, probe) != HSP_EINVAL) return HSP_EINVAL;
         const int e = hsp_conv_tile_S64G2(a, epi, act, s, plan_out);
         if (e != HSP_EINVAL) return e;
       }
diff --git a/megatts2_hierspeechpp_amd/csrc/hsp_conv1d_mfma_kernel.h b/megatts2_hierspeechpp_amd/csrc/hsp_conv1d_mfma_kernel.h
--- a/megatts2_hierspeechpp_amd/csrc/hsp_conv1d_mfma_kernel.h
+++ b/megatts2_hierspeechpp_amd/csrc/hsp_conv1d_mfma_kernel.h
@@ -21,8 +21,9 @@
 
 namespace hspconv {
 
-template <int WM, int WN, int TM, int TN, int NPW_, int MINW_, int XSLACK_ = 64, int KS_ = 1>
+template <int WM, int WN, int TM, int TN, int NPW_, int MINW_, int XSLACK_ = 64, int KS_ = 1, bool FOLD_ = false>
 struct Cfg {
+  static constexpr bool kFOLD = FOLD_;
   static constexpr int kKS = KS_;
   static constexpr int NCW = WM * WN * KS_;
   static constexpr int kWM = WM, kWN = WN, kTM = TM, kTN = TN;
@@ -120,6 +121,15 @@
 
 __device__ __forceinline__ void wave_lds_fence() { asm volatile("s_waitcnt lgkmcnt(0)" ::: "memory"); }
 
+__device__ __forceinline__ void fold_col(int col, int ts0, int T, int& i, int& t) {
+  i = 0;
+  t = ts0 + col;
+  while (t >= T) {
+    t -= T;
+    ++i;
+  }
+}
+
 struct ProdArgs {
   const float* w;
   const float* zeros;
@@ -185,6 +195,15 @@
           const float* src = (ci < a.Cin && p >= 0 && p < a.Lin) ? xc + p : a.zeros;
           dma16(src, Xa + kc * P.xwp + 4 * g0);
         }
+      }
+    }
+  }
+  static __device__ __forceinline__ void dma_x_fold(const float* xl, int xs, const float* zeros, int Cin, const LdsPlan& P,
+                                                    float* Xa, int c0, int pw, bool on) {
+    if (on) {
+      for (int kc = pw; kc < P.kc; kc += C::NPW) {
+        const int ci = c0 + kc;
+        dma16(ci < Cin ? xl + (int64_t)ci * xs : zeros, Xa + kc * P.xwp);
       }
     }
   }
@@ -311,18 +330,31 @@
 };
 
 
-template <class C, int EPI, bool ACT, int TM, int TN>
+template <class C, int EPI, bool ACT, int TM, int TN, bool FOLD = false>
 __device__ __forceinline__ void conv_consume(const hsp_conv1d_args& a, const LdsPlan& P, float* const lds, const int b,
                                              const int m0, const int t0, const int p0, const int wm, const int wn,
                                              const int lane, const int nchunks, const int lkc, const int xvec,
-                                             const int ks = 0) {
+                                             const int ks = 0, const int ts0 = 0) {
   constexpr int BM = C::BM;
   const int KC = P.kc;
   __builtin_assume(nchunks > 0);
   const int wave = wm * C::kWN + wn;
   const int l32 = lane & 31, half = lane >> 5;
   const int mw = m0 + wm * (TM * 32);
-  const int tw = t0 + wn * (TN * 32) + l32;
+  int tw = t0 + wn * (TN * 32) + l32;
+  int bl = b;
+  int xfold = 0;
+  if constexpr (FOLD) {
+    static_assert(TN == 1 && C::kKS == 1 && EPI != HSP_EPI_SHUF && !ACT, "folded columns: one column per lane, plain kernels");
+    int i;
+    fold_col(wn * 32 + l32, ts0, a.ncols, i, tw);
+    xfold = 8 * i + 4 - a.pad;
+    bl = b + i;
+    if (bl >= a.B) {
+      bl = a.B - 1;
+      tw = a.ncols;
+    }
+  }
   f32x16 acc[TM][TN];
 
   static_assert(C::kKS == 1 || EPI != HSP_EPI_INIT, "a K split with the accumulator-init epilogue would add the residual once per group");
@@ -358,7 +390,7 @@
           for (int r = 0; r < 16; ++r) add[i][r] = 0.0f;
       }
       if (a.res) {
-        const float* const rb = a.res + (int64_t)b * a.res_bs;
+        const float* const rb = a.res + (int64_t)bl * a.res_bs;
         static_for<TM>([&](auto ii) __attribute__((always_inline)) {
           constexpr int i = decltype(ii)::value;
           static_for<16>([&](auto rr) __attribute__((always_inline)) {
@@ -388,7 +420,7 @@
         });
       });
       if (a.cbias) {
-        const float* const cb = a.cbias + (int64_t)b * a.cbias_bs;
+        const float* const cb = a.cbias + (int64_t)bl * a.cbias_bs;
         static_for<TM>([&](auto ii) __attribute__((always_inline)) {
           constexpr int i = decltype(ii)::value;
           static_for<16>([&](auto rr) __attribute__((always_inline)) {
@@ -402,7 +434,7 @@
         });
       }
       if (a.accumulate) {
-        const float* const yb = a.y + (int64_t)b * a.y_bs;
+        const float* const yb = a.y + (int64_t)bl * a.y_bs;
         static_for<TM>([&](auto ii) __attribute__((always_inline)) {
           constexpr int i = decltype(ii)::value;
           static_for<TN>([&](auto nn) __attribute__((always_inline)) {
@@ -444,7 +476,7 @@
   }
 
   const int wlane = half * BM + wm * (TM * 32) + l32;
-  const int xlane = half * P.xwp + wn * (TN * 32) + l32 + (xvec ? (p0 & 3) : 0);
+  const int xlane = half * P.xwp + wn * (TN * 32) + l32 + (FOLD ? xfold : (xvec ? (p0 & 3) : 0));
   const int nsteps = ((a.K * KC) >> 1) / C::kKS;
 
   HSP_BARRIER(a);
@@ -570,9 +602,10 @@
 
   if (HSP_DBG(a, 16)) return;
   if constexpr (EPI == HSP_EPI_INIT) {
-    float* const yb = a.y + (int64_t)b * a.y_bs;
+    float* const yb = a.y + (int64_t)bl * a.y_bs;
     const int ycs = (int)a.y_cs;
-    const bool full = mw + TM * 32 <= a.Cout && t0 + wn * (TN * 32) + TN * 32 <= a.ncols;
+    const bool full = mw + TM * 32 <= a.Cout &&
+                      t0 + wn * (TN * 32) + TN * 32 <= (FOLD ? a.B * a.ncols : a.ncols);
     const float ps = a.post_scale;
     if (full) {
       const int lrow = mw + 4 * half;
@@ -610,6 +643,16 @@
     float* const stage = lds + wave * (32 * ESTR);
     const int er = lane >> 3, ec = (lane & 7) * 4;
     const float4 z4 = make_float4(0.f, 0.f, 0.f, 0.f);
+    int bv = b, tv = t0 + wn * (TN * 32) + ec;
+    if constexpr (FOLD) {
+      int i;
+      fold_col(wn * 32 + ec, ts0, a.ncols, i, tv);
+      bv = b + i;
+      if (bv >= a.B) {
+        bv = a.B - 1;
+        tv = a.ncols;
+      }
+    }
     static_for<TM>([&](auto ii) __attribute__((always_inline)) {
       constexpr int i = decltype(ii)::value;
       float add[4], cs[4];
@@ -620,13 +663,13 @@
         cs[q] = a.scale;
         if (co < a.Cout) {
           if (a.bias) add[q] = a.bias[co];
-          if (a.cbias) add[q] += a.cbias[(int64_t)b * a.cbias_bs + co];
-          if (a.cscale) cs[q] *= a.cscale[(int64_t)b * a.cscale_bs + co];
+          if (a.cbias) add[q] += a.cbias[(int64_t)bv * a.cbias_bs + co];
+          if (a.cscale) cs[q] *= a.cscale[(int64_t)bv * a.cscale_bs + co];
         }
       }
       static_for<TN>([&](auto nn) __attribute__((always_inline)) {
         constexpr int n = decltype(nn)::value;
-        const int t = t0 + wn * (TN * 32) + n * 32 + ec;
+        const int t = tv + n * 32;
         const bool tok = t < a.ncols;
         float4 rs[4], yo[4];
 #pragma unroll
@@ -635,11 +678,11 @@
           const bool ok = tok && co < a.Cout;
           rs[q] = z4;
           yo[q] = z4;
-          if (ok && a.res) rs[q] = *reinterpret_cast<const float4*>(a.res + (int64_t)b * a.res_bs + (int64_t)co * a.res_cs + t);
-          if (ok && a.accumulate) yo[q] = *reinterpret_cast<const float4*>(a.y + (int64_t)b * a.y_bs + (int64_t)co * a.y_cs + t);
+          if (ok && a.res) rs[q] = *reinterpret_cast<const float4*>(a.res + (int64_t)bv * a.res_bs + (int64_t)co * a.res_cs + t);
+          if (ok && a.accumulate) yo[q] = *reinterpret_cast<const float4*>(a.y + (int64_t)bv * a.y_bs + (int64_t)co * a.y_cs + t);
         }
         float4 mk = make_float4(1.f, 1.f, 1.f, 1.f);
-        if (a.mask_mode != HSP_MASK_NONE && tok) mk = *reinterpret_cast<const float4*>(a.mask + (int64_t)b * a.mask_bs + t);
+        if (a.mask_mode != HSP_MASK_NONE && tok) mk = *reinterpret_cast<const float4*>(a.mask + (int64_t)bv * a.mask_bs + t);
         static_for<16>([&](auto rr) __attribute__((always_inline)) {
           constexpr int r = decltype(rr)::value;
           stage[HSP_ACC_ROW(r, half) * ESTR + l32] = acc[i][n][r];
@@ -662,7 +705,7 @@
               if (a.mask_mode & HSP_MASK_POST) x *= m4[u];
               e[u] = (x + y4[u]) * a.post_scale;
             }
-            *reinterpret_cast<float4*>(a.y + (int64_t)b * a.y_bs + (int64_t)co * a.y_cs + t) =
+            *reinterpret_cast<float4*>(a.y + (int64_t)bv * a.y_bs + (int64_t)co * a.y_cs + t) =
                 make_float4(e[0], e[1], e[2], e[3]);
           }
         }
@@ -686,11 +729,11 @@
               float va = acc[i][n][r], vb = acc[i + 1][n][r];
               if (a.bias) { va += a.bias[co]; vb += a.bias[H + co]; }
               if (a.cbias) {
-                va += a.cbias[(int64_t)b * a.cbias_bs + co];
-                vb += a.cbias[(int64_t)b * a.cbias_bs + H + co];
+                va += a.cbias[(int64_t)bl * a.cbias_bs + co];
+                vb += a.cbias[(int64_t)bl * a.cbias_bs + H + co];
               }
               const float v = (a.rows == HSP_ROWS_GATE_WN ? hsp_tanh(va) : va) * hsp_sigmoid(vb);
-              hsp_epilogue_store(a, b, co, t, v);
+              hsp_epilogue_store(a, bl, co, t, v);
             }
           });
         }
@@ -805,9 +848,9 @@
             if (ok) {
               float v = acc[i][n][r];
               if (a.bias) v += a.bias[co];
-              if (a.cbias) v += a.cbias[(int64_t)b * a.cbias_bs + co];
+              if (a.cbias) v += a.cbias[(int64_t)bl * a.cbias_bs + co];
               v = hsp_apply_act(v, a.act);
-              hsp_epilogue_store(a, b, co, to, v);
+              hsp_epilogue_store(a, bl, co, to, v);
             }
           });
         }
@@ -821,7 +864,7 @@
   return EPI == HSP_EPI_INIT && !ACT && C::kWM * C::kWN == 4 && C::kTM * C::kWM == 4 && C::kTN * C::kWN == 4;
 }
 
-template <class C, int EPI, bool ACT>
+template <class C, int EPI, bool ACT, bool FOLD = false>
 __global__ __launch_bounds__(C::THREADS, C::MINW) void conv1d_mfma_kernel(const hsp_conv1d_args a, const int n_mt,
                                                                           const int n_nt, const int lkc,
                                                                           const int xvec, const int sched) {
@@ -847,7 +890,10 @@
   }
   int nt, b;
   bool tail_tile = false;
-  if (sched >> 8) {
+  if constexpr (FOLD) {
+    nt = ct;
+    b = (nt * BN) / a.ncols;
+  } else if (sched >> 8) {
     const int n_main = (n_nt - 1) * a.B;
     if (ct < n_main) {
       nt = ct % (n_nt - 1);
@@ -863,6 +909,7 @@
   }
   const int m0 = mt * BM, t0 = nt * BN;
   const int p0 = t0 - a.pad;
+  const int ts0 = FOLD ? t0 - b * a.ncols : 0;
 
   const int wave = __builtin_amdgcn_readfirstlane(threadIdx.x >> 6);
   const int lane = threadIdx.x & 63;
@@ -877,7 +924,35 @@
     using PR = Prod<C>;
     float* const Ws0 = lds;
     float* const Xa0 = lds + P.xa_off;
-    if constexpr (!ACT) {
+    if constexpr (FOLD) {
+      const int T = a.ncols;
+      const int ngrp = (BN + 8 * ((BN + T - 1) / T + 1)) >> 2;
+      int q = 4 * lane + ts0, piece = 0;
+      while (q >= T + 8) {
+        q -= T + 8;
+        ++piece;
+      }
+      const bool inside = b + piece < a.B && q >= 4 && q < T + 4;
+      const float* const xl = inside ? a.x + (int64_t)(b + piece) * a.x_bs + (q - 4) : a.zeros;
+      const int xs = inside ? (int)a.x_cs : 0;
+      const bool wfast = m0 + BM <= a.M && (a.Cin & (KC - 1)) == 0;
+      const float* const wtile = wb + m0;
+      const unsigned wofs = 4u * (unsigned)((lane / PR::CPR) * a.w_ld + (lane % PR::CPR) * 4);
+      auto stage = [&](int c0, float* Ws, float* Xa) __attribute__((always_inline)) {
+        if (wfast) PR::dma_w_fast(wtile, a.w_ld, a.Cin, a.K, P, Ws, c0, pw, wofs);
+        else PR::dma_w(pa, P, Ws, c0, m0, pw, lane);
+        PR::dma_x_fold(xl, xs, a.zeros, a.Cin, P, Xa, c0, pw, lane < ngrp);
+        wait_vm0();
+        if (a.prologue == HSP_PRO_LRELU) PR::lrelu_x(pa, P, Xa, pw, lane);
+      };
+      stage(0, Ws0, Xa0);
+      HSP_BARRIER(a);
+      for (int c = 0; c < nchunks; ++c) {
+        const int nb = (c + 1) & 1;
+        if (c + 1 < nchunks && !HSP_DBG(a, 1)) stage((c + 1) << lkc, Ws0 + nb * P.ws_sz, Xa0 + nb * P.xa_sz);
+        HSP_BARRIER(a);
+      }
+    } else if constexpr (!ACT) {
       const int p0a = p0 & ~3;
       const bool fast = xvec && m0 + BM <= a.M && (a.Cin & (KC - 1)) == 0 && !HSP_DBG(a, 512);
       if (fast) {
@@ -950,7 +1025,9 @@
       return;
     }
   }
-  if constexpr (C::kKS > 1) {
+  if constexpr (FOLD) {
+    conv_consume<C, EPI, ACT, TM, TN, true>(a, P, lds, b, m0, t0, p0, wave / C::kWN, wave % C::kWN, lane, nchunks, lkc, xvec, 0, ts0);
+  } else if constexpr (C::kKS > 1) {
     const int ks = wave / (C::kWM * C::kWN), w2 = wave % (C::kWM * C::kWN);
     conv_consume<C, EPI, ACT, TM, TN>(a, P, lds, b, m0, t0, p0, w2 / C::kWN, w2 % C::kWN, lane, nchunks, lkc, xvec, ks);
   } else {
@@ -979,7 +1056,22 @@
 }
 
 template <class C, int EPI, bool ACT>
+constexpr bool has_fold_path() {
+  return C::kFOLD && !ACT && EPI != HSP_EPI_SHUF;
+}
+
+template <class C>
+bool fold_fits(const hsp_conv1d_args& a, bool xvec) {
+  const int T = a.ncols;
+  if (!a.fold_cols || a.B < 2 || !xvec || (T & 3) || (T % C::BN) == 0 || a.w_bs) return false;
+  if (a.Lin != T || a.Lout != T || a.pad > 4 || (a.K - 1) * a.dil - a.pad > 4) return false;
+  if (C::BN + 8 * ((C::BN + T - 1) / T + 1) > C::XWP) return false;
+  return (int64_t)a.B * T <= 0x3fffffff;
+}
+
+template <class C, int EPI, bool ACT>
 int launch_one(const hsp_conv1d_args& a, hipStream_t s, int32_t* plan_out) {
+  if (a.fold_cols && !has_fold_path<C, EPI, ACT>()) return HSP_EINVAL;
   const int64_t tiles = (int64_t)((a.M + C::BM - 1) / C::BM) * ((a.ncols + C::BN - 1) / C::BN) * a.B;
   const bool deep_k3 = HSP_DBG(a, 1 << 29) && a.K <= 3;
   const bool two_per_cu = !deep_k3 && (C::MINW * 256 >= 2 * C::THREADS || ((tiles > 256 || HSP_DBG(a, 1 << 26)) && tiles <= 512 && !HSP_DBG(a, 1 << 21)));
@@ -1018,6 +1110,17 @@
   auto al16 = [](const void* p) { return (reinterpret_cast<uintptr_t>(p) & 15) == 0; };
   const bool xvec = !ACT && a.x_ts == 1 && (a.Lin & 3) == 0 && (a.x_cs & 3) == 0 && (a.x_bs & 3) == 0 && al16(a.x) &&
                     !HSP_DBG(a, 64);
+  if constexpr (has_fold_path<C, EPI, ACT>()) {
+    if (fold_fits<C>(a, xvec)) {
+      auto kfold = conv1d_mfma_kernel<C, EPI, ACT, true>;
+      static hsp_lds_flags fflags;
+      if (lds_bytes > 32 * 1024)
+        if (int e = hsp_raise_lds_limit(reinterpret_cast<const void*>(kfold), kMaxLdsBytes, fflags)) return e;
+      const int n_vt = (int)(((int64_t)a.B * a.ncols + C::BN - 1) / C::BN);
+      hipLaunchKernelGGL(kfold, dim3((unsigned)(n_mt * n_vt)), dim3(C::THREADS), lds_bytes, s, a, n_mt, n_vt, lkc, 1, 0);
+      return (int)hipGetLastError();
+    }
+  }
   hipLaunchKernelGGL(kern, dim3((unsigned)blocks), dim3(C::THREADS), lds_bytes, s, a, n_mt, n_nt, lkc, xvec ? 1 : 0, sched);
   return (int)hipGetLastError();
 }
@@ -1040,8 +1143,8 @@
 using M32 = Cfg<1, 4, 1, 4, 8, 3>;
 using M64P = Cfg<1, 4, 2, 2, 4, 4>;
 using M32P = Cfg<1, 4, 1, 4, 4, 4>;
-using S64 = Cfg<2, 2, 1, 1, 4, 2>;
-using S64G = Cfg<1, 4, 2, 1, 4, 2>;
+using S64 = Cfg<2, 2, 1, 1, 4, 2, 64, 1, true>;
+using S64G = Cfg<1, 4, 2, 1, 4, 2, 64, 1, true>;
 using S32 = Cfg<1, 4, 1, 1, 4, 2>;
 using S64W = Cfg<2, 2, 1, 1, 4, 2, 128>;
 using S64GW = Cfg<1, 4, 2, 1, 4, 2, 128>;
diff --git a/megatts2_hierspeechpp_amd/hip_layers.py b/megatts2_hierspeechpp_amd/hip_layers.py
--- a/megatts2_hierspeechpp_amd/hip_layers.py
+++ b/megatts2_hierspeechpp_amd/hip_layers.py
@@ -16,6 +16,7 @@
 
 LAUNCH_HOOK = None
 DEBUG_FLAGS = 0
+FOLD_COLS = os.environ.get("HSP_FOLD_COLS", "1")
 
 
 _ZEROS = {}
@@ -169,6 +170,31 @@
     if SURVEY_ABI:
         fn = L.lib().hsp_convtr1d_f32 if a.rows == L.ROWS_SHUFFLE else L.lib().hsp_conv1d_f32
     return _bracket(kind, lambda: fn(C.byref(a), L.stream_ptr()), flops, nbytes, a, soft=soft)[0]
+
+
+def _set_fold_cols(a) -> None:
+    a.fold_cols = 0
+    if FOLD_COLS != "0" and a.B > 1 and a.ncols % 4 == 0:
+        a.debug = DEBUG_FLAGS
+        plan = (C.c_int32 * 4)()
+        gated = a.rows in (L.ROWS_GATE_WN, L.ROWS_GATE_GLU)
+        if L.lib().hsp_conv1d_mfma_plan(C.byref(a), C.byref(plan)) == 0 and \
+                FOLD_COLS in ("1", "gemm" if plan[2] == -2 else "conv") and \
+                fold_cols_wanted(plan, a.B, a.ncols, gated=gated, halo=(a.K - 1) * a.dil, act1d=a.prologue == L.PRO_ACT1D):
+            a.fold_cols = 1
+
+
+def fold_cols_kernel(plan, gated: bool = False, halo: int = 0, act1d: bool = False) -> bool:
+    bm, bn, kc = int(plan[0]), int(plan[1]), int(plan[2])
+    if kc == -2:
+        return True
+    return kc > 0 and not act1d and halo + 3 <= 64 and (bm, bn) == ((64, 128) if gated else (64, 64))
+
+
+def fold_cols_wanted(plan, B: int, ncols: int, gated: bool = False, halo: int = 0, act1d: bool = False) -> bool:
+    if B < 2 or ncols % 4 != 0 or ncols % int(plan[1]) == 0 or (int(plan[2]) == -2 and int(plan[0]) != 64):
+        return False
+    return fold_cols_kernel(plan, gated, halo, act1d)
 
 
 def _round_up(x: int, m: int) -> int:
@@ -654,8 +680,11 @@
             a.y2, a.y2_bs, a.y2_cs = L.fptr(out2), out2.stride(0), out2.stride(1)
             flops = 2 * B * self.cout * Cin * Lout
             nbytes += 4 * B * (self.cout - split_row) * Lout * (1 + bool(acc2))
+            _set_fold_cols(a)
             rc = _launch("hsp_conv1d_mfma_f32", L.lib().hsp_conv1d_mfma_f32, a, flops, nbytes, soft=True, keep=keep)
             return None if rc else (out, out2)
+        if not direct:
+            _set_fold_cols(a)
         if self._pre_norm is not None:
             if _DEFER.get() is None and not _launch(kind, fn, a, flops, nbytes, soft=True, keep=keep):
                 return out
@@ -663,6 +692,8 @@
             _set_in(a, xn)
             a.ln_c1 = None
             keep += (xn,)
+            if not direct:
+                _set_fold_cols(a)
         _launch(kind, fn, a, flops, nbytes, keep=keep)
         return out
 
```

Result: faster. 35.69 million samples/s, median of 6 (+1.5%).
